# jihun1998/AO

Measured on AMD Instinct MI355X. Metric: points/sec fwd+bwd PTv2m2 S3DIS, higher is better.
Workload: dtype fp32

## Files before the change

ao_amd/_abi.py:

```python
import ctypes
import os
import re

HEADER = os.path.normpath(os.path.join(os.path.dirname(os.path.abspath(__file__)), "..", "include", "ptv2_hip.h"))

_VALUES = {"int": ctypes.c_int, "unsigned": ctypes.c_uint, "float": ctypes.c_float, "double": ctypes.c_double,
           "long long": ctypes.c_longlong, "size_t": ctypes.c_size_t}
_POINTEES = ("void", "char", "unsigned long long")
_TYPE = re.compile(r"\s*(unsigned\s+long\s+long|long\s+long|unsigned\b|\w+)(.*)", re.S)
_DECLARATOR = re.compile(r"\s*((?:\*\s*)*)(\w+)\s*(?:\[([^\]]*)\])?\s*")
_ITEM = re.compile(r"""
    ^[ \t]*\#[ \t]*define[ \t]+(?P<define>\w+)[ \t]+(?P<value>\S.*?)[ \t]*$
  | ^[ \t]*\#[ \t]*(?:include\b.*|ifndef\b.*|endif\b.*|define[ \t]+\w+[ \t]*)$
  | \benum\s*\{(?P<enum>[^{}]*)\}\s*;
  | \btypedef\s+struct\s+(?P<tag>\w+)\s*\{(?P<fields>[^{}]*)\}\s*(?P<struct>\w+)\s*;
  | (?P<result>[\w\s*]+?)\b(?P<function>\w+)\s*\((?P<params>[^(){};]*)\)\s*;
""", re.M | re.X)


def _const_expr(text, consts, where):
    expr = re.sub(r"[A-Za-z_]\w*", lambda m: str(consts[m.group()]) if m.group() in consts else m.group(), text)
    if not re.fullmatch(r"[\d\s+\-*()]+", expr):
        raise RuntimeError("ao_amd: %s: `%s` is not an integer constant expression of known names" % (where, text.strip()))
    try:
        return int(eval(expr, {"__builtins__": {}}))
    except SyntaxError:
        raise RuntimeError("ao_amd: %s: cannot evaluate `%s`" % (where, text.strip())) from None


def _declarations(text, structs, consts, where, fields):
    m = _TYPE.match(re.sub(r"\b(const|volatile)\b", " ", text))
    base = " ".join(m.group(1).split()) if m else None
    out = []
    for decl in m.group(2).split(",") if m else [""]:
        d = _DECLARATOR.fullmatch(decl)
        if d is None:
            raise RuntimeError("ao_amd: %s: cannot read the declaration `%s`" % (where, " ".join(text.split())))
        stars, name, bound = d.group(1).count("*"), d.group(2), d.group(3)
        value = _VALUES.get(base) or (structs.get(base) if fields else None)
        if stars or (bound is not None and not fields):
            if value is None and base not in _POINTEES and base not in structs:
                raise RuntimeError("ao_amd: %s: unknown type `%s` of `%s`" % (where, base, name))
            ctype = ctypes.c_char_p if (base, stars, bound) == ("char", 1, None) else ctypes.c_void_p
        elif value is None:
            raise RuntimeError("ao_amd: %s: no ctypes type for `%s` of `%s`" % (where, base, name))
        else:
            ctype = value
        if bound is not None and fields:
            ctype = ctype * _const_expr(bound, consts, "%s, bound of `%s`" % (where, name))
        out.append((name, ctype))
    return out


def parse(text):
    text = re.sub(r"/\*.*?\*/", " ", text, flags=re.S)
    text = re.sub(r"^[ \t]*#[ \t]*ifdef[ \t]+__cplusplus\b.*?^[ \t]*#[ \t]*endif\b.*?$", " ", text, flags=re.S | re.M)
    consts, structs, signatures = {}, {}, {}
    at = 0
    for m in _ITEM.finditer(text):
        if text[at:m.start()].strip():
            break
        at = m.end()
        if m.group("define"):
            consts[m.group("define")] = _const_expr(m.group("value"), consts, "#define " + m.group("define"))
        elif m.group("enum") is not None:
            value = -1
            for item in filter(None, (i.strip() for i in m.group("enum").split(","))):
                name, _, init = (s.strip() for s in item.partition("="))
                value = _const_expr(init, consts, "enumerator " + name) if init else value + 1
                consts[name] = value
        elif m.group("struct"):
            name = m.group("struct")
            if name != m.group("tag"):
                raise RuntimeError("ao_amd: typedef struct %s is named %s" % (m.group("tag"), name))
            fields = [f for line in m.group("fields").split(";") if line.strip()
                      for f in _declarations(line, structs, consts, "struct " + name, True)]
            structs[name] = type(name, (ctypes.Structure,), {"_fields_": fields})
        elif m.group("function"):
            name, params = m.group("function"), m.group("params").strip()
            where = "prototype of " + name
            (_, restype), = _declarations(m.group("result") + " result", structs, consts, where, False)
            signatures[name] = (restype, [] if params in ("", "void") else [
                ctype for p in params.split(",") for _, ctype in _declarations(p, structs, consts, where, False)])
    rest = text[at:].strip()
    if rest:
        raise RuntimeError("ao_amd: cannot read this declaration of the C header: `%s`" % " ".join(rest.split())[:160])
    return consts, structs, signatures


if not os.path.exists(HEADER):
    raise RuntimeError("ao_amd: %s not found: the ctypes bindings are derived from it" % HEADER)
with open(HEADER) as _f:
    consts, structs, signatures = parse(_f.read())

DATA_HEADER = os.path.join(os.path.dirname(HEADER), "ptv2_data_hip.h")
if not os.path.exists(DATA_HEADER):
    raise RuntimeError("ao_amd: %s not found: the ctypes bindings are derived from it" % DATA_HEADER)
with open(DATA_HEADER) as _f:
    data_consts, data_structs, data_signatures = parse(_f.read())

REFINE_HEADER = os.path.join(os.path.dirname(HEADER), "ptv2_refine_hip.h")
if not os.path.exists(REFINE_HEADER):
    raise RuntimeError("ao_amd: %s not found: the ctypes bindings are derived from it" % REFINE_HEADER)
with open(REFINE_HEADER) as _f:
    refine_consts, refine_structs, refine_signatures = parse(_f.read())

PP2S_HEADER = os.path.join(os.path.dirname(HEADER), "ptv2_pp2s_hip.h")
if not os.path.exists(PP2S_HEADER):
    raise RuntimeError("ao_amd: %s not found: the ctypes bindings are derived from it" % PP2S_HEADER)
with open(PP2S_HEADER) as _f:
    pp2s_consts, pp2s_structs, pp2s_signatures = parse(_f.read())

PTV1_HEADER = os.path.join(os.path.dirname(HEADER), "ptv2_ptv1_hip.h")
if not os.path.exists(PTV1_HEADER):
    raise RuntimeError("ao_amd: %s not found: the ctypes bindings are derived from it" % PTV1_HEADER)
with open(PTV1_HEADER) as _f:
    ptv1_consts, ptv1_structs, ptv1_signatures = parse(_f.read())

SPCONV_HEADER = os.path.join(os.path.dirname(HEADER), "ptv2_spconv_hip.h")
if not os.path.exists(SPCONV_HEADER):
    raise RuntimeError("ao_amd: %s not found: the ctypes bindings are derived from it" % SPCONV_HEADER)
with open(SPCONV_HEADER) as _f:
    spconv_consts, spconv_structs, spconv_signatures = parse(_f.read())

PG_HEADER = os.path.join(os.path.dirname(HEADER), "ptv2_pg_hip.h")
if not os.path.exists(PG_HEADER):
    raise RuntimeError("ao_amd: %s not found: the ctypes bindings are derived from it" % PG_HEADER)
with open(PG_HEADER) as _f:
    pg_consts, pg_structs, pg_signatures = parse(_f.read())

MSC_HEADER = os.path.join(os.path.dirname(HEADER), "ptv2_msc_hip.h")
if not os.path.exists(MSC_HEADER):
    raise RuntimeError("ao_amd: %s not found: the ctypes bindings are derived from it" % MSC_HEADER)
with open(MSC_HEADER) as _f:
    msc_consts, msc_structs, msc_signatures = parse(_f.read())

ST_HEADER = os.path.join(os.path.dirname(HEADER), "ptv2_st_hip.h")
if not os.path.exists(ST_HEADER):
    raise RuntimeError("ao_amd: %s not found: the ctypes bindings are derived from it" % ST_HEADER)
with open(ST_HEADER) as _f:
    st_consts, st_structs, st_signatures = parse(_f.read())

INSEVAL_HEADER = os.path.join(os.path.dirname(HEADER), "ptv2_inseval_hip.h")
if not os.path.exists(INSEVAL_HEADER):
    raise RuntimeError("ao_amd: %s not found: the ctypes bindings are derived from it" % INSEVAL_HEADER)
with open(INSEVAL_HEADER) as _f:
    inseval_consts, inseval_structs, inseval_signatures = parse(_f.read())
```

ao_amd/_lib.py:

```python
import ctypes
import os
import subprocess

import torch

from . import _abi

_HERE = os.path.dirname(os.path.abspath(__file__))
LIB_PATH = os.path.join(_HERE, "lib", "libptv2_hip.so")
CSRC = os.path.join(_HERE, "csrc")

_SIGNATURES = _abi.signatures

_ERR = {1: "PTV2_ERR_ARG (invalid argument)", 2: "PTV2_ERR_WORKSPACE (workspace too small)",
        3: "PTV2_ERR_LAUNCH (HIP launch failed)"}
_lib = None
EXPECTED_ABI = 11
EXPECTED_DATA_ABI = 1
EXPECTED_REFINE_ABI = 1
EXPECTED_PP2S_ABI = 1
EXPECTED_PTV1_ABI = 1
EXPECTED_SPCONV_ABI = 1
EXPECTED_PG_ABI = 1
EXPECTED_MSC_ABI = 1
EXPECTED_ST_ABI = 1
EXPECTED_INSEVAL_ABI = 1


def build(verbose=False):
    cmd = ["make", "-C", CSRC, "-j4", "all"]
    subprocess.check_call(cmd, stdout=None if verbose else subprocess.DEVNULL)
    return LIB_PATH


def lib():
    global _lib
    if _lib is None:
        if not os.path.exists(LIB_PATH):
            raise RuntimeError(
                "ao_amd: %s not found. Build it with `python -c 'import __graft_entry__ as g; g.build()'` "
                "or `make -C ao_amd/csrc` (needs hipcc). There is no CPU fallback." % LIB_PATH)
        handle = ctypes.CDLL(LIB_PATH)
        for table in (_SIGNATURES, _abi.data_signatures, _abi.refine_signatures, _abi.pp2s_signatures,
                      _abi.ptv1_signatures, _abi.spconv_signatures, _abi.pg_signatures, _abi.msc_signatures,
                      _abi.st_signatures, _abi.inseval_signatures):
            for name, (res, args) in table.items():
                try:
                    fn = getattr(handle, name)
                except AttributeError:
                    raise RuntimeError("ao_amd: %s has no `%s` -- stale build; rebuild with `make -C ao_amd/csrc`"
                                       % (LIB_PATH, name)) from None
                fn.restype = res
                fn.argtypes = args
        have = handle.ptv2_abi_version()
        if have != EXPECTED_ABI:
            raise RuntimeError("ao_amd: %s has ABI version %d, the python side expects %d -- stale build; rebuild with "
                               "`make -C ao_amd/csrc`" % (LIB_PATH, have, EXPECTED_ABI))
        have = handle.ptv2_data_abi_version()
        if have != EXPECTED_DATA_ABI:
            raise RuntimeError("ao_amd: %s has data ABI version %d, the python side expects %d -- stale build; rebuild with "
                               "`make -C ao_amd/csrc`" % (LIB_PATH, have, EXPECTED_DATA_ABI))
        have = handle.ptv2_refine_abi_version()
        if have != EXPECTED_REFINE_ABI:
            raise RuntimeError("ao_amd: %s has refine ABI version %d, the python side expects %d -- stale build; rebuild with "
                               "`make -C ao_amd/csrc`" % (LIB_PATH, have, EXPECTED_REFINE_ABI))
        have = handle.ptv2_pp2s_abi_version()
        if have != EXPECTED_PP2S_ABI:
            raise RuntimeError("ao_amd: %s has pp2s ABI version %d, the python side expects %d -- stale build; rebuild with "
                               "`make -C ao_amd/csrc`" % (LIB_PATH, have, EXPECTED_PP2S_ABI))
        have = handle.ptv2_ptv1_abi_version()
        if have != EXPECTED_PTV1_ABI:
            raise RuntimeError("ao_amd: %s has ptv1 ABI version %d, the python side expects %d -- stale build; rebuild with "
                               "`make -C ao_amd/csrc`" % (LIB_PATH, have, EXPECTED_PTV1_ABI))
        have = handle.ptv2_spconv_abi_version()
        if have != EXPECTED_SPCONV_ABI:
            raise RuntimeError("ao_amd: %s has spconv ABI version %d, the python side expects %d -- stale build; rebuild with "
                               "`make -C ao_amd/csrc`" % (LIB_PATH, have, EXPECTED_SPCONV_ABI))
        if handle.ptv2_spconv_struct_bytes(0) != ctypes.sizeof(_abi.spconv_structs["spconv_tables"]):
            raise RuntimeError("ao_amd: spconv_tables is %d bytes in python, %d in %s (stale build)" % (
                ctypes.sizeof(_abi.spconv_structs["spconv_tables"]), handle.ptv2_spconv_struct_bytes(0), LIB_PATH))
        have = handle.ptv2_pg_abi_version()
        if have != EXPECTED_PG_ABI:
            raise RuntimeError("ao_amd: %s has pg ABI version %d, the python side expects %d -- stale build; rebuild with "
                               "`make -C ao_amd/csrc`" % (LIB_PATH, have, EXPECTED_PG_ABI))
        if handle.ptv2_pg_struct_bytes(0) != ctypes.sizeof(_abi.pg_structs["pg_csr"]):
            raise RuntimeError("ao_amd: pg_csr is %d bytes in python, %d in %s (stale build)" % (
                ctypes.sizeof(_abi.pg_structs["pg_csr"]), handle.ptv2_pg_struct_bytes(0), LIB_PATH))
        have = handle.ptv2_msc_abi_version()
        if have != EXPECTED_MSC_ABI:
            raise RuntimeError("ao_amd: %s has msc ABI version %d, the python side expects %d -- stale build; rebuild with "
                               "`make -C ao_amd/csrc`" % (LIB_PATH, have, EXPECTED_MSC_ABI))
        have = handle.ptv2_st_abi_version()
        if have != EXPECTED_ST_ABI:
            raise RuntimeError("ao_amd: %s has st ABI version %d, the python side expects %d -- stale build; rebuild with "
                               "`make -C ao_amd/csrc`" % (LIB_PATH, have, EXPECTED_ST_ABI))
        if handle.ptv2_st_struct_bytes(0) != ctypes.sizeof(_abi.st_structs["st_args"]):
            raise RuntimeError("ao_amd: st_args is %d bytes in python, %d in %s (stale build)" % (
                ctypes.sizeof(_abi.st_structs["st_args"]), handle.ptv2_st_struct_bytes(0), LIB_PATH))
        have = handle.ptv2_inseval_abi_version()
        if have != EXPECTED_INSEVAL_ABI:
            raise RuntimeError("ao_amd: %s has inseval ABI version %d, the python side expects %d -- stale build; rebuild "
                               "with `make -C ao_amd/csrc`" % (LIB_PATH, have, EXPECTED_INSEVAL_ABI))
        for which, name in enumerate(("ptv1_params", "ptv1_norms", "ptv1_grads")):
            if handle.ptv2_ptv1_struct_bytes(which) != ctypes.sizeof(_abi.ptv1_structs[name]):
                raise RuntimeError("ao_amd: %s is %d bytes in python, %d in %s (stale build)" % (
                    name, ctypes.sizeof(_abi.ptv1_structs[name]), handle.ptv2_ptv1_struct_bytes(which), LIB_PATH))
        for which, name in enumerate(("ptv2_aug_step", "ptv2_aug_program")):
            if handle.ptv2_data_struct_bytes(which) != ctypes.sizeof(_abi.data_structs[name]):
                raise RuntimeError("ao_amd: %s is %d bytes in python, %d in %s (stale build)" % (
                    name, ctypes.sizeof(_abi.data_structs[name]), handle.ptv2_data_struct_bytes(which), LIB_PATH))
        _lib = handle
    return _lib


def check_struct(which, mirror):
    have, want = lib().ptv2_struct_bytes(which), ctypes.sizeof(mirror)
    if have != want:
        raise RuntimeError("ao_amd: %s is %d bytes in python, %d in %s (stale build or a drifted mirror)"
                           % (mirror.__name__, want, have, LIB_PATH))


def check(status, what):
    if status != 0:
        raise RuntimeError("ao_amd: %s failed with status %d: %s" % (what, status, _ERR.get(status, "?")))


def stream_ptr():
    return torch.cuda.current_stream().cuda_stream


def require_cuda(*tensors):
    for t in tensors:
        if t is not None and not t.is_cuda:
            raise RuntimeError("ao_amd ops run on the GPU only (got a %s tensor); there is no CPU fallback" % t.device)


def ptr(t):
    return 0 if t is None else t.data_ptr()


_WS = {}


def workspace(nbytes, device):
    nbytes = max(int(nbytes), 256)
    key = (device.index if device.index is not None else torch.cuda.current_device(),
           torch.cuda.current_stream(device).cuda_stream)
    buf = _WS.get(key)
    if buf is None or buf.numel() < nbytes:
        buf = torch.empty(int(nbytes * 1.25) + 4096, dtype=torch.uint8, device=device)
        _WS[key] = buf
    return buf


def kernel_timer(enable, only=None, stride=1):
    L = lib()
    kid = -1
    if only is not None:
        name = ctypes.create_string_buffer(64)
        us, cnt, byt = ctypes.c_double(), ctypes.c_longlong(), ctypes.c_double()
        for i in range(L.ptv2_profile_kernel_count()):
            L.ptv2_profile_read(i, name, ctypes.byref(us), ctypes.byref(cnt), ctypes.byref(byt))
            if name.value.decode() == only:
                kid = i
        if kid < 0:
            raise ValueError("unknown kernel name %r" % only)
    L.ptv2_profile_select(kid)
    L.ptv2_profile_stride(int(stride))
    L.ptv2_profile_enable(1 if enable else 0)


def graph_stats(reset=False):
    out = (ctypes.c_double * 9)()
    lib().ptv2_graph_stats(out, 1 if reset else 0)
    keys = ("scopes", "updated", "instantiated", "declined", "nodes", "capture_us", "update_us", "launch_us", "wait_us")
    return dict(zip(keys, [float(v) for v in out]))


def kernel_timer_read():
    L = lib()
    out = {}
    name = ctypes.create_string_buffer(64)
    us, cnt, byt = ctypes.c_double(), ctypes.c_longlong(), ctypes.c_double()
    for kid in range(L.ptv2_profile_kernel_count()):
        if L.ptv2_profile_read(kid, name, ctypes.byref(us), ctypes.byref(cnt), ctypes.byref(byt)) == 0 and cnt.value > 0:
            out[name.value.decode()] = dict(launches=cnt.value, total_us=us.value, avg_us=us.value / cnt.value,
                                            bytes_per_launch=byt.value)
    return out
```

ao_amd/csrc/abi.hip:

```cpp
#include <algorithm>
#include <cstdlib>
#include <cstring>
#include <mutex>
#include <unordered_map>
#include <vector>

#include "gva_common.h"

extern "C" int ptv2_abi_version(void) { return 11; }

extern "C" long long ptv2_struct_bytes(int which) {
    switch (which) {
        case 0: return (long long)sizeof(ptv2_block);
        case 1: return (long long)sizeof(ptv2_block_grads);
        case 2: return (long long)sizeof(ptv2_model);
        case 3: return (long long)sizeof(ptv2_gva_block);
        case 4: return (long long)sizeof(ptv2_scene_geo);
        default: return -1;
    }
}

namespace { thread_local int g_matmul_bf16 = 0; }
int ptv2_matmul_bf16(void) { return g_matmul_bf16; }
void ptv2_set_matmul_bf16(int on) { g_matmul_bf16 = on ? 1 : 0; }
extern "C" int ptv2_matmul_precision(int bf16) {
    const int prev = g_matmul_bf16;
    if (bf16 >= 0) g_matmul_bf16 = bf16 ? 1 : 0;
    return prev;
}

namespace gva {
namespace { thread_local PtvDrop g_drop{1.f, 0u, 0u}; }
PtvDrop ptv2_attn_drop_current() { return g_drop; }
void ptv2_attn_drop_set(float p, unsigned seed) {
    if (!(p > 0.f)) { g_drop = PtvDrop{1.f, 0u, 0u}; return; }
    const double pp = p < 1.f ? (double)p : 1.0;
    const double t = pp * 4294967296.0;
    g_drop.thresh = t >= 4294967295.0 ? 4294967295u : (unsigned)t;
    if (g_drop.thresh == 0u) g_drop.thresh = 1u;
    g_drop.scale = pp < 1.0 ? (float)(1.0 / (1.0 - pp)) : 0.f;
    g_drop.seed = seed;
}
PtvAttnDropScope::~PtvAttnDropScope() { g_drop = prev; }
}

namespace gva {
namespace {
thread_local int g_defer_depth = 0;
thread_local PtvRiders g_pending{};
__global__ __launch_bounds__(256) void rider_kernel(PtvRiders Rs) { rider_run(Rs, blockIdx.x); }
void launch_alone(const PtvRider &r, hipStream_t st) {
    PtvRiders one{};
    one.count = 1;
    one.r[0] = r;
    hipLaunchKernelGGL(rider_kernel, dim3(r.blocks), dim3(256), 0, st, one);
}
}
bool ptv2_rider_defer_active() {
    static const bool off = ptv2_env_is("AO_AMD_RIDERS", '0');
    return g_defer_depth > 0 && !off;
}
void ptv2_rider_defer_depth(int delta) { g_defer_depth += delta; }
void ptv2_rider_defer(const PtvRider &r, hipStream_t st) {
    if (g_pending.count == RIDER_QUEUE) {
        launch_alone(g_pending.r[0], st);
        for (int i = 1; i < RIDER_QUEUE; ++i) g_pending.r[i - 1] = g_pending.r[i];
        g_pending.count = RIDER_QUEUE - 1;
    }
    g_pending.r[g_pending.count++] = r;
}
PtvRiders ptv2_rider_take() {
    const PtvRiders out = g_pending;
    g_pending.count = 0;
    return out;
}
void ptv2_rider_flush(hipStream_t st) {
    for (int i = 0; i < g_pending.count; ++i) launch_alone(g_pending.r[i], st);
    g_pending.count = 0;
}
int ptv2_rider_drop() {
    const int had = g_pending.count;
    g_pending.count = 0;
    return had;
}
}

#ifndef PTV2_SRC_HASH
#define PTV2_SRC_HASH "unknown"
#endif

extern "C" const char *ptv2_build_info(void) {
    return "libptv2_hip gfx950 (MI355X) src " PTV2_SRC_HASH " hipcc " __VERSION__ " built " __DATE__;
}

extern "C" int basket_scatter_rows_host(float *dst, long long dst_rows, const long long *ids, const float *src, long long rows,
                                        int c) {
    if (!dst || !ids || !src || rows < 0 || c < 1 || dst_rows < 0) return PTV2_ERR_ARG;
    for (long long r = 0; r < rows; ++r)
        if (ids[r] < 0 || ids[r] >= dst_rows) return PTV2_ERR_ARG;
    for (long long r = 0; r < rows; ++r) memcpy(dst + ids[r] * c, src + r * c, sizeof(float) * (size_t)c);
    return PTV2_OK;
}

namespace {
std::mutex g_cnt_mu;
struct CounterKey {
    int device;
    hipStream_t stream;
    bool operator==(const CounterKey &o) const { return device == o.device && stream == o.stream; }
};
struct CounterKeyHash {
    size_t operator()(const CounterKey &k) const { return std::hash<void *>()((void *)k.stream) * 31u + (size_t)k.device; }
};
std::unordered_map<CounterKey, unsigned *, CounterKeyHash> g_counters;
}

unsigned *ptv2_stream_counters(hipStream_t st) {
    int device = 0;
    if (hipGetDevice(&device) != hipSuccess) return nullptr;
    std::lock_guard<std::mutex> lk(g_cnt_mu);
    const CounterKey key{device, st};
    auto it = g_counters.find(key);
    if (it != g_counters.end()) return it->second;
    unsigned *p = nullptr;
    if (hipMalloc((void **)&p, sizeof(unsigned) * PTV2_NUM_COUNTERS) != hipSuccess) return nullptr;
    if (hipMemsetAsync(p, 0, sizeof(unsigned) * PTV2_NUM_COUNTERS, st) != hipSuccess) return nullptr;
    g_counters[key] = p;
    return p;
}

namespace {
const char *kNames[KID_COUNT] = {
    "knn_row_query_kernel [family]", "logits_fwd_kernel [family]", "softmax_rows_kernel [family]", "aggregate_tile_kernel [family]",
    "peb_fwd_kernel [family]", "peb_bwd_kernel<8>", "aggregate_bwd_tile_kernel [family]", "aggregate_bwd_rows_kernel [family]",
    "aggregate_bwd_gv_kernel<8>", "logits_bwd_rows_kernel [family]", "logits_bwd_gather_kernel", "logits_bwd_params_kernel [family]",
    "linear_wgrad_kernel [family]", "bn_stats_kernel", "bn_apply_kernel [family]", "bn_bwd_reduce_kernel [family]",
    "bn_bwd_apply_kernel [family]", "skinny_fwd_kernel", "skinny_bwd_kernel", "rows_gemm_kernel<48, false, 32> [family]",
    "rows_gemm_kernel<48, false, 64> [family]", "rows_gemm_kernel<48, true, 32> [family]", "rows_gemm_kernel<48, true, 64> [family]",
    "rows_gemm_kernel<64, false, 32> [family]", "rows_gemm_kernel<64, false, 64> [family]", "rows_gemm_kernel<64, true, 32> [family]",
    "rows_gemm_kernel<64, true, 64> [family]",
    "attention_bwd_point_kernel<6, 48, 1, true>",
    "attention_bwd_point_kernel<12, 96, 1, false>", "attention_bwd_point_kernel<24, 192, 2, false>",
    "attention_bwd_point_kernel<48, 384, 4, false>", "attention_bwd_point_kernel<64, 512, 4, false>",
    "linear_wgrad_lds_kernel [family]",
    "grouped_wgrad_kernel_jobs", "attention_fwd_point6_kernel",
    "logits_bwd_fused6_kernel<48>", "logits_bwd_fused_kernel<12, 96, 1>", "logits_bwd_fused_kernel<24, 192, 4>",
    "logits_bwd_fused_kernel<48, 384, 4>", "logits_bwd_fused_kernel<64, 512, 4>",
    "bn_bwd_apply_residual_kernel", "bn_bwd_finapply_kernel [family]",
    "attention_fwd_tile_kernel<12, 96, 12>", "attention_fwd_tile_kernel<24, 192, 12>", "attention_fwd_tile_kernel<48, 384, 12>",
    "attention_fwd_tile_kernel<64, 512, 16>", "wp2_wgrad_tile_kernel_jobs",
    "attention_bwd_tile_kernel<12, 96, 8>", "attention_bwd_tile_kernel<24, 192, 8>", "attention_bwd_tile_kernel<48, 384, 8>",
    "attention_bwd_tile_kernel<64, 512, 8>", "aug_points_kernel"};
struct Rec { hipEvent_t a, b; double bytes; };
std::mutex g_mu;
int g_on = 0;
int g_only = -1;
int g_stride = 1;
unsigned g_seen[KID_COUNT];
std::vector<hipEvent_t> g_free;
hipEvent_t take_event() {
    if (!g_free.empty()) { hipEvent_t e = g_free.back(); g_free.pop_back(); return e; }
    hipEvent_t e = nullptr;
    if (hipEventCreate(&e) != hipSuccess) return nullptr;
    return e;
}
std::vector<Rec> g_recs[KID_COUNT];
std::vector<hipEvent_t> g_pending[KID_COUNT];
constexpr int STAMP_CAP = 1 << 15;
unsigned long long *g_stamp_buf = nullptr;
double g_stamp_us_per_tick = 0.01;
int g_stamp_n = 0;
struct StampRec { int slot; double bytes; };
std::vector<StampRec> g_stamp_recs[KID_COUNT];
std::vector<int> g_stamp_pending[KID_COUNT];
unsigned g_scope_period[GRAPH_SLOTS][KID_COUNT];
unsigned g_scope_phase[GRAPH_SLOTS];
thread_local unsigned t_scope_seen[KID_COUNT];
thread_local int t_scope_which = -1;
__global__ void stamp_kernel(unsigned long long *p) {
    if (threadIdx.x == 0) *p = wall_clock64();
// ... 161 lines not shown
```

ao_amd/csrc/common.h:

```cpp
#pragma once
#include <hip/hip_runtime.h>
#include <stdint.h>
#include <stdlib.h>

#include "../../include/ptv2_hip.h"

#define WAVE 64

#define PTV2_CHECK_LAUNCH()                         \
    do {                                            \
        if (hipGetLastError() != hipSuccess) return PTV2_ERR_LAUNCH; \
    } while (0)

#define RUN(call)                        \
    do {                                 \
        int rc_ = (call);                \
        if (rc_ != PTV2_OK) return rc_;  \
    } while (0)

static inline int divup(long long a, long long b) { return (int)((a + b - 1) / b); }

static constexpr size_t ptv2_align256(size_t v) { return (v + 255) & ~(size_t)255; }
struct PtvCarver {
    char *p; size_t off;
    char *take(size_t bytes) { char *r = p ? p + off : nullptr; off += ptv2_align256(bytes); return r; }
    template <class T> T *take_n(size_t count) { return (T *)take(sizeof(T) * count); }
};

static inline bool ptv2_env_set(const char *name) { return getenv(name) != nullptr; }
static inline bool ptv2_env_is(const char *name, char c) { const char *e = getenv(name); return e && e[0] == c; }

enum PtvKernelId {
    KID_KNN_QUERY = 0, KID_LOGITS_FWD, KID_SOFTMAX_ROWS, KID_AGG_TILE, KID_PEB_FWD, KID_PEB_BWD, KID_BWD_TILE,
    KID_BWD_ROWS, KID_BWD_GV, KID_LOGITS_BWD_ROWS, KID_LOGITS_BWD_GATHER, KID_LOGITS_BWD_PARAMS, KID_WGRAD,
    KID_BN_STATS, KID_BN_APPLY, KID_BN_BWD_REDUCE, KID_BN_BWD_APPLY, KID_SKINNY_FWD, KID_SKINNY_BWD, KID_ROWS_GEMM,  KID_BWD_POINT = KID_ROWS_GEMM + 8,
     KID_WGRAD_LDS = KID_BWD_POINT + 5 ,
    KID_WGRAD_GROUPED ,
    KID_FWD_POINT ,
    KID_LOGITS_BWD_FUSED ,
    KID_BN_BWD_APPLY_RES = KID_LOGITS_BWD_FUSED + 5 ,
    KID_BN_BWD_FINAPPLY ,
    KID_FWD_TILE ,
    KID_WGRAD_TILE = KID_FWD_TILE + 4 ,
    KID_BWD_TILE_K ,
    KID_AUG_POINTS = KID_BWD_TILE_K + 4 ,
    KID_COUNT
};
extern "C" int ptv2_profile_is_on(void);
int ptv2_profile_wants(int kid);
void ptv2_profile_begin(int kid, hipStream_t st);
void ptv2_profile_end(int kid, hipStream_t st, double algorithmic_bytes);
struct PtvScopedTimer {
    int kid; hipStream_t st; double bytes; bool on;
    PtvScopedTimer(int k, hipStream_t s, double b) : kid(k), st(s), bytes(b), on(ptv2_profile_wants(k) != 0) {
        if (on) ptv2_profile_begin(kid, st);
    }
    ~PtvScopedTimer() { if (on) ptv2_profile_end(kid, st, bytes); }
};

enum PtvGraphSlot { GRAPH_MODEL_FWD = 0, GRAPH_MODEL_BWD = 1, GRAPH_MODEL_FWD_PREFIX = 2, GRAPH_MODEL_FWD_REST = 3, GRAPH_SLOTS = 4 };
struct PtvGraphScope {
    void *st, *cap; int which, ring_entry; bool active; long long t0;
    PtvGraphScope(void *stream, int which, bool allow = true);
    void *stream() const { return cap; }
    int finish(int rc);
    ~PtvGraphScope();
    PtvGraphScope(const PtvGraphScope &) = delete;
    PtvGraphScope &operator=(const PtvGraphScope &) = delete;
};
int ptv2_graph_capturing(void);
int ptv2_profile_stamps(void);
int ptv2_zero_async(void *p, size_t bytes, hipStream_t st);

void ptv2_wgrad_defer_begin(void *arena, size_t bytes);
bool ptv2_wgrad_defer_active();
float *ptv2_wgrad_defer_alloc(size_t floats);
void ptv2_wgrad_defer_arm(bool on);
void ptv2_wgrad_defer_arm_rs(bool on);
bool ptv2_wgrad_defer_armed_rs();
struct PtvWgradArm {
    explicit PtvWgradArm(bool on) { ptv2_wgrad_defer_arm(on); }
    ~PtvWgradArm() { ptv2_wgrad_defer_arm(false); }
    PtvWgradArm(const PtvWgradArm &) = delete;
    PtvWgradArm &operator=(const PtvWgradArm &) = delete;
};
struct PtvWgradArmRs {
    explicit PtvWgradArmRs(bool on) { ptv2_wgrad_defer_arm_rs(on); }
    ~PtvWgradArmRs() { ptv2_wgrad_defer_arm_rs(false); }
    PtvWgradArmRs(const PtvWgradArmRs &) = delete;
    PtvWgradArmRs &operator=(const PtvWgradArmRs &) = delete;
};
int ptv2_wgrad_defer_flush(void *stream);
void ptv2_wgrad_defer_end();
size_t ptv2_wgrad_defer_table_bytes();

int ptv2_matmul_bf16(void);
void ptv2_set_matmul_bf16(int on);
struct PtvMatmulScope {
    int prev;
    explicit PtvMatmulScope(int on) : prev(ptv2_matmul_bf16()) { ptv2_set_matmul_bf16(on); }
    ~PtvMatmulScope() { ptv2_set_matmul_bf16(prev); }
};
typedef __bf16 ptv2_bf16x8 __attribute__((ext_vector_type(8)));
__device__ __forceinline__ ptv2_bf16x8 ptv2_pack_bf16(float4 lo, float4 hi) {
    ptv2_bf16x8 r;
    r[0] = (__bf16)lo.x; r[1] = (__bf16)lo.y; r[2] = (__bf16)lo.z; r[3] = (__bf16)lo.w;
    r[4] = (__bf16)hi.x; r[5] = (__bf16)hi.y; r[6] = (__bf16)hi.z; r[7] = (__bf16)hi.w;
    return r;
}

static __device__ __attribute__((aligned(16), unused)) float ptv2_zero_pad[1024];
template <class T>
__device__ __forceinline__ T ptv2_ld_or_zero(const T *p, bool ok) {
    return *(ok ? p : (const T *)ptv2_zero_pad);
}

#define PTV2_NUM_COUNTERS 64
enum PtvCounterSlot { CNT_LOGITS_FWD = 0, CNT_BP2, CNT_LOGITS_BWD_ROWS, CNT_CE, CNT_LOVASZ, CNT_BN_TILES = 16  };
unsigned *ptv2_stream_counters(hipStream_t st);

__device__ __forceinline__ float ref_d2(float qx, float qy, float qz, float x, float y, float z) {
    float dx = qx - x, dy = qy - y, dz = qz - z;
    return __builtin_fmaf(dz, dz, __builtin_fmaf(dx, dx, dy * dy));
}

__device__ __forceinline__ int seg_of(int pt, const int *__restrict__ offset, int b) {
    int lo = 0, hi = b - 1;
    while (lo < hi) {
        int mid = (lo + hi) >> 1;
        if (pt < offset[mid]) hi = mid; else lo = mid + 1;
    }
    return lo;
}

__device__ __forceinline__ int f2ord(float f) {
    int i = __float_as_int(f);
    return i >= 0 ? i : i ^ 0x7fffffff;
}
__device__ __forceinline__ float ord2f(int i) {
    return __int_as_float(i >= 0 ? i : i ^ 0x7fffffff);
}

__device__ __forceinline__ unsigned long long shfl_xor_u64(unsigned long long v, int m) {
    unsigned lo = (unsigned)v, hi = (unsigned)(v >> 32);
    lo = __shfl_xor(lo, m, WAVE);
    hi = __shfl_xor(hi, m, WAVE);
    return ((unsigned long long)hi << 32) | lo;
}

__device__ __forceinline__ int xcd_remap(int orig, int nwg) {
    int q = nwg >> 3, r = nwg & 7, x = orig & 7;
    return (x < r ? x * (q + 1) : r * (q + 1) + (x - r) * q) + (orig >> 3);
}

#include "internal.h"
```

ao_amd/csrc/gather_ops.hip:

```cpp
#include "common.h"

namespace {

constexpr int TPB = 256;
inline int grid_for(long long work) { return (int)std::min<long long>(divup(work, TPB), 256 * 8); }

template <int VEC>
__global__ __launch_bounds__(TPB) void grouping_fwd(long long total, int cv, const float *__restrict__ input,
                                                    const int *__restrict__ idx, float *__restrict__ output) {
    for (long long e = (long long)blockIdx.x * TPB + threadIdx.x; e < total; e += (long long)gridDim.x * TPB) {
        long long row = e / cv;
        int ci = (int)(e - row * cv);
        int src = idx[row];
        if (VEC == 4) {
            float4 v = make_float4(0.f, 0.f, 0.f, 0.f);
            if (src >= 0) v = ((const float4 *)input)[(long long)src * cv + ci];
            ((float4 *)output)[e] = v;
        } else {
            output[e] = src >= 0 ? input[(long long)src * cv + ci] : 0.f;
        }
    }
}

__global__ __launch_bounds__(TPB) void grouping_bwd(long long total, int c, const float *__restrict__ grad_output,
// ... 139 lines not shown
}

__global__ __launch_bounds__(TPB) void aggregation_bwd(long long total, int nsample, int c, int w_c,
                                                       const float *__restrict__ input,
                                                       const float *__restrict__ position,
                                                       const float *__restrict__ weight,
                                                       const int *__restrict__ idx,
                                                       const float *__restrict__ grad_output, float *grad_input,
                                                       float *__restrict__ grad_position, float *grad_weight) {
    for (long long e = (long long)blockIdx.x * TPB + threadIdx.x; e < total; e += (long long)gridDim.x * TPB) {
        long long ni = e / c;
        int ci = (int)(e - ni * c);
        int wi = ci % w_c;
        float go = grad_output[e];
        for (int s = 0; s < nsample; ++s) {
            long long ii = ni * nsample + s;
            long long src = (long long)idx[ii] * c + ci;
            float w = weight[ii * w_c + wi];
            atomicAdd(grad_input + src, go * w);
            grad_position[ii * c + ci] = go * w;
            atomicAdd(grad_weight + ii * w_c + wi, go * (input[src] + position[ii * c + ci]));
        }
    }
}

__global__ __launch_bounds__(TPB) void attn_relation_fwd(long long total, int g, int c,
                                                         const float *__restrict__ query,
                                                         const float *__restrict__ key,
                                                         const float *__restrict__ weight,
                                                         const int *__restrict__ tgt, const int *__restrict__ ref,
                                                         float *output) {
    for (long long e = (long long)blockIdx.x * TPB + threadIdx.x; e < total; e += (long long)gridDim.x * TPB) {
        long long r = e / g;
        int gi = (int)(e - r * g);
        const float *q = query + ((long long)tgt[r] * g + gi) * c;
        const float *k = key + ((long long)ref[r] * g + gi) * c;
        float acc = output[e];
        for (int ci = 0; ci < c; ++ci) acc += q[ci] * k[ci] * weight[ci];
        output[e] = acc;
    }
}

__global__ __launch_bounds__(TPB) void attn_relation_bwd(long long total, int g, int c,
                                                         const float *__restrict__ query, float *grad_query,
                                                         const float *__restrict__ key, float *grad_key,
                                                         const float *__restrict__ weight, float *grad_weight,
                                                         const int *__restrict__ tgt, const int *__restrict__ ref,
                                                         const float *__restrict__ grad_output) {
    for (long long e = (long long)blockIdx.x * TPB + threadIdx.x; e < total; e += (long long)gridDim.x * TPB) {
        long long rg = e / c;
        int ci = (int)(e - rg * c);
        long long r = rg / g;
        int gi = (int)(rg - r * g);
        long long qi = ((long long)tgt[r] * g + gi) * c + ci;
        long long ki = ((long long)ref[r] * g + gi) * c + ci;
        float gr = grad_output[rg];
        float qv = query[qi], kv = key[ki], wv = weight[ci];
        atomicAdd(grad_query + qi, gr * kv * wv);
        atomicAdd(grad_key + ki, gr * qv * wv);
        atomicAdd(grad_weight + ci, gr * kv * qv);
    }
}

__global__ __launch_bounds__(TPB) void attn_fusion_fwd(long long total, int g, int c,
                                                       const float *__restrict__ weight,
                                                       const float *__restrict__ value,
                                                       const int *__restrict__ tgt, const int *__restrict__ ref,
                                                       float *output) {
    for (long long e = (long long)blockIdx.x * TPB + threadIdx.x; e < total; e += (long long)gridDim.x * TPB) {
        long long rg = e / c;
        int ci = (int)(e - rg * c);
        long long r = rg / g;
        int gi = (int)(rg - r * g);
        float f = weight[rg] * value[((long long)ref[r] * g + gi) * c + ci];
        atomicAdd(output + ((long long)tgt[r] * g + gi) * c + ci, f);
    }
}

__global__ __launch_bounds__(TPB) void attn_fusion_bwd(long long total, int g, int c,
                                                       const float *__restrict__ weight, float *grad_weight,
                                                       const float *__restrict__ value, float *grad_value,
                                                       const int *__restrict__ tgt, const int *__restrict__ ref,
                                                       const float *__restrict__ grad_output) {
    for (long long e = (long long)blockIdx.x * TPB + threadIdx.x; e < total; e += (long long)gridDim.x * TPB) {
        long long r = e / g;
        int gi = (int)(e - r * g);
        long long oi = ((long long)tgt[r] * g + gi) * c;
        long long vi = ((long long)ref[r] * g + gi) * c;
        float w = weight[e];
        float acc = grad_weight[e];
        for (int ci = 0; ci < c; ++ci) {
            float go = grad_output[oi + ci];
            acc += go * value[vi + ci];
            atomicAdd(grad_value + vi + ci, go * w);
        }
        grad_weight[e] = acc;
    }
}

inline bool aligned16(const void *p) { return ((uintptr_t)p & 15) == 0; }

}

#define ST ((hipStream_t)stream)

extern "C" int grouping_forward_hip_launcher(int m, int nsample, int c, const float *input, const int *idx,
                                             float *output, void *stream) {
    if (m < 0 || nsample < 0 || c < 0) return PTV2_ERR_ARG;
    long long rows = (long long)m * nsample;
    if (rows == 0 || c == 0) return PTV2_OK;
    if (c % 4 == 0 && aligned16(input) && aligned16(output)) {
        long long total = rows * (c / 4);
        hipLaunchKernelGGL(grouping_fwd<4>, dim3(grid_for(total)), dim3(TPB), 0, ST, total, c / 4, input, idx, output);
    } else {
        long long total = rows * c;
        hipLaunchKernelGGL(grouping_fwd<1>, dim3(grid_for(total)), dim3(TPB), 0, ST, total, c, input, idx, output);
    }
    PTV2_CHECK_LAUNCH();
    return PTV2_OK;
}

extern "C" int grouping_backward_hip_launcher(int m, int nsample, int c, const float *grad_output,
                                              const int *idx, float *grad_input, void *stream) {
    if (m < 0 || nsample < 0 || c < 0) return PTV2_ERR_ARG;
    long long total = (long long)m * nsample * c;
    if (total == 0) return PTV2_OK;
    hipLaunchKernelGGL(grouping_bwd, dim3(grid_for(total)), dim3(TPB), 0, ST, total, c, grad_output, idx, grad_input);
    PTV2_CHECK_LAUNCH();
    return PTV2_OK;
}

__global__ __launch_bounds__(256) void interpolation_weights_kernel(long long m, int k, int n, const float *__restrict__ dist2,
                                                                    int *__restrict__ idx, float *__restrict__ weight) {
    for (long long i = (long long)blockIdx.x * 256 + threadIdx.x; i < m; i += (long long)gridDim.x * 256) {
        float r[8];
        float norm = 0.f;
        for (int s = 0; s < k; ++s) {
            r[s & 7] = __fdiv_rn(1.0f, __fadd_rn(__fsqrt_rn(dist2[i * k + s]), 1e-8f));
            norm = __fadd_rn(norm, r[s & 7]);
        }
        for (int s = 0; s < k; ++s) {
            weight[i * k + s] = __fdiv_rn(r[s & 7], norm);
            const int j = idx[i * k + s];
            if (j < 0) idx[i * k + s] = j + n;
        }
    }
}

extern "C" int interpolation_weights_hip_launcher(int m, int k, int n, const float *dist2, int *idx, float *weight, void *stream) {
    if (m < 0 || k < 1 || k > 8 || n < 0) return PTV2_ERR_ARG;
    if (m == 0) return PTV2_OK;
    if (!dist2 || !idx || !weight) return PTV2_ERR_ARG;
    const int nblk = (int)std::min<long long>(((long long)m + 255) / 256, 256 * 8);
    hipLaunchKernelGGL(interpolation_weights_kernel, dim3(nblk), dim3(256), 0, (hipStream_t)stream, (long long)m, k, n, dist2, idx,
                       weight);
    PTV2_CHECK_LAUNCH();
    return PTV2_OK;
}

extern "C" int interpolation_forward_hip_launcher(int n, int c, int k, const float *input, const int *idx,
                                                  const float *weight, float *output, void *stream) {
    if (n < 0 || c < 0 || k < 0) return PTV2_ERR_ARG;
    long long total = (long long)n * c;
    if (total == 0) return PTV2_OK;
    hipLaunchKernelGGL(interpolation_fwd, dim3(grid_for(total)), dim3(TPB), 0, ST, total, c, k, input, idx, weight,
                       output);
    PTV2_CHECK_LAUNCH();
    return PTV2_OK;
}

extern "C" int interpolation_backward_hip_launcher(int n, int c, int k, const float *grad_output,
                                                   const int *idx, const float *weight, float *grad_input,
                                                   void *stream) {
    if (n < 0 || c < 0 || k < 0) return PTV2_ERR_ARG;
    long long total = (long long)n * c;
    if (total == 0) return PTV2_OK;
    hipLaunchKernelGGL(interpolation_bwd, dim3(grid_for(total)), dim3(TPB), 0, ST, total, c, k, grad_output, idx,
                       weight, grad_input);
    PTV2_CHECK_LAUNCH();
    return PTV2_OK;
}

extern "C" int interpolation_backward_gather_hip_launcher(int m, int c, int k, const float *grad_output, const int *inv_ptr,
                                                          const int *inv_rows, const float *weight, float *grad_input,
                                                          void *stream) {
    if (m < 0 || c < 0 || k < 1 || !inv_ptr || !inv_rows) return PTV2_ERR_ARG;
    if ((long long)m * c == 0) return PTV2_OK;
    if (c % 4 == 0 && aligned16(grad_output) && aligned16(grad_input)) {
        const long long total = (long long)m * (c / 4);
        hipLaunchKernelGGL(interpolation_bwd_gather<4>, dim3(grid_for(total)), dim3(TPB), 0, ST, total, c / 4, k, grad_output,
                           inv_ptr, inv_rows, weight, grad_input);
    } else {
        const long long total = (long long)m * c;
        hipLaunchKernelGGL(interpolation_bwd_gather<1>, dim3(grid_for(total)), dim3(TPB), 0, ST, total, c, k, grad_output, inv_ptr,
                           inv_rows, weight, grad_input);
    }
    PTV2_CHECK_LAUNCH();
    return PTV2_OK;
}

extern "C" int subtraction_forward_hip_launcher(int n, int nsample, int c, const float *input1,
                                                const float *input2, const int *idx, float *output,
                                                void *stream) {
    if (n < 0 || nsample < 0 || c < 0) return PTV2_ERR_ARG;
    long long rows = (long long)n * nsample;
    if (rows == 0 || c == 0) return PTV2_OK;
    if (c % 4 == 0 && aligned16(input1) && aligned16(input2) && aligned16(output)) {
        long long total = rows * (c / 4);
        hipLaunchKernelGGL(subtraction_fwd<4>, dim3(grid_for(total)), dim3(TPB), 0, ST, total, nsample, c / 4, input1,
                           input2, idx, output);
    } else {
        long long total = rows * c;
        hipLaunchKernelGGL(subtraction_fwd<1>, dim3(grid_for(total)), dim3(TPB), 0, ST, total, nsample, c, input1,
                           input2, idx, output);
    }
    PTV2_CHECK_LAUNCH();
    return PTV2_OK;
}

extern "C" int subtraction_backward_hip_launcher(int n, int nsample, int c, const int *idx,
                                                 const float *grad_output, float *grad_input1,
                                                 float *grad_input2, void *stream) {
    if (n < 0 || nsample < 0 || c < 0) return PTV2_ERR_ARG;
    long long total = (long long)n * c;
    if (total == 0) return PTV2_OK;
    hipLaunchKernelGGL(subtraction_bwd, dim3(grid_for(total)), dim3(TPB), 0, ST, total, nsample, c, idx, grad_output,
                       grad_input1, grad_input2);
    PTV2_CHECK_LAUNCH();
    return PTV2_OK;
}

extern "C" int aggregation_forward_hip_launcher(int n, int nsample, int c, int w_c, const float *input,
                                                const float *position, const float *weight, const int *idx,
                                                float *output, void *stream) {
    if (n < 0 || nsample < 0 || c < 0 || w_c < 1) return PTV2_ERR_ARG;
    long long total = (long long)n * c;
    if (total == 0) return PTV2_OK;
    hipLaunchKernelGGL(aggregation_fwd, dim3(grid_for(total)), dim3(TPB), 0, ST, total, nsample, c, w_c, input,
                       position, weight, idx, output);
    PTV2_CHECK_LAUNCH();
    return PTV2_OK;
}

extern "C" int aggregation_backward_hip_launcher(int n, int nsample, int c, int w_c, const float *input,
                                                 const float *position, const float *weight, const int *idx,
                                                 const float *grad_output, float *grad_input,
                                                 float *grad_position, float *grad_weight, void *stream) {
    if (n < 0 || nsample < 0 || c < 0 || w_c < 1) return PTV2_ERR_ARG;
    long long total = (long long)n * c;
    if (total == 0) return PTV2_OK;
    hipLaunchKernelGGL(aggregation_bwd, dim3(grid_for(total)), dim3(TPB), 0, ST, total, nsample, c, w_c, input,
                       position, weight, idx, grad_output, grad_input, grad_position, grad_weight);
    PTV2_CHECK_LAUNCH();
    return PTV2_OK;
}

extern "C" int attention_relation_step_forward_hip_launcher(int m, int g, int c, const float *query,
                                                            const float *key, const float *weight,
                                                            const int *index_target, const int *index_refer,
                                                            float *output, void *stream) {
    if (m < 0 || g < 0 || c < 0) return PTV2_ERR_ARG;
    long long total = (long long)m * g;
    if (total == 0) return PTV2_OK;
    hipLaunchKernelGGL(attn_relation_fwd, dim3(grid_for(total)), dim3(TPB), 0, ST, total, g, c, query, key, weight,
                       index_target, index_refer, output);
    PTV2_CHECK_LAUNCH();
    return PTV2_OK;
}

extern "C" int attention_relation_step_backward_hip_launcher(int m, int g, int c, const float *query,
                                                             float *grad_query, const float *key,
                                                             float *grad_key, const float *weight,
                                                             float *grad_weight, const int *index_target,
                                                             const int *index_refer, const float *grad_output,
                                                             void *stream) {
    if (m < 0 || g < 0 || c < 0) return PTV2_ERR_ARG;
    long long total = (long long)m * g * c;
    if (total == 0) return PTV2_OK;
    hipLaunchKernelGGL(attn_relation_bwd, dim3(grid_for(total)), dim3(TPB), 0, ST, total, g, c, query, grad_query, key,
                       grad_key, weight, grad_weight, index_target, index_refer, grad_output);
    PTV2_CHECK_LAUNCH();
    return PTV2_OK;
}

extern "C" int attention_fusion_step_forward_hip_launcher(int m, int g, int c, const float *weight,
                                                          const float *value, const int *index_target,
                                                          const int *index_refer, float *output, void *stream) {
    if (m < 0 || g < 0 || c < 0) return PTV2_ERR_ARG;
    long long total = (long long)m * g * c;
    if (total == 0) return PTV2_OK;
    hipLaunchKernelGGL(attn_fusion_fwd, dim3(grid_for(total)), dim3(TPB), 0, ST, total, g, c, weight, value,
                       index_target, index_refer, output);
    PTV2_CHECK_LAUNCH();
    return PTV2_OK;
}

extern "C" int attention_fusion_step_backward_hip_launcher(int m, int g, int c, const float *weight,
                                                           float *grad_weight, const float *value,
                                                           float *grad_value, const int *index_target,
                                                           const int *index_refer, const float *grad_output,
                                                           void *stream) {
    if (m < 0 || g < 0 || c < 0) return PTV2_ERR_ARG;
    long long total = (long long)m * g;
    if (total == 0) return PTV2_OK;
    hipLaunchKernelGGL(attn_fusion_bwd, dim3(grid_for(total)), dim3(TPB), 0, ST, total, g, c, weight, grad_weight,
                       value, grad_value, index_target, index_refer, grad_output);
    PTV2_CHECK_LAUNCH();
// ... 3 lines not shown
```

ao_amd/csrc/gridpool.hip:

```cpp
#include <hipcub/hipcub.hpp>

#include <algorithm>

#include "common.h"

namespace {

constexpr int TPB = 256;
struct PoolDims {
    long long nx, ny, nz;
    long long total;
};
constexpr int KEY_BITS = 48;

__device__ __forceinline__ PoolDims pool_dims_of(int b, const float *__restrict__ lo, const float *__restrict__ hi, float size) {
    float e[3] = {0.f, 0.f, 0.f};
    for (int s = 0; s < b; ++s)
        for (int a = 0; a < 3; ++a) e[a] = fmaxf(e[a], hi[3 * s + a] - lo[3 * s + a]);
    PoolDims d;
    d.nx = (long long)(e[0] / size) + 1;
    d.ny = (long long)(e[1] / size) + 1;
    d.nz = (long long)(e[2] / size) + 1;
    d.total = d.nx * d.ny * d.nz * (long long)b;
    return d;
}
__global__ void pool_dims_kernel(int b, const float *__restrict__ lo, const float *__restrict__ hi, float size,
                                 PoolDims *dims) {
    if (threadIdx.x != 0 || blockIdx.x != 0) return;
    *dims = pool_dims_of(b, lo, hi, size);
}

__global__ __launch_bounds__(TPB) void pool_keys_kernel(int n, int b, const float *__restrict__ coord,
                                                        const int *__restrict__ offset, const float *__restrict__ lo,
                                                        float size, const PoolDims *__restrict__ dims,
                                                        unsigned long long *__restrict__ keys, int *__restrict__ vals) {
    const int i = blockIdx.x * TPB + threadIdx.x;
    if (i >= n) return;
    const int s = seg_of(i, offset, b);
    const long long cx = (long long)((coord[3 * (size_t)i] - lo[3 * s]) / size);
    const long long cy = (long long)((coord[3 * (size_t)i + 1] - lo[3 * s + 1]) / size);
    const long long cz = (long long)((coord[3 * (size_t)i + 2] - lo[3 * s + 2]) / size);
    const long long nx = dims->nx, ny = dims->ny, nz = dims->nz;
    keys[i] = (unsigned long long)(cx + cy * nx + cz * nx * ny + (long long)s * nx * ny * nz);
    vals[i] = i;
}

__global__ __launch_bounds__(TPB) void pool_heads_kernel(int n, const unsigned long long *__restrict__ keys,
                                                         int *__restrict__ flags) {
    const int i = blockIdx.x * TPB + threadIdx.x;
    if (i >= n) return;
    flags[i] = (i == 0 || keys[i] != keys[i - 1]) ? 1 : 0;
}

__global__ __launch_bounds__(TPB) void pool_scatter_kernel(int n, const int *__restrict__ rank,
                                                           const int *__restrict__ flags, const int *__restrict__ order,
                                                           long long *__restrict__ cluster, int *__restrict__ idx_ptr,
                                                           int *__restrict__ n_out, const PoolDims *__restrict__ dims) {
    const int i = blockIdx.x * TPB + threadIdx.x;
    if (i >= n) return;
    const int r = rank[i] - 1;
    cluster[order[i]] = r;
    if (flags[i]) idx_ptr[r] = i;
    if (i == n - 1) {
        idx_ptr[r + 1] = n;
        *n_out = (dims->total > 0 && dims->total < (1ll << KEY_BITS)) ? r + 1 : -1;
    }
}

__global__ __launch_bounds__(TPB) void pool_mean_kernel(int *n_out, int b,
                                                        const float *__restrict__ coord, const int *__restrict__ offset,
                                                        int *order, const int *__restrict__ idx_ptr,
                                                        float *__restrict__ new_coord, int *__restrict__ new_offset, int sort_members,
                                                        const int *__restrict__ over) {
    if (over && *over) {
        if (blockIdx.x == 0 && threadIdx.x == 0 && *n_out >= 0) *n_out = -2;
        return;
    }
    const int m = *n_out;
    for (int j = blockIdx.x * TPB + threadIdx.x; j < m; j += gridDim.x * TPB) {
        const int p0 = idx_ptr[j], p1 = idx_ptr[j + 1];
        if (sort_members) {
            for (int p = p0 + 1; p < p1; ++p) {
                const int v = order[p];
                int q = p - 1;
                while (q >= p0 && order[q] > v) { order[q + 1] = order[q]; --q; }
                order[q + 1] = v;
            }
        }
        float sx = 0.f, sy = 0.f, sz = 0.f;
        for (int p = p0; p < p1; ++p) {
            const size_t r = (size_t)order[p];
            sx += coord[3 * r]; sy += coord[3 * r + 1]; sz += coord[3 * r + 2];
        }
        const float cnt = (float)(p1 - p0);
        new_coord[3 * (size_t)j] = sx / cnt;
        new_coord[3 * (size_t)j + 1] = sy / cnt;
        new_coord[3 * (size_t)j + 2] = sz / cnt;
        const int s0 = seg_of(order[p0], offset, b);
        const int s1 = (j + 1 < m) ? seg_of(order[idx_ptr[j + 1]], offset, b) : b;
        for (int s = s0; s < s1; ++s) new_offset[s] = j + 1;
        if (j == 0)
            for (int s = 0; s < s0; ++s) new_offset[s] = 0;
    }
}

constexpr long long DENSE_CAP = 1ll << 23;
constexpr int DENSE_MAX_MEMBERS = 64;
constexpr int DSCAN_THREADS = 256, DSCAN_ITEMS = 8, DSCAN_TILE = DSCAN_THREADS * DSCAN_ITEMS;

__global__ __launch_bounds__(TPB) void dense_zero_kernel(int b, const float *__restrict__ lo, const float *__restrict__ hi, float size,
                                                         PoolDims *__restrict__ dims, int *__restrict__ count, int *n_out,
                                                         long long cells_cap, int *__restrict__ over) {
    const PoolDims d = pool_dims_of(b, lo, hi, size);
    if (blockIdx.x == 0 && threadIdx.x == 0) { *dims = d; *over = 0; }
    const long long total = d.total;
    if (total <= 0 || total > cells_cap) {
        if (blockIdx.x == 0 && threadIdx.x == 0) *n_out = (total > 0 && total < (1ll << KEY_BITS)) ? -2 : -1;
        return;
    }
    const long long pad = (total + DSCAN_TILE - 1) / DSCAN_TILE * DSCAN_TILE;
    const int4 z = make_int4(0, 0, 0, 0);
    for (long long i = ((long long)blockIdx.x * TPB + threadIdx.x) * 4; i < pad; i += (long long)gridDim.x * TPB * 4) *(int4 *)(count + i) = z;
    if (blockIdx.x == 0 && threadIdx.x == 0) *n_out = 0;
}

__global__ __launch_bounds__(TPB) void dense_keys_kernel(int n, int b, const float *__restrict__ coord, const int *__restrict__ offset,
                                                         const float *__restrict__ lo, float size, const PoolDims *__restrict__ dims,
                                                         const int *__restrict__ n_out, int *__restrict__ count,
                                                         int *__restrict__ key32, int *__restrict__ slot) {
    const int i = blockIdx.x * TPB + threadIdx.x;
    if (i >= n || *n_out < 0) return;
    const int s = seg_of(i, offset, b);
    const long long cx = (long long)((coord[3 * (size_t)i] - lo[3 * s]) / size);
    const long long cy = (long long)((coord[3 * (size_t)i + 1] - lo[3 * s + 1]) / size);
    const long long cz = (long long)((coord[3 * (size_t)i + 2] - lo[3 * s + 2]) / size);
    const long long nx = dims->nx, ny = dims->ny, nz = dims->nz;
    const int key = (int)(cx + cy * nx + cz * nx * ny + (long long)s * nx * ny * nz);
    key32[i] = key;
    slot[i] = atomicAdd(&count[key], 1);
}

__global__ __launch_bounds__(DSCAN_THREADS) void dense_scan_reduce_kernel(const PoolDims *__restrict__ dims, const int *__restrict__ n_out,
                                                                          const int *__restrict__ count, int2 *__restrict__ tile_sums) {
    if (*n_out < 0 || (long long)blockIdx.x * DSCAN_TILE >= dims->total) return;
    __shared__ int2 s_w[DSCAN_THREADS / WAVE];
    const int4 *p = (const int4 *)(count + (size_t)blockIdx.x * DSCAN_TILE) + threadIdx.x * 2;
    const int4 a = p[0], c = p[1];
    int v = a.x + a.y + a.z + a.w + c.x + c.y + c.z + c.w;
    int o = (a.x > 0) + (a.y > 0) + (a.z > 0) + (a.w > 0) + (c.x > 0) + (c.y > 0) + (c.z > 0) + (c.w > 0);
#pragma unroll
    for (int d = 32; d >= 1; d >>= 1) { v += __shfl_xor(v, d, WAVE); o += __shfl_xor(o, d, WAVE); }
    if ((threadIdx.x & 63) == 0) s_w[threadIdx.x >> 6] = make_int2(v, o);
    __syncthreads();
    if (threadIdx.x == 0) {
        int2 t = make_int2(0, 0);
        for (int i = 0; i < DSCAN_THREADS / WAVE; ++i) { t.x += s_w[i].x; t.y += s_w[i].y; }
        tile_sums[blockIdx.x] = t;
    }
}

__global__ __launch_bounds__(DSCAN_THREADS) void dense_scan_apply_kernel(const PoolDims *__restrict__ dims, int *n_out, int n,
                                                                         const int *__restrict__ count, const int2 *__restrict__ tile_sums,
                                                                         int2 *__restrict__ base, int *__restrict__ idx_ptr,
                                                                         int *__restrict__ over) {
    const long long total = dims->total;
    if (*n_out < 0 || (long long)blockIdx.x * DSCAN_TILE >= total) return;
    __shared__ int2 s_w[DSCAN_THREADS / WAVE];
    __shared__ int2 s_base;
    const int lane = threadIdx.x & 63, wid = threadIdx.x >> 6;
    int2 part = make_int2(0, 0);
    for (int i = threadIdx.x; i < (int)blockIdx.x; i += DSCAN_THREADS) { const int2 t = tile_sums[i]; part.x += t.x; part.y += t.y; }
#pragma unroll
    for (int d = 32; d >= 1; d >>= 1) { part.x += __shfl_xor(part.x, d, WAVE); part.y += __shfl_xor(part.y, d, WAVE); }
    if (lane == 0) s_w[wid] = part;
    __syncthreads();
    if (threadIdx.x == 0) {
        int2 t = make_int2(0, 0);
        for (int i = 0; i < DSCAN_THREADS / WAVE; ++i) { t.x += s_w[i].x; t.y += s_w[i].y; }
        s_base = t;
    }
    __syncthreads();
    const int2 tb = s_base;
    __syncthreads();
    const int4 *p = (const int4 *)(count + (size_t)blockIdx.x * DSCAN_TILE) + threadIdx.x * 2;
    const int4 a = p[0], c = p[1];
    const int v[8] = {a.x, a.y, a.z, a.w, c.x, c.y, c.z, c.w};
    int ex[8], eo[8], tot = 0, occ = 0, big = 0;
#pragma unroll
    for (int i = 0; i < 8; ++i) { ex[i] = tot; eo[i] = occ; tot += v[i]; occ += v[i] > 0; big |= v[i] > DENSE_MAX_MEMBERS; }
    if (big) *over = 1;
    int inc = tot, inco = occ;
#pragma unroll
    for (int d = 1; d < WAVE; d <<= 1) {
        const int y = __shfl_up(inc, d, WAVE), yo = __shfl_up(inco, d, WAVE);
        if (lane >= d) { inc += y; inco += yo; }
    }
    if (lane == 63) s_w[wid] = make_int2(inc, inco);
    __syncthreads();
    int wx = 0, wo = 0;
    for (int i = 0; i < wid; ++i) { wx += s_w[i].x; wo += s_w[i].y; }
    const int bx = tb.x + wx + inc - tot, bo = tb.y + wo + inco - occ;
    int2 *q = base + (size_t)blockIdx.x * DSCAN_TILE + (size_t)threadIdx.x * 8;
#pragma unroll
    for (int i = 0; i < 8; ++i) q[i] = make_int2(bx + ex[i], bo + eo[i]);
    const long long last_tile = (total - 1) / DSCAN_TILE;
    if ((long long)blockIdx.x == last_tile && threadIdx.x == DSCAN_THREADS - 1) {
        const int m = bo + occ;
        *n_out = m;
        idx_ptr[m] = n;
    }
}

__global__ __launch_bounds__(TPB) void dense_scatter_kernel(int n, const int *__restrict__ n_out, const int *__restrict__ key32,
                                                            const int *__restrict__ slot, const int2 *__restrict__ base,
                                                            long long *__restrict__ cluster, int *__restrict__ order,
                                                            int *__restrict__ idx_ptr) {
    const int i = blockIdx.x * TPB + threadIdx.x;
    if (i >= n || *n_out < 0) return;
    const int2 bb = base[key32[i]];
    cluster[i] = bb.y;
    order[bb.x + slot[i]] = i;
    if (slot[i] == 0) idx_ptr[bb.y] = bb.x;
}

struct Ws {
    float *lo, *hi;
    PoolDims *dims;
    unsigned long long *keys_in, *keys_out;
    int *vals_in, *flags, *rank;
    void *mm, *cub;
    size_t mm_bytes, cub_bytes, bytes;
    int *d_count, *d_key, *d_slot, *d_over;
    int2 *d_tiles, *d_base;
    long long d_cells;
};

}

static Ws carve(void *base, int n, int b) {
    Ws w;
    PtvCarver cv{(char *)base, 0};
    w.lo = cv.take_n<float>(3 * b); w.hi = cv.take_n<float>(3 * b);
    w.dims = cv.take_n<PoolDims>(1);
    w.keys_in = cv.take_n<unsigned long long>(n); w.keys_out = cv.take_n<unsigned long long>(n);
    w.vals_in = cv.take_n<int>(n); w.flags = cv.take_n<int>(n); w.rank = cv.take_n<int>(n);
    w.mm_bytes = segment_minmax_hip_workspace_bytes(b);
    w.mm = cv.take(w.mm_bytes);
    size_t s1 = 0, s2 = 0;
    (void)hipcub::DeviceRadixSort::SortPairs(nullptr, s1, (const unsigned long long *)nullptr, (unsigned long long *)nullptr,
                                             (const int *)nullptr, (int *)nullptr, n, 0, 64, (hipStream_t)0);
    (void)hipcub::DeviceScan::InclusiveSum(nullptr, s2, (const int *)nullptr, (int *)nullptr, n, (hipStream_t)0);
    w.cub_bytes = std::max(s1, s2) + 256;
    w.cub = cv.take(w.cub_bytes);
    w.d_cells = std::min<long long>(DENSE_CAP, std::max<long long>(64ll * n, 1 << 16));
    const size_t cells = (size_t)w.d_cells + DSCAN_TILE;
    w.d_count = cv.take_n<int>(cells); w.d_base = cv.take_n<int2>(cells);
    w.d_tiles = cv.take_n<int2>(cells / DSCAN_TILE + 1);
    w.d_key = cv.take_n<int>(n); w.d_slot = cv.take_n<int>(n); w.d_over = cv.take_n<int>(4);
    w.bytes = cv.off;
    return w;
}

extern "C" size_t grid_pool_hip_workspace_bytes(int n, int b) {
    if (n < 1 || b < 1) return 0;
    return carve(nullptr, n, b).bytes + 1024;
}

extern "C" int grid_pool_hip_launcher(int n, int b, const float *coord, const int *offset, float grid_size,
                                      long long *cluster, int *order, int *idx_ptr, float *new_coord,
                                      int *new_offset, int *n_out, int sort_path, void *workspace, size_t workspace_bytes,
                                      void *stream) {
    if (n < 1 || b < 1 || !(grid_size > 0.f)) return PTV2_ERR_ARG;
    Ws w = carve(workspace, n, b);
    if (!workspace || workspace_bytes < w.bytes) return PTV2_ERR_WORKSPACE;
    hipStream_t st = (hipStream_t)stream;
    int rc = segment_minmax_hip_launcher(b, coord, offset, w.lo, w.hi, w.mm, w.mm_bytes, stream);
    if (rc != PTV2_OK) return rc;
    const int nb = divup(n, TPB);
    if (sort_path)
        hipLaunchKernelGGL(pool_dims_kernel, dim3(1), dim3(64), 0, st, b, (const float *)w.lo, (const float *)w.hi, grid_size,
                           w.dims);
    if (!sort_path) {
        const int ztiles = (int)((w.d_cells + DSCAN_TILE) / DSCAN_TILE);
        hipLaunchKernelGGL(dense_zero_kernel, dim3(1024), dim3(TPB), 0, st, b, (const float *)w.lo, (const float *)w.hi, grid_size,
                           w.dims, w.d_count, n_out, w.d_cells, w.d_over);
        hipLaunchKernelGGL(dense_keys_kernel, dim3(nb), dim3(TPB), 0, st, n, b, coord, offset, (const float *)w.lo, grid_size,
                           (const PoolDims *)w.dims, (const int *)n_out, w.d_count, w.d_key, w.d_slot);
        hipLaunchKernelGGL(dense_scan_reduce_kernel, dim3(ztiles), dim3(DSCAN_THREADS), 0, st, (const PoolDims *)w.dims,
                           (const int *)n_out, (const int *)w.d_count, w.d_tiles);
        hipLaunchKernelGGL(dense_scan_apply_kernel, dim3(ztiles), dim3(DSCAN_THREADS), 0, st, (const PoolDims *)w.dims, n_out, n,
                           (const int *)w.d_count, (const int2 *)w.d_tiles, w.d_base, idx_ptr, w.d_over);
        hipLaunchKernelGGL(dense_scatter_kernel, dim3(nb), dim3(TPB), 0, st, n, (const int *)n_out, (const int *)w.d_key,
                           (const int *)w.d_slot, (const int2 *)w.d_base, cluster, order, idx_ptr);
        hipLaunchKernelGGL(pool_mean_kernel, dim3(std::min(nb, 2048)), dim3(TPB), 0, st, n_out, b, coord, offset,
                           order, (const int *)idx_ptr, new_coord, new_offset, 1, (const int *)w.d_over);
        PTV2_CHECK_LAUNCH();
        return PTV2_OK;
    }
    hipLaunchKernelGGL(pool_keys_kernel, dim3(nb), dim3(TPB), 0, st, n, b, coord, offset, (const float *)w.lo, grid_size,
                       (const PoolDims *)w.dims, w.keys_in, w.vals_in);
    size_t cb = w.cub_bytes;
    if (hipcub::DeviceRadixSort::SortPairs(w.cub, cb, (const unsigned long long *)w.keys_in, w.keys_out,
                                           (const int *)w.vals_in, order, n, 0, KEY_BITS, st) != hipSuccess)
        return PTV2_ERR_LAUNCH;
    hipLaunchKernelGGL(pool_heads_kernel, dim3(nb), dim3(TPB), 0, st, n, (const unsigned long long *)w.keys_out, w.flags);
    cb = w.cub_bytes;
    if (hipcub::DeviceScan::InclusiveSum(w.cub, cb, (const int *)w.flags, w.rank, n, st) != hipSuccess) return PTV2_ERR_LAUNCH;
    hipLaunchKernelGGL(pool_scatter_kernel, dim3(nb), dim3(TPB), 0, st, n, (const int *)w.rank, (const int *)w.flags,
                       (const int *)order, cluster, idx_ptr, n_out, (const PoolDims *)w.dims);
    hipLaunchKernelGGL(pool_mean_kernel, dim3(std::min(nb, 2048)), dim3(TPB), 0, st, n_out, b, coord, offset,
                       order, (const int *)idx_ptr, new_coord, new_offset, 0, (const int *)nullptr);
    PTV2_CHECK_LAUNCH();
    return PTV2_OK;
}
```

ao_amd/csrc/gva_fwd.hip:

```cpp
#include <cstdlib>

#include "gva_common.h"

namespace gva {

__global__ __launch_bounds__(TPB) void pos_stats_kernel(int n, int k, const float *__restrict__ coord,
                                                        const int *__restrict__ idx, float *__restrict__ part) {
    __shared__ float s_w[WPB][9];
    const long long rows = (long long)n * k;
    float acc[9] = {0, 0, 0, 0, 0, 0, 0, 0, 0};
    for (long long row = (long long)blockIdx.x * TPB + threadIdx.x; row < rows; row += (long long)gridDim.x * TPB) {
        Rel r = rel_pos(coord, idx, row, (int)(row / k));
        acc[0] += r.x; acc[1] += r.y; acc[2] += r.z;
        acc[3] += r.x * r.x; acc[4] += r.x * r.y; acc[5] += r.x * r.z;
        acc[6] += r.y * r.y; acc[7] += r.y * r.z; acc[8] += r.z * r.z;
    }
#pragma unroll
    for (int j = 0; j < 9; ++j) {
        float v = wave_sum(acc[j]);
        if ((threadIdx.x & 63) == 0) s_w[threadIdx.x >> 6][j] = v;
    }
    __syncthreads();
    if (threadIdx.x < 9) {
        float v = 0.f;
        for (int w = 0; w < WPB; ++w) v += s_w[w][threadIdx.x];
        part[blockIdx.x * 9 + threadIdx.x] = v;
    }
}

struct MapPosStats {
    double *s1, *s2;
    __device__ void operator()(int j, double v) const {
        if (j < 3) { s1[j] = v; return; }
        const int r[6] = {0, 0, 0, 1, 1, 2}, c[6] = {0, 1, 2, 1, 2, 2};
        const int a = r[j - 3], b = c[j - 3];
        s2[a * 3 + b] = v;
        s2[b * 3 + a] = v;
    }
};

#ifndef FWD_RPL
#define FWD_RPL 2
#endif
template <int G, int SPLIT>
__global__ __launch_bounds__(TPB) void logits_fwd_kernel(int n, int k, int c, const float *__restrict__ kW,
                                                         const float *__restrict__ qW, const float *__restrict__ a,
                                                         const float *__restrict__ b, const float *__restrict__ M,
                                                         const float *__restrict__ cW, const float *__restrict__ coord,
                                                         const int *__restrict__ idx, float *__restrict__ W1, float *part,
                                                         unsigned *counter, double *__restrict__ T1,
                                                         double *__restrict__ T2, FoldWFwdArgs F) {
    extern __shared__ float4 lds4[];
    constexpr int G4 = (G + 3) & ~3;
    constexpr int RPL = SPLIT == 1 ? (G <= 8 ? FWD_RPL : 2) : 1;
    constexpr int RPB = TPB / SPLIT * RPL;
    float4 *sAB = lds4;
    float *sM = (float *)(sAB + c);
    float *sRed = sM + (size_t)c * G4;
    __shared__ float s_w[WPB][2 * G];
    for (int i = threadIdx.x; i < c; i += TPB) sAB[i] = make_float4(a[3 * i], a[3 * i + 1], a[3 * i + 2], b[i]);
    for (int e = threadIdx.x; e < c * G; e += TPB) sM[(e / G) * G4 + (e % G)] = M[e];
    __syncthreads();
    const int lane = threadIdx.x & 63, wid = threadIdx.x >> 6;
    const long long rows = (long long)n * k;
    const long long iters = (rows + RPB - 1) / RPB;
    const int cs = (c + SPLIT - 1) / SPLIT;
    const int c0 = SPLIT == 1 ? 0 : wid * cs, c1 = SPLIT == 1 ? c : (c0 + cs < c ? c0 + cs : c);
    const bool finisher = SPLIT == 1 || wid == 0;
    float t1[G], t2[G];
#pragma unroll
    for (int g = 0; g < G; ++g) t1[g] = t2[g] = 0.f;
    for (long long it = blockIdx.x; it < iters; it += gridDim.x) {
        long long row[RPL];
        bool act[RPL];
        int nn[RPL];
        Rel r[RPL];
        float kq[RPL][G], acc[RPL][G];
#pragma unroll
        for (int j = 0; j < RPL; ++j) {
            row[j] = it * RPB + (SPLIT == 1 ? j * TPB + (int)threadIdx.x : lane);
            act[j] = row[j] < rows;
            nn[j] = act[j] ? (int)(row[j] / k) : 0;
            r[j].x = r[j].y = r[j].z = 0.f; r[j].src = -1;
            if (act[j]) r[j] = rel_pos(coord, idx, row[j], nn[j]);
        }
        if (finisher) {
#pragma unroll
            for (int j = 0; j < RPL; ++j)
#pragma unroll
                for (int g = 0; g < G; ++g)
                    kq[j][g] = ptv2_ld_or_zero(kW + (long long)r[j].src * G + g, act[j] && r[j].src >= 0) -
                               ptv2_ld_or_zero(qW + (long long)nn[j] * G + g, act[j]);
        }
#pragma unroll
        for (int j = 0; j < RPL; ++j)
#pragma unroll
            for (int g = 0; g < G; ++g) acc[j][g] = 0.f;
        for (int ci = c0; ci < c1; ++ci) {
            const float4 ab = sAB[ci];
            float p[RPL];
#pragma unroll
            for (int j = 0; j < RPL; ++j) p[j] = pe_act(ab.x, ab.y, ab.z, ab.w, r[j].x, r[j].y, r[j].z);
            const float *mr = sM + (size_t)ci * G4;
            if (G % 4 == 0) {
#pragma unroll
                for (int g = 0; g < G; g += 4) {
                    const float4 m4 = *(const float4 *)(mr + g);
#pragma unroll
                    for (int j = 0; j < RPL; ++j) {
                        acc[j][g] = __builtin_fmaf(p[j], m4.x, acc[j][g]); acc[j][g + 1] = __builtin_fmaf(p[j], m4.y, acc[j][g + 1]);
                        acc[j][g + 2] = __builtin_fmaf(p[j], m4.z, acc[j][g + 2]); acc[j][g + 3] = __builtin_fmaf(p[j], m4.w, acc[j][g + 3]);
                    }
                }
            } else {
#pragma unroll
                for (int g = 0; g < G; g += 2) {
                    const float2 m2 = *(const float2 *)(mr + g);
#pragma unroll
                    for (int j = 0; j < RPL; ++j) {
                        acc[j][g] = __builtin_fmaf(p[j], m2.x, acc[j][g]); acc[j][g + 1] = __builtin_fmaf(p[j], m2.y, acc[j][g + 1]);
                    }
                }
            }
        }
        if (SPLIT > 1) {
            float *mine = sRed + ((size_t)wid * WAVE + lane) * (G + 1);
#pragma unroll
            for (int g = 0; g < G; ++g) mine[g] = acc[0][g];
            __syncthreads();
            if (wid == 0) {
#pragma unroll
                for (int g = 0; g < G; ++g) {
                    float t = 0.f;
#pragma unroll
                    for (int w = 0; w < SPLIT; ++w) t += sRed[((size_t)w * WAVE + lane) * (G + 1) + g];
                    acc[0][g] = t;
                }
            }
        }
#pragma unroll
        for (int j = 0; j < RPL; ++j) {
            if (finisher && act[j]) {
#pragma unroll
                for (int g = 0; g < G; ++g) {
                    acc[j][g] += kq[j][g] + cW[g];
                    t1[g] += acc[j][g];
                    t2[g] = __builtin_fmaf(acc[j][g], acc[j][g], t2[g]);
                }
                float *o = W1 + row[j] * G;
                if (G % 4 == 0) {
#pragma unroll
                    for (int g = 0; g < G; g += 4) *(float4 *)(o + g) = make_float4(acc[j][g], acc[j][g + 1], acc[j][g + 2], acc[j][g + 3]);
                } else {
#pragma unroll
                    for (int g = 0; g < G; g += 2) *(float2 *)(o + g) = make_float2(acc[j][g], acc[j][g + 1]);
                }
            }
        }
        if (SPLIT > 1) __syncthreads();
    }
#pragma unroll
    for (int g = 0; g < G; ++g) {
        const float v1 = wave_sum(t1[g]), v2 = wave_sum(t2[g]);
        if (lane == 0) { s_w[wid][g] = v1; s_w[wid][G + g] = v2; }
    }
    __syncthreads();
    if (threadIdx.x < 2 * G) {
        float v = 0.f;
        for (int w = 0; w < WPB; ++w) v += s_w[w][threadIdx.x];
        part_store(part + (size_t)blockIdx.x * 2 * G + threadIdx.x, v);
    }
    if (counter && last_block_arrives(counter)) finalize_logit_sums(part, gridDim.x, G, T1, T2, F);
}

inline int stage_grid(long long work_items, int per_block) {
    long long b = (work_items + per_block - 1) / per_block;
    return (int)(b < 1 ? 1 : (b > 256 * 8 ? 256 * 8 : b));
}

inline bool pow2(int k) { return k > 0 && (k & (k - 1)) == 0; }

}

using namespace gva;

extern "C" size_t gva_workspace_bytes(int n, int k, int c, int g) {
    if (n < 0 || k < 1 || c < 1 || g < 1) return 0;
    return rows_offset_bytes(c, g) + ptv2_align256(sizeof(float) * (size_t)n * k * g) + 1024;
}

extern "C" int gva_pos_stats_hip_launcher(int n, int k, const float *coord, const int *idx, double *s1, double *s2,
                                          void *workspace, size_t workspace_bytes, void *stream) {
    if (n < 0 || k < 1) return PTV2_ERR_ARG;
    if (!workspace || workspace_bytes < sizeof(float) * 9 * 2048) return PTV2_ERR_WORKSPACE;
    hipStream_t st = (hipStream_t)stream;
    float *part = (float *)workspace;
    int nblk = stage_grid((long long)n * k, TPB * 4);
    hipLaunchKernelGGL(pos_stats_kernel, dim3(nblk), dim3(TPB), 0, st, n, k, coord, idx, part);
    launch_finalize(st, (const float *)part, nblk, 9, MapPosStats{s1, s2});
    PTV2_CHECK_LAUNCH();
    return PTV2_OK;
}

__global__ __launch_bounds__(1024) void pos_moments_finalize_kernel(const float *__restrict__ part, int nblk, double rows,
                                                                    double *__restrict__ mu, double *__restrict__ cov) {
    constexpr int SL = 113;
    __shared__ double s_acc[SL][9];
    __shared__ double s_sum[9];
    const int col = threadIdx.x % 9, sl = threadIdx.x / 9;
    if (sl < SL) {
        double a = 0.0;
        for (int b = sl; b < nblk; b += SL) a += (double)part[(size_t)b * 9 + col];
        s_acc[sl][col] = a;
    }
    __syncthreads();
    if (threadIdx.x < 9) {
        double v = 0.0;
        for (int t = 0; t < SL; ++t) v += s_acc[t][threadIdx.x];
        s_sum[threadIdx.x] = v;
    }
    __syncthreads();
    if (threadIdx.x < 9) {
        const int r[6] = {0, 0, 0, 1, 1, 2}, c[6] = {0, 1, 2, 1, 2, 2};
        if (threadIdx.x < 3) mu[threadIdx.x] = s_sum[threadIdx.x] / rows;
        if (threadIdx.x >= 3) {
            const int a = r[threadIdx.x - 3], b = c[threadIdx.x - 3];
            const double ma = s_sum[a] / rows, mb = s_sum[b] / rows;
            const double v = __dsub_rn(s_sum[threadIdx.x] / rows, __dmul_rn(ma, mb));
            cov[a * 3 + b] = v;
            cov[b * 3 + a] = v;
        }
    }
}

extern "C" int gva_pos_moments_hip_launcher(int n, int k, const float *coord, const int *idx, double *mu, double *cov,
                                            void *workspace, size_t workspace_bytes, void *stream) {
    if (n < 1 || k < 1 || !coord || !idx || !mu || !cov) return PTV2_ERR_ARG;
    if (!workspace || workspace_bytes < sizeof(float) * 9 * 2048) return PTV2_ERR_WORKSPACE;
    hipStream_t st = (hipStream_t)stream;
    float *part = (float *)workspace;
    const int nblk = stage_grid((long long)n * k, TPB * 4);
    hipLaunchKernelGGL(pos_stats_kernel, dim3(nblk), dim3(TPB), 0, st, n, k, coord, idx, part);
    hipLaunchKernelGGL(pos_moments_finalize_kernel, dim3(1), dim3(1024), 0, st, (const float *)part, nblk, (double)n * k, mu, cov);
    PTV2_CHECK_LAUNCH();
    return PTV2_OK;
}

int gva_logits_forward_fold(const GvaPlan &P, int n, int k, int c, int g, const LogitsIn &I, const LogitsOut &O,
                            const FoldWFwdArgs &F, void *workspace, size_t workspace_bytes, void *stream) {
    if (n < 0 || k < 1 || c < 1 || g < 1) return PTV2_ERR_ARG;
    if (!workspace || workspace_bytes < gva_workspace_bytes(n, k, c, g)) return PTV2_ERR_WORKSPACE;
    hipStream_t st = (hipStream_t)stream;
    float *part = (float *)workspace;
    const long long rows = (long long)n * k;
    if (P.logits_fwd != GvaPlan::LF_ROWS) {
        PtvScopedTimer t(KID_LOGITS_FWD, st, 4.0 * ((double)n * k * (g + 1) + (double)n * (3 + 2 * g)));
        const int rc = P.logits_fwd == GvaPlan::LF_MFMA
                           ? gva_logits_fwd_mfma_launch(n, k, c, g, I, O, part, F, st)
                           : gva_logits_point_launch(n, k, c, g, I, O, part, F, st);
        if (rc != PTV2_OK) return rc;
        PTV2_CHECK_LAUNCH();
        return PTV2_OK;
    }
    const int g4 = (g + 3) & ~3;
    const size_t lds_base = sizeof(float4) * (size_t)c + sizeof(float) * (size_t)c * g4;
    const size_t lds_red = sizeof(float) * 4 * WAVE * (g + 1);
    const bool split = rows < 400000 && lds_base + lds_red <= 96 * 1024;
    const size_t lds = lds_base + (split ? lds_red : 0);
    if (lds > 150 * 1024 || g % 2 != 0) return PTV2_ERR_ARG;
    const int nblk = stage_grid(rows, split ? WAVE : (g <= 8 ? FWD_RPL : 2) * TPB);
    const bool own_final = (size_t)nblk * 2 * g <= FUSED_FINAL_MAX;
    unsigned *cnt = own_final ? ptv2_stream_counters(st) : nullptr;
    if (own_final && !cnt) return PTV2_ERR_LAUNCH;
#define CALL(GG)                                                                                                   \
    if (split) {                                                                                                   \
        if (lds > 32 * 1024)                                                                                       \
            (void)hipFuncSetAttribute((const void *)logits_fwd_kernel<GG, 4>, hipFuncAttributeMaxDynamicSharedMemorySize, \
                                      (int)lds);                                                                   \
        hipLaunchKernelGGL((logits_fwd_kernel<GG, 4>), dim3(nblk), dim3(TPB), lds, st, n, k, c, I.kW, I.qW, I.a, I.b, I.M, I.cW, \
                           I.coord, I.idx, O.W1, part, cnt ? cnt + CNT_LOGITS_FWD : nullptr, O.T1, O.T2, F);                       \
    } else {                                                                                                       \
        if (lds > 32 * 1024)                                                                                       \
            (void)hipFuncSetAttribute((const void *)logits_fwd_kernel<GG, 1>, hipFuncAttributeMaxDynamicSharedMemorySize, \
                                      (int)lds);                                                                   \
        hipLaunchKernelGGL((logits_fwd_kernel<GG, 1>), dim3(nblk), dim3(TPB), lds, st, n, k, c, I.kW, I.qW, I.a, I.b, I.M, I.cW, \
                           I.coord, I.idx, O.W1, part, cnt ? cnt + CNT_LOGITS_FWD : nullptr, O.T1, O.T2, F);                       \
    }
    {
        PtvScopedTimer t(KID_LOGITS_FWD, st, 4.0 * ((double)n * k * (g + 1) + (double)n * (3 + 2 * g)));
        GVA_DISPATCH_G(g, CALL)
    }
#undef CALL
    if (!own_final) hipLaunchKernelGGL(finalize_logit_sums_kernel, dim3((g + FLS_GROUPS - 1) / FLS_GROUPS), dim3(1024), 0, st, (const float *)part, nblk, g, O.T1, O.T2, F);
    PTV2_CHECK_LAUNCH();
    return PTV2_OK;
}

extern "C" int gva_logits_forward_hip_launcher(int n, int k, int c, int g, const float *kW, const float *qW,
                                               const float *a, const float *b, const float *M, const float *cW,
                                               const float *coord, const int *idx, float *W1, double *T1, double *T2,
                                               void *workspace, size_t workspace_bytes, void *stream) {
    LogitsIn I{};
    I.kW = kW; I.qW = qW; I.a = a; I.b = b; I.M = M; I.cW = cW; I.coord = coord; I.idx = idx;
    LogitsOut O{};
    O.W1 = W1; O.T1 = T1; O.T2 = T2;
    return gva_logits_forward_fold(gva_plan(n, k, c, g, false, true), n, k, c, g, I, O, FoldWFwdArgs{}, workspace, workspace_bytes, stream);
}
```

ao_amd/csrc/inverse.hip:

```cpp
#include <algorithm>

#include "common.h"

namespace {

constexpr int TPB = 256;
constexpr int INV_MAX = PTV2_INVERSE_MAX_JOBS;
constexpr int CHUNK = 4096;
constexpr int MAX_PARTS = 512;
constexpr int MIN_WIDTH = 256, MAX_WIDTH = 4096;
constexpr int STAGE = 12288;
constexpr int SCAN_TPB = 1024, SCAN_ITEMS = 4, SCAN_TILE = SCAN_TPB * SCAN_ITEMS;
constexpr int GROUP = 16, GROUPS = TPB / GROUP;
struct InvJobs {
    int count;
    int n[INV_MAX];
    const int *idx[INV_MAX];
    int *inv_ptr[INV_MAX];
    int *inv_rows[INV_MAX];
    int rows[INV_MAX];
    int shift[INV_MAX];
    int parts[INV_MAX];
    int chunks[INV_MAX];
    int row0[INV_MAX + 1];
    int chunk0[INV_MAX + 1];
    int part0[INV_MAX + 1];
    int cell0[INV_MAX + 1];
};

__device__ __forceinline__ int job_of(const int *starts, int count, int v) {
    int t = 0;
    while (t + 1 < count && v >= starts[t + 1]) ++t;
    return t;
}

__device__ __forceinline__ int key_of(int v, int n) { return ((unsigned)v < (unsigned)n) ? v + 1 : 0; }

template <bool SPREAD>
__global__ __launch_bounds__(TPB) void inv_split_kernel(InvJobs J, int *__restrict__ cells, int2 *__restrict__ pairs,
                                                        unsigned long long *__restrict__ handoff, int handoff_words,
                                                        int cells_used, int cells_padded) {
    __shared__ int s_part[MAX_PARTS];
    const int t = job_of(J.chunk0, J.count, blockIdx.x);
    const int chunk = blockIdx.x - J.chunk0[t], parts = J.parts[t], chunks = J.chunks[t], shift = J.shift[t], n = J.n[t];
    int *cell = cells + J.cell0[t] + chunk;
    if (!SPREAD && blockIdx.x == 0) {
        for (int i = threadIdx.x; i < handoff_words; i += TPB) handoff[i] = 0ull;
        for (int i = cells_used + threadIdx.x; i < cells_padded; i += TPB) cells[i] = 0;
    }
    for (int p = threadIdx.x; p < parts; p += TPB) s_part[p] = SPREAD ? cell[(size_t)p * chunks] : 0;
    __syncthreads();
    const int *idx = J.idx[t];
    const int r0 = chunk * CHUNK, r1 = min(r0 + CHUNK, J.rows[t]);
    for (int r = r0 + threadIdx.x; r < r1; r += TPB) {
        const int key = key_of(idx[r], n);
        const int place = atomicAdd(&s_part[key >> shift], 1);
        if (SPREAD) pairs[place] = make_int2(r, key);
    }
    if (!SPREAD) {
        __syncthreads();
        for (int p = threadIdx.x; p < parts; p += TPB) cell[(size_t)p * chunks] = s_part[p];
    }
}

__global__ __launch_bounds__(SCAN_TPB) void inv_scan_kernel(int *__restrict__ cells, unsigned long long *__restrict__ handoff) {
    __shared__ int s_wave[SCAN_TPB / 64];
    __shared__ int s_base;
    const int tid = threadIdx.x, lane = tid & 63, wid = tid >> 6, b = blockIdx.x;
    int4 *at = (int4 *)(cells + (size_t)b * SCAN_TILE + tid * SCAN_ITEMS);
    const int4 v = *at;
    const int tsum = v.x + v.y + v.z + v.w;
    int incl = tsum;
#pragma unroll
    for (int d = 1; d < 64; d <<= 1) {
        const int o = __shfl_up(incl, d, 64);
        if (lane >= d) incl += o;
    }
    if (lane == 63) s_wave[wid] = incl;
    __syncthreads();
    int wave_excl = 0, total = 0;
#pragma unroll
    for (int w = 0; w < SCAN_TPB / 64; ++w) {
        const int s = s_wave[w];
        if (w < wid) wave_excl += s;
        total += s;
    }
    if (tid == 0)
        __hip_atomic_store(handoff + b, (1ull << 32) | (unsigned)total, __ATOMIC_RELEASE, __HIP_MEMORY_SCOPE_AGENT);
    int before = 0;
    for (int i = tid; i < b; i += SCAN_TPB) {
        unsigned long long w;
        do {
            w = __hip_atomic_load(handoff + i, __ATOMIC_ACQUIRE, __HIP_MEMORY_SCOPE_AGENT);
            if (!(w >> 32)) __builtin_amdgcn_s_sleep(1);
        } while (!(w >> 32));
        before += (int)(unsigned)w;
    }
#pragma unroll
    for (int d = 32; d >= 1; d >>= 1) before += __shfl_xor(before, d, 64);
    __syncthreads();
    if (lane == 0) s_wave[wid] = before;
    __syncthreads();
    if (tid == 0) {
        int s = 0;
        for (int w = 0; w < SCAN_TPB / 64; ++w) s += s_wave[w];
        s_base = s;
    }
    __syncthreads();
    const int e0 = s_base + wave_excl + incl - tsum;
    *at = make_int4(e0, e0 + v.x, e0 + v.x + v.y, e0 + v.x + v.y + v.z);
}

template <typename Src>
__device__ __forceinline__ void order_bucket(Src src, int s, int *__restrict__ dst, int l) {
    if (s <= GROUP) {
        const int mine = l < s ? src(l) : 0x7fffffff;
        int rank = 0;
#pragma unroll
        for (int q = 0; q < GROUP; ++q) rank += __shfl(mine, q, GROUP) < mine;
        if (l < s) dst[rank] = mine;
        return;
    }
    for (int e = l; e < s; e += GROUP) {
        const int mine = src(e);
        int rank = 0;
        for (int q = 0; q < s; ++q) rank += src(q) < mine;
        dst[rank] = mine;
    }
}

__global__ __launch_bounds__(TPB) void inv_build_kernel(InvJobs J, const int *__restrict__ cells, const int2 *__restrict__ pairs,
                                                        int *__restrict__ spill) {
    extern __shared__ int lds[];
    const int t = job_of(J.part0, J.count, blockIdx.x);
    const int p = blockIdx.x - J.part0[t], shift = J.shift[t], width = 1 << shift, n = J.n[t], chunks = J.chunks[t];
    int *s_start = lds;
    int *s_cur = lds + width + 1;
    int *s_stage = s_cur + width;
    __shared__ int s_wave[TPB / 64];
    const int tid = threadIdx.x, lane = tid & 63, wid = tid >> 6;
    const int *cell = cells + J.cell0[t] + (size_t)p * chunks;
    const int P0 = cell[0];
    const int P1 = (p + 1 < J.parts[t]) ? cell[chunks] : J.row0[t] + J.rows[t];
    const int S = P1 - P0, key0 = p << shift;
    for (int i = tid; i < width; i += TPB) s_cur[i] = 0;
    __syncthreads();
    for (int i = tid; i < S; i += TPB) atomicAdd(&s_cur[pairs[P0 + i].y - key0], 1);
    __syncthreads();
    const int per = width / TPB;
    int c[MAX_WIDTH / TPB], tsum = 0;
#pragma unroll
    for (int q = 0; q < MAX_WIDTH / TPB; ++q)
        if (q < per) { c[q] = s_cur[tid * per + q]; tsum += c[q]; }
    int incl = tsum;
#pragma unroll
    for (int d = 1; d < 64; d <<= 1) {
        const int o = __shfl_up(incl, d, 64);
        if (lane >= d) incl += o;
    }
    if (lane == 63) s_wave[wid] = incl;
    __syncthreads();
    int run = incl - tsum;
    for (int w = 0; w < wid; ++w) run += s_wave[w];
    int *inv_ptr = J.inv_ptr[t];
    const int base = P0 - J.row0[t];
#pragma unroll
    for (int q = 0; q < MAX_WIDTH / TPB; ++q)
        if (q < per) {
            const int kl = tid * per + q;
            s_start[kl] = run;
            s_cur[kl] = run;
            run += c[q];
            if (key0 + kl <= n) inv_ptr[key0 + kl] = base + run;
        }
    if (tid == TPB - 1) s_start[width] = run;
    __syncthreads();
    const bool staged = S <= STAGE;
    int *place = staged ? s_stage : spill + P0;
    if (staged) {
        for (int i = tid; i < S; i += TPB) {
            const int2 m = pairs[P0 + i];
            s_stage[atomicAdd(&s_cur[m.y - key0], 1)] = m.x;
        }
    } else {
        for (int i = tid; i < S; i += TPB) {
            const int2 m = pairs[P0 + i];
            place[atomicAdd(&s_cur[m.y - key0], 1)] = m.x;
        }
        __threadfence_block();
    }
    __syncthreads();
    int *inv_rows = J.inv_rows[t] + base;
    const int l = tid & (GROUP - 1);
    for (int kl = tid >> 4; kl < width; kl += GROUPS) {
        const int m0 = s_start[kl], s = s_start[kl + 1] - m0;
        if (s == 0) continue;
        if (staged) {
            const int *src = s_stage + m0;
            order_bucket([src](int e) { return src[e]; }, s, inv_rows + m0, l);
        } else {
            const int *src = place + m0;
            order_bucket([src](int e) { return __builtin_nontemporal_load(src + e); }, s, inv_rows + m0, l);
        }
    }
}

struct Plan {
    InvJobs J;
    int total_chunks, total_parts, cells_used, cells_padded, scan_wgs, max_width;
    long long total_rows;
    size_t cell_bytes, handoff_bytes, pair_bytes, spill_bytes;
};

int make_plan(int count, const ptv2_inverse_job *jobs, Plan &P) {
    if (count < 1 || count > INV_MAX || !jobs) return PTV2_ERR_ARG;
    InvJobs &J = P.J;
    J.count = count;
    long long rows = 0, chunks = 0, parts = 0, cells = 0;
    P.max_width = MIN_WIDTH;
    for (int t = 0; t < count; ++t) {
        const ptv2_inverse_job &j = jobs[t];
        if (j.n < 1 || j.k < 1) return PTV2_ERR_ARG;
        const long long r = (long long)j.n * j.k;
        int shift = 8;
        while ((((long long)j.n + 1 + (1 << shift) - 1) >> shift) > MAX_PARTS) ++shift;
        if ((1 << shift) > MAX_WIDTH) return PTV2_ERR_ARG;
        P.max_width = std::max(P.max_width, 1 << shift);
        J.n[t] = j.n; J.idx[t] = j.idx; J.inv_ptr[t] = j.inv_ptr; J.inv_rows[t] = j.inv_rows;
        J.rows[t] = (int)r;
        J.shift[t] = shift;
        J.parts[t] = (int)(((long long)j.n + 1 + (1 << shift) - 1) >> shift);
        J.chunks[t] = (int)((r + CHUNK - 1) / CHUNK);
        J.row0[t] = (int)rows; J.chunk0[t] = (int)chunks; J.part0[t] = (int)parts; J.cell0[t] = (int)cells;
        rows += r;
        chunks += J.chunks[t];
        parts += J.parts[t];
        cells += (long long)J.parts[t] * J.chunks[t];
        if (rows >= (1ll << 31) || cells >= (1ll << 30)) return PTV2_ERR_ARG;
    }
    for (int t = count; t <= INV_MAX; ++t) {
        J.row0[t] = (int)rows; J.chunk0[t] = (int)chunks; J.part0[t] = (int)parts; J.cell0[t] = (int)cells;
        if (t < INV_MAX) {
            J.n[t] = 0; J.rows[t] = 0; J.shift[t] = 8; J.parts[t] = 0; J.chunks[t] = 0;
            J.idx[t] = nullptr; J.inv_ptr[t] = nullptr; J.inv_rows[t] = nullptr;
        }
    }
    P.total_rows = rows;
    P.total_chunks = (int)chunks;
    P.total_parts = (int)parts;
    P.cells_used = (int)cells;
    P.scan_wgs = (int)((cells + SCAN_TILE - 1) / SCAN_TILE);
    P.cells_padded = P.scan_wgs * SCAN_TILE;
    P.cell_bytes = ptv2_align256(sizeof(int) * (size_t)P.cells_padded);
    P.handoff_bytes = ptv2_align256(sizeof(unsigned long long) * (size_t)P.scan_wgs);
    P.pair_bytes = ptv2_align256(sizeof(int2) * (size_t)rows);
    P.spill_bytes = ptv2_align256(sizeof(int) * (size_t)rows);
    return PTV2_OK;
}

size_t build_lds_bytes(int width) { return sizeof(int) * ((size_t)2 * width + 1 + STAGE); }

}

extern "C" size_t inverse_tables_hip_workspace_bytes(int count, const ptv2_inverse_job *jobs) {
    Plan P;
    if (make_plan(count, jobs, P) != PTV2_OK) return 0;
    return P.cell_bytes + P.handoff_bytes + P.pair_bytes + P.spill_bytes + 1024;
}

extern "C" int inverse_tables_hip_launcher(int count, const ptv2_inverse_job *jobs, void *workspace, size_t workspace_bytes,
                                           void *stream) {
    Plan P;
    const int rc = make_plan(count, jobs, P);
    if (rc != PTV2_OK) return rc;
    for (int t = 0; t < count; ++t)
        if (!jobs[t].idx || !jobs[t].inv_ptr || !jobs[t].inv_rows) return PTV2_ERR_ARG;
    if (!workspace || workspace_bytes < P.cell_bytes + P.handoff_bytes + P.pair_bytes + P.spill_bytes) return PTV2_ERR_WORKSPACE;
    hipStream_t st = (hipStream_t)stream;
    char *p = (char *)workspace;
    int *cells = (int *)p;                                     p += P.cell_bytes;
    unsigned long long *handoff = (unsigned long long *)p;     p += P.handoff_bytes;
    int2 *pairs = (int2 *)p;                                   p += P.pair_bytes;
    int *spill = (int *)p;
    const size_t lds = build_lds_bytes(P.max_width);
    static bool raised = [] {
        return hipFuncSetAttribute((const void *)inv_build_kernel, hipFuncAttributeMaxDynamicSharedMemorySize,
                                   (int)build_lds_bytes(MAX_WIDTH)) == hipSuccess;
    }();
    if (!raised) return PTV2_ERR_LAUNCH;
    const dim3 chunks((unsigned)P.total_chunks);
    hipLaunchKernelGGL(inv_split_kernel<false>, chunks, dim3(TPB), 0, st, P.J, cells, pairs, handoff, P.scan_wgs, P.cells_used,
                       P.cells_padded);
    hipLaunchKernelGGL(inv_scan_kernel, dim3((unsigned)P.scan_wgs), dim3(SCAN_TPB), 0, st, cells, handoff);
    hipLaunchKernelGGL(inv_split_kernel<true>, chunks, dim3(TPB), 0, st, P.J, cells, pairs, handoff, P.scan_wgs, P.cells_used,
                       P.cells_padded);
    hipLaunchKernelGGL(inv_build_kernel, dim3((unsigned)P.total_parts), dim3(TPB), lds, st, P.J, (const int *)cells,
                       (const int2 *)pairs, spill);
    PTV2_CHECK_LAUNCH();
    return PTV2_OK;
}

extern "C" size_t inverse_table_hip_workspace_bytes(int n, int k) {
    if (n < 1 || k < 1) return 0;
    const ptv2_inverse_job job = {n, k, nullptr, nullptr, nullptr};
    return inverse_tables_hip_workspace_bytes(1, &job);
}

extern "C" int inverse_table_hip_launcher(int n, int k, const int *idx, int *inv_ptr, int *inv_rows, void *workspace,
                                          size_t workspace_bytes, void *stream) {
    const ptv2_inverse_job job = {n, k, idx, inv_ptr, inv_rows};
    return inverse_tables_hip_launcher(1, &job, workspace, workspace_bytes, stream);
}
```

ao_amd/csrc/knn.hip:

```cpp
#include <cstdlib>

#include "common.h"

namespace {

struct SegGrid {
    float minx, miny, minz, h, inv_h;
    int gx, gy, gz, cell_base, n_pts, start;
    int pad;
};

struct Workspace {
    int *tie_count;
    int *bbox_lo;
    int *bbox_hi;
    SegGrid *seg;
    int *block_sums;
    int *cell_count;
    int *cell_start;
    int *point_cell;
    int *point_rank;
    float4 *sorted;
    int *tie_list;
    size_t bytes;
};

constexpr int CELLS_PER_POINT = 4;
constexpr int SCAN_ITEMS = 8;
constexpr int SCAN_THREADS = 256;
constexpr int SCAN_TILE = SCAN_ITEMS * SCAN_THREADS;

Workspace carve(void *base, int m, int n, int b) {
    Workspace w;
    size_t ncell = (size_t)CELLS_PER_POINT * n + b + 1;
    size_t ncell_pad = (size_t)divup(ncell + 1, SCAN_TILE) * SCAN_TILE;
    PtvCarver cv{(char *)base, 0};
    w.tie_count = cv.take_n<int>(4);
    w.bbox_lo = cv.take_n<int>(3 * b); w.bbox_hi = cv.take_n<int>(3 * b);
    w.seg = cv.take_n<SegGrid>(b);
    w.block_sums = cv.take_n<int>(ncell_pad / SCAN_TILE + 1);
    w.cell_count = cv.take_n<int>(ncell_pad); w.cell_start = cv.take_n<int>(ncell_pad + 1);
    w.point_cell = cv.take_n<int>(n); w.point_rank = cv.take_n<int>(n);
    w.sorted = cv.take_n<float4>(n);
    w.tie_list = cv.take_n<int>(m > 0 ? m : 1);
    w.bytes = cv.off;
    return w;
}

__global__ void knn_init_kernel(int *tie_count, int *bbox_lo, int *bbox_hi, int b, int *cell_count,
                                int ncell_pad, int *block_sums, int ntiles) {
    int t = blockIdx.x * blockDim.x + threadIdx.x;
    for (int i = t; i < ntiles; i += gridDim.x * blockDim.x) block_sums[i] = 0;
    if (t < 4) tie_count[t] = 0;
    if (t < 3 * b) {
        bbox_lo[t] = 0x7fffffff;
        bbox_hi[t] = (int)0x80000000;
    }
    for (int i = t; i < ncell_pad; i += gridDim.x * blockDim.x) cell_count[i] = 0;
}

__global__ __launch_bounds__(256) void knn_bbox_kernel(int n, const float *__restrict__ xyz,
                                                       const int *__restrict__ offset, int b,
                                                       int *bbox_lo, int *bbox_hi) {
    __shared__ int s_lo[3], s_hi[3];
    int t = blockIdx.x * 256 + threadIdx.x;
    int first = blockIdx.x * 256, last = min(first + 255, n - 1);
    int seg_first = seg_of(first, offset, b), seg_last = seg_of(last, offset, b);
    bool valid = t < n;
    float x = 0, y = 0, z = 0;
    if (valid) {
        x = xyz[3 * t];
        y = xyz[3 * t + 1];
        z = xyz[3 * t + 2];
    }
    if (seg_first == seg_last) {
        if (threadIdx.x < 3) {
            s_lo[threadIdx.x] = 0x7fffffff;
            s_hi[threadIdx.x] = (int)0x80000000;
        }
        __syncthreads();
        float v[3] = {x, y, z};
#pragma unroll
        for (int a = 0; a < 3; ++a) {
            int lo = valid ? f2ord(v[a]) : 0x7fffffff, hi = valid ? f2ord(v[a]) : (int)0x80000000;
#pragma unroll
            for (int o = 32; o >= 1; o >>= 1) {
                lo = min(lo, __shfl_xor(lo, o, WAVE));
                hi = max(hi, __shfl_xor(hi, o, WAVE));
            }
            if ((threadIdx.x & 63) == 0) {
                atomicMin(&s_lo[a], lo);
                atomicMax(&s_hi[a], hi);
            }
        }
        __syncthreads();
        if (threadIdx.x < 3) {
            atomicMin(&bbox_lo[seg_first * 3 + threadIdx.x], s_lo[threadIdx.x]);
            atomicMax(&bbox_hi[seg_first * 3 + threadIdx.x], s_hi[threadIdx.x]);
        }
    } else if (valid) {
        int s = seg_of(t, offset, b);
        atomicMin(&bbox_lo[s * 3 + 0], f2ord(x));
        atomicMax(&bbox_hi[s * 3 + 0], f2ord(x));
        atomicMin(&bbox_lo[s * 3 + 1], f2ord(y));
        atomicMax(&bbox_hi[s * 3 + 1], f2ord(y));
        atomicMin(&bbox_lo[s * 3 + 2], f2ord(z));
        atomicMax(&bbox_hi[s * 3 + 2], f2ord(z));
    }
}

__device__ __forceinline__ int cell_coord(float v, float lo, float inv_h, int g) {
    float c = floorf((v - lo) * inv_h);
    c = fminf(fmaxf(c, 0.f), (float)(g - 1));
    return (int)c;
}

__device__ __forceinline__ SegGrid seg_grid_of(int s, const int *__restrict__ offset, const int *bbox_lo, const int *bbox_hi,
                                               float occupancy) {
    int start = s == 0 ? 0 : offset[s - 1];
    int cnt = offset[s] - start;
    SegGrid g;
    g.start = start;
    g.n_pts = cnt > 0 ? cnt : 0;
    g.cell_base = CELLS_PER_POINT * start + s;
    g.gx = g.gy = g.gz = 1;
    g.minx = g.miny = g.minz = 0.f;
    g.h = 1.f;
    g.inv_h = 1.f;
    g.pad = 0;
    if (cnt > 0) {
        float lo[3], ext[3];
        for (int a = 0; a < 3; ++a) {
            lo[a] = ord2f(bbox_lo[s * 3 + a]);
            ext[a] = fmaxf(ord2f(bbox_hi[s * 3 + a]) - lo[a], 0.f);
        }
        float emax = fmaxf(fmaxf(ext[0], ext[1]), fmaxf(ext[2], 1e-12f));
        float vol = 1.f;
        for (int a = 0; a < 3; ++a) vol *= fmaxf(ext[a], emax * (1.f / 64.f));
        float h = cbrtf(vol * occupancy / (float)cnt);
        h = fmaxf(h, emax * (1.f / 1000.f));
        int gx, gy, gz;
        for (int it = 0; it < 200; ++it) {
            gx = (int)fminf(floorf(ext[0] / h) + 1.f, 1024.f);
            gy = (int)fminf(floorf(ext[1] / h) + 1.f, 1024.f);
            gz = (int)fminf(floorf(ext[2] / h) + 1.f, 1024.f);
            if ((long long)gx * gy * gz <= (long long)cnt * CELLS_PER_POINT) break;
            h *= 1.08f;
        }
        if ((long long)gx * gy * gz > (long long)cnt * CELLS_PER_POINT) { gx = gy = gz = 1; h = emax * 2.f + 1.f; }
        g.gx = gx; g.gy = gy; g.gz = gz;
        g.h = h;
        g.inv_h = 1.f / h;
        g.minx = lo[0]; g.miny = lo[1]; g.minz = lo[2];
    }
    return g;
}

constexpr int COUNT_SEGS = 64;
__global__ __launch_bounds__(256) void knn_cell_count_kernel(int n, const float *__restrict__ xyz,
                                                             const int *__restrict__ offset, int b,
                                                             const int *bbox_lo, const int *bbox_hi, float occupancy,
                                                             SegGrid *seg, int *cell_count, int *point_cell,
                                                             int *point_rank) {
    __shared__ SegGrid s_grid[COUNT_SEGS];
    const int first = blockIdx.x * 256, last = min(first + 255, n - 1);
    const int s0 = seg_of(first, offset, b), s1 = seg_of(last, offset, b);
    for (int s = s0 + (int)threadIdx.x; s <= s1; s += 256) {
        const SegGrid g = seg_grid_of(s, offset, bbox_lo, bbox_hi, occupancy);
        if (s - s0 < COUNT_SEGS) s_grid[s - s0] = g;
        if (g.n_pts > 0 && g.start >= first) seg[s] = g;
    }
    if (blockIdx.x == 0)
        for (int s = (int)threadIdx.x; s < b; s += 256) {
            const int start = s == 0 ? 0 : offset[s - 1];
            if (offset[s] - start <= 0) seg[s] = seg_grid_of(s, offset, bbox_lo, bbox_hi, occupancy);
        }
    __syncthreads();
    int t = first + threadIdx.x;
    if (t >= n) return;
    int s = seg_of(t, offset, b);
    const SegGrid g = (s - s0 < COUNT_SEGS) ? s_grid[s - s0] : seg_grid_of(s, offset, bbox_lo, bbox_hi, occupancy);
    int cx = cell_coord(xyz[3 * t], g.minx, g.inv_h, g.gx);
    int cy = cell_coord(xyz[3 * t + 1], g.miny, g.inv_h, g.gy);
    int cz = cell_coord(xyz[3 * t + 2], g.minz, g.inv_h, g.gz);
    int cell = g.cell_base + (cz * g.gy + cy) * g.gx + cx;
    point_cell[t] = cell;
    point_rank[t] = atomicAdd(&cell_count[cell], 1);
}

__global__ __launch_bounds__(SCAN_THREADS) void knn_scan_kernel(const int *__restrict__ in, int *block_sums, int *out, int ntiles) {
    __shared__ int s_w[SCAN_THREADS / WAVE];
    __shared__ int s_base;
    int lane = threadIdx.x & 63, wid = threadIdx.x >> 6;
    {
        const int4 *p = (const int4 *)(in + (size_t)blockIdx.x * SCAN_TILE) + threadIdx.x * 2;
        const int4 a = p[0], c = p[1];
        int v = a.x + a.y + a.z + a.w + c.x + c.y + c.z + c.w;
#pragma unroll
        for (int o = 32; o >= 1; o >>= 1) v += __shfl_xor(v, o, WAVE);
        if (lane == 0) s_w[wid] = v;
        __syncthreads();
        if (threadIdx.x == 0) {
            int t = 0;
            for (int i = 0; i < SCAN_THREADS / WAVE; ++i) t += s_w[i];
            __hip_atomic_store(block_sums + blockIdx.x, (int)(0x80000000u | (unsigned)t), __ATOMIC_RELEASE, __HIP_MEMORY_SCOPE_AGENT);
        }
        __syncthreads();
    }
    int part = 0;
    for (int i = threadIdx.x; i < (int)blockIdx.x; i += SCAN_THREADS) {
        int w;
        do {
            w = __hip_atomic_load(block_sums + i, __ATOMIC_ACQUIRE, __HIP_MEMORY_SCOPE_AGENT);
            if (w >= 0) __builtin_amdgcn_s_sleep(1);
        } while (w >= 0);
        part += w & 0x7fffffff;
    }
#pragma unroll
    for (int o = 32; o >= 1; o >>= 1) part += __shfl_xor(part, o, WAVE);
    if (lane == 0) s_w[wid] = part;
    __syncthreads();
    if (threadIdx.x == 0) {
        int t = 0;
        for (int i = 0; i < SCAN_THREADS / WAVE; ++i) t += s_w[i];
        s_base = t;
    }
    __syncthreads();
    int base = s_base;
    __syncthreads();
    const int4 *p = (const int4 *)(in + (size_t)blockIdx.x * SCAN_TILE) + threadIdx.x * 2;
    int4 a = p[0], c = p[1];
    int v[8] = {a.x, a.y, a.z, a.w, c.x, c.y, c.z, c.w};
    int tot = 0;
#pragma unroll
    for (int i = 0; i < 8; ++i) { int x = v[i]; v[i] = tot; tot += x; }
    int inc = tot;
#pragma unroll
    for (int o = 1; o < WAVE; o <<= 1) {
        int y = __shfl_up(inc, o, WAVE);
        if (lane >= o) inc += y;
    }
    if (lane == 63) s_w[wid] = inc;
    __syncthreads();
    int wbase = 0;
    for (int i = 0; i < wid; ++i) wbase += s_w[i];
    int tbase = base + wbase + inc - tot;
    int4 *q = (int4 *)(out + (size_t)blockIdx.x * SCAN_TILE) + threadIdx.x * 2;
    q[0] = make_int4(tbase + v[0], tbase + v[1], tbase + v[2], tbase + v[3]);
    q[1] = make_int4(tbase + v[4], tbase + v[5], tbase + v[6], tbase + v[7]);
    if (blockIdx.x == ntiles - 1 && threadIdx.x == SCAN_THREADS - 1)
        out[(size_t)ntiles * SCAN_TILE] = tbase + tot;
}

__global__ __launch_bounds__(256) void knn_scatter_kernel(int n, const float *__restrict__ xyz,
                                                          const int *__restrict__ cell_start,
                                                          const int *__restrict__ point_cell,
                                                          const int *__restrict__ point_rank,
                                                          float4 *sorted) {
    int t = blockIdx.x * 256 + threadIdx.x;
    if (t >= n) return;
    int pos = cell_start[point_cell[t]] + point_rank[t];
    sorted[pos] = make_float4(xyz[3 * t], xyz[3 * t + 1], xyz[3 * t + 2], __int_as_float(t));
}

template <int KC>
__device__ __forceinline__ void topk_insert(float (&bd)[KC], int (&bi)[KC], float d2, int id) {
#pragma unroll
    for (int j = KC - 1; j > 0; --j) {
        bool shift = d2 < bd[j - 1];
        bool here = !shift && d2 < bd[j];
        float nd = shift ? bd[j - 1] : (here ? d2 : bd[j]);
        int ni = shift ? bi[j - 1] : (here ? id : bi[j]);
        bd[j] = nd;
        bi[j] = ni;
    }
    if (d2 < bd[0]) { bd[0] = d2; bi[0] = id; }
}

template <int KC>
__device__ __forceinline__ void scan_range(const float4 *__restrict__ sorted, int p0, int p1, float qx,
                                           float qy, float qz, float (&bd)[KC], int (&bi)[KC], unsigned &visited) {
    visited += (unsigned)(p1 - p0);
    for (int p = p0; p < p1; ++p) {
        float4 c = sorted[p];
        float d2 = ref_d2(qx, qy, qz, c.x, c.y, c.z);
        if (d2 < bd[KC - 1]) topk_insert<KC>(bd, bi, d2, __float_as_int(c.w));
    }
}

template <int KC, bool COUNT>
__global__ __launch_bounds__(256) void knn_grid_query_kernel(
    int m, int k, const float4 *__restrict__ sorted, const float *__restrict__ new_xyz,
    const int *__restrict__ offset, const int *__restrict__ new_offset, int b,
    const SegGrid *__restrict__ seg, const int *__restrict__ cell_start, int *__restrict__ idx,
    float *__restrict__ dist2, int pad_with_start, int self_mode, int *tie_count, int *tie_list,
    unsigned long long *pairs) {
    int t = blockIdx.x * 256 + threadIdx.x;
    unsigned visited = 0;
    if (t >= m) return;
    int qid, s;
    float qx, qy, qz;
    if (self_mode) {
        float4 p = sorted[t];
        qx = p.x; qy = p.y; qz = p.z;
        qid = __float_as_int(p.w);
        s = seg_of(qid, offset, b);
    } else {
        qid = t;
        qx = new_xyz[3 * t]; qy = new_xyz[3 * t + 1]; qz = new_xyz[3 * t + 2];
        s = seg_of(t, new_offset, b);
    }
    const SegGrid g = seg[s];
    float bd[KC];
    int bi[KC];
#pragma unroll
    for (int j = 0; j < KC; ++j) { bd[j] = 1e10f; bi[j] = -1; }

    if (g.n_pts > 0) {
        const int cx = cell_coord(qx, g.minx, g.inv_h, g.gx);
        const int cy = cell_coord(qy, g.miny, g.inv_h, g.gy);
        const int cz = cell_coord(qz, g.minz, g.inv_h, g.gz);
        const int rmax = max(max(max(cx, g.gx - 1 - cx), max(cy, g.gy - 1 - cy)), max(cz, g.gz - 1 - cz));
        const float fx = (qx - g.minx) * g.inv_h, fy = (qy - g.miny) * g.inv_h, fz = (qz - g.minz) * g.inv_h;
        const float h2 = g.h * g.h, inv_h2 = g.inv_h * g.inv_h;
        auto gap = [](float f, int c) { return fmaxf(fmaxf(fmaxf((float)c - f, f - (float)(c + 1)), 0.f) - 0.01f, 0.f); };
        for (int R = 1;; ++R) {
            const int z0 = max(cz - R, 0), z1 = min(cz + R, g.gz - 1);
            const int y0 = max(cy - R, 0), y1 = min(cy + R, g.gy - 1);
            const int xa = max(cx - R, 0), xb = min(cx + R, g.gx - 1);
            for (int z = z0; z <= z1; ++z) {
                const float dz = gap(fz, z);
                for (int y = y0; y <= y1; ++y) {
                    const float dy = gap(fy, y);
                    const float base2 = (dz * dz + dy * dy) * h2;
                    if (base2 >= bd[KC - 1]) continue;
                    const int row = g.cell_base + (z * g.gy + y) * g.gx;
                    const bool full = (R == 1) || (z - cz == R) || (cz - z == R) || (y - cy == R) || (cy - y == R);
                    if (full) {
                        int xlo = xa, xhi = xb;
                        if (bd[KC - 1] < 1e10f) {
                            const float r = sqrtf((bd[KC - 1] - base2) * inv_h2) * 1.0001f + 0.03f;
                            xlo = max(xa, (int)floorf(fmaxf(fx - r, -1.f)));
                            xhi = min(xb, (int)floorf(fminf(fx + r, 1.0e6f)));
                        }
                        if (xlo <= xhi)
                            scan_range<KC>(sorted, cell_start[row + xlo], cell_start[row + xhi + 1], qx, qy, qz, bd, bi, visited);
                    } else {
                        if (cx - R >= 0) {
                            const float dx = gap(fx, cx - R);
                            if (dx * dx * h2 + base2 < bd[KC - 1])
                                scan_range<KC>(sorted, cell_start[row + cx - R], cell_start[row + cx - R + 1], qx, qy, qz, bd, bi, visited);
                        }
                        if (cx + R <= g.gx - 1) {
                            const float dx = gap(fx, cx + R);
                            if (dx * dx * h2 + base2 < bd[KC - 1])
                                scan_range<KC>(sorted, cell_start[row + cx + R], cell_start[row + cx + R + 1], qx, qy, qz, bd, bi, visited);
                        }
                    }
                }
            }
            if (R >= rmax) break;
            const float lim = ((float)R - 0.01f) * g.h;
            if (bd[KC - 1] < lim * lim) break;
        }
    }

    if (COUNT) atomicAdd(pairs, (unsigned long long)visited);
    bool tie = false;
#pragma unroll
    for (int j = 0; j + 1 < KC; ++j)
        if (j < k && bd[j] == bd[j + 1] && bd[j + 1] < 1e10f) tie = true;
    if (tie) tie_list[atomicAdd(tie_count, 1)] = qid;

    const int pad = pad_with_start ? g.start : -1;
    int *orow = idx + (size_t)qid * k;
    float *drow = dist2 + (size_t)qid * k;
    if (k == KC - 1 && (KC - 1) % 4 == 0) {
#pragma unroll
        for (int j = 0; j < KC - 1; j += 4) {
            int4 iv = make_int4(bd[j] < 1e10f ? bi[j] : pad, bd[j + 1] < 1e10f ? bi[j + 1] : pad,
                                bd[j + 2] < 1e10f ? bi[j + 2] : pad, bd[j + 3] < 1e10f ? bi[j + 3] : pad);
            *(int4 *)(orow + j) = iv;
            *(float4 *)(drow + j) = make_float4(bd[j], bd[j + 1], bd[j + 2], bd[j + 3]);
        }
    } else {
#pragma unroll
        for (int j = 0; j < KC - 1; ++j)
            if (j < k) {
                orow[j] = bd[j] < 1e10f ? bi[j] : pad;
                drow[j] = bd[j];
            }
    }
}

__device__ __forceinline__ float row_shr1_f(float x, float fill) {
    return __int_as_float(__builtin_amdgcn_update_dpp(__float_as_int(fill), __float_as_int(x), 0x111, 0xf, 0xf, false));
}
__device__ __forceinline__ int row_shr1_i(int x, int fill) { return __builtin_amdgcn_update_dpp(fill, x, 0x111, 0xf, 0xf, false); }
__device__ __forceinline__ float row_shl1_f(float x, float fill) {
    return __int_as_float(__builtin_amdgcn_update_dpp(__float_as_int(fill), __float_as_int(x), 0x101, 0xf, 0xf, false));
}
__device__ __forceinline__ float row_min16(float x) {
    x = fminf(x, __int_as_float(__builtin_amdgcn_update_dpp(0, __float_as_int(x), 0x121, 0xf, 0xf, false)));
    x = fminf(x, __int_as_float(__builtin_amdgcn_update_dpp(0, __float_as_int(x), 0x122, 0xf, 0xf, false)));
    x = fminf(x, __int_as_float(__builtin_amdgcn_update_dpp(0, __float_as_int(x), 0x124, 0xf, 0xf, false)));
    x = fminf(x, __int_as_float(__builtin_amdgcn_update_dpp(0, __float_as_int(x), 0x128, 0xf, 0xf, false)));
    return x;
}

struct RowList {
    float v;
    int vi;
    float tau;
    float e;
};
template <int K>
__device__ __forceinline__ float row_kth(float v, int km1) {
    if constexpr (K > 0) return __int_as_float(__builtin_amdgcn_update_dpp(0, __float_as_int(v), 0x150 + (K - 1), 0xf, 0xf, false));
    else return __shfl(v, km1, 16);
}

template <int STRIDE>
__device__ __forceinline__ void row_cmpx(float &d, int &id, bool up) {
    const float od = __int_as_float(__builtin_amdgcn_ds_swizzle(__float_as_int(d), (STRIDE << 10) | 0x1f));
    const int oi = __builtin_amdgcn_ds_swizzle(id, (STRIDE << 10) | 0x1f);
    const bool take = up ? (od < d) : (od > d);
    d = take ? od : d;
    id = take ? oi : id;
}
__device__ __forceinline__ void row_sort16(float &d, int &id, int r) {
    row_cmpx<1>(d, id, ((r & 1) == 0) == ((r & 2) == 0));
    row_cmpx<2>(d, id, ((r & 2) == 0) == ((r & 4) == 0));
    row_cmpx<1>(d, id, ((r & 1) == 0) == ((r & 4) == 0));
    row_cmpx<4>(d, id, ((r & 4) == 0) == ((r & 8) == 0));
    row_cmpx<2>(d, id, ((r & 2) == 0) == ((r & 8) == 0));
    row_cmpx<1>(d, id, ((r & 1) == 0) == ((r & 8) == 0));
    row_cmpx<8>(d, id, (r & 8) == 0);
    row_cmpx<4>(d, id, (r & 4) == 0);
    row_cmpx<2>(d, id, (r & 2) == 0);
    row_cmpx<1>(d, id, (r & 1) == 0);
}

template <int K>
__device__ __forceinline__ void row_scan_range(const float4 *__restrict__ sorted, int p0, int p1, float qx, float qy, float qz,
                                               int km1, int r, int lane, RowList &L, unsigned &visited) {
    visited += (unsigned)(p1 - p0);
    for (int p = p0; p < p1; p += 16) {
        const bool have = p + r < p1;
        const float4 c = ptv2_ld_or_zero(sorted + p + r, have);
        float d2 = have ? ref_d2(qx, qy, qz, c.x, c.y, c.z) : 3.0e38f;
        int id = __float_as_int(c.w);
        const bool surv = d2 < L.tau;
        unsigned my = (unsigned)((__ballot(surv) >> (lane & 48)) & 0xffffull);
        if (__popc(my) >= 7) {
            row_sort16(d2, id, r);
            const float rd = __int_as_float(__builtin_amdgcn_update_dpp(0, __float_as_int(d2), 0x140, 0xf, 0xf, false));
            const int ri = __builtin_amdgcn_update_dpp(0, id, 0x140, 0xf, 0xf, false);
            const bool keep = L.v <= rd;
            L.e = fminf(L.e, keep ? rd : L.v);
            L.v = keep ? L.v : rd;
            L.vi = keep ? L.vi : ri;
            row_cmpx<8>(L.v, L.vi, (r & 8) == 0);
            row_cmpx<4>(L.v, L.vi, (r & 4) == 0);
            row_cmpx<2>(L.v, L.vi, (r & 2) == 0);
            row_cmpx<1>(L.v, L.vi, (r & 1) == 0);
            L.tau = row_kth<K>(L.v, km1);
            continue;
        }
        L.e = fminf(L.e, surv ? 3.0e38f : d2);
        while (my) {
            const int src = __builtin_ctz(my);
            my &= my - 1;
            const float cd = __shfl(d2, src, 16);
            const int ci = __shfl(id, src, 16);
            if (cd < L.tau) {
                const bool gt = L.v > cd;
                const float vp = row_shr1_f(L.v, cd);
                const int ip = row_shr1_i(L.vi, ci);
                const int gtp = row_shr1_i(gt ? 1 : 0, 0);
                if (r == 15) L.e = fminf(L.e, L.v);
                L.v = gt ? (gtp ? vp : cd) : L.v;
                L.vi = gt ? (gtp ? ip : ci) : L.vi;
                L.tau = row_kth<K>(L.v, km1);
            } else {
                L.e = fminf(L.e, cd);
            }
        }
    }
}

struct RowRange { int p0, p1; float lb2; };
__device__ __forceinline__ RowRange ring_slot(const SegGrid &g, const int *__restrict__ cell_start, int R, int u, int cx, int cy, int cz,
                                              float fx, float fy, float fz, float tau) {
    RowRange out{0, 0, 3.0e38f};
    const int w = 2 * R + 1;
    int t, side;
    if (R == 1) { t = u; side = 0; } else { t = u >> 1; side = u & 1; }
    if (t >= w * w) return out;
    const int dz = t / w - R, dy = t - (t / w) * w - R;
    const int z = cz + dz, y = cy + dy;
    if (z < 0 || z >= g.gz || y < 0 || y >= g.gy) return out;
    auto gap = [](float f, int c) { return fmaxf(fmaxf(fmaxf((float)c - f, f - (float)(c + 1)), 0.f) - 0.01f, 0.f); };
    const float h2 = g.h * g.h;
    const float gz_ = gap(fz, z), gy_ = gap(fy, y);
    const float base2 = (gz_ * gz_ + gy_ * gy_) * h2;
    if (base2 > tau) return out;
    const int row = g.cell_base + (z * g.gy + y) * g.gx;
    const bool shell = (R == 1) || (dz == R) || (dz == -R) || (dy == R) || (dy == -R);
    if (shell) {
        if (side) return out;
        int xlo = max(cx - R, 0), xhi = min(cx + R, g.gx - 1);
        if (tau < 1e10f) {
            const float rr = sqrtf((tau - base2) * g.inv_h * g.inv_h) * 1.0001f + 0.03f;
            xlo = max(xlo, (int)floorf(fmaxf(fx - rr, -1.f)));
            xhi = min(xhi, (int)floorf(fminf(fx + rr, 1.0e6f)));
        }
        if (xlo > xhi) return out;
        out.p0 = cell_start[row + xlo];
        out.p1 = cell_start[row + xhi + 1];
        out.lb2 = base2;
    } else {
        const int x = side ? cx + R : cx - R;
        if (x < 0 || x >= g.gx) return out;
        const float gx_ = gap(fx, x);
        const float lb = gx_ * gx_ * h2 + base2;
        if (lb > tau) return out;
        out.p0 = cell_start[row + x];
        out.p1 = cell_start[row + x + 1];
        out.lb2 = lb;
    }
    return out;
}

template <int K, bool COUNT>
__global__ __launch_bounds__(256) void knn_row_query_kernel(
    int m, int k, const float4 *__restrict__ sorted, const float *__restrict__ new_xyz,
    const int *__restrict__ offset, const int *__restrict__ new_offset, int b,
    const SegGrid *__restrict__ seg, const int *__restrict__ cell_start, int *__restrict__ idx,
    float *__restrict__ dist2, int pad_with_start, int self_mode, int *tie_count, int *tie_list,
    unsigned long long *pairs) {
    const int lane = threadIdx.x & 63, r = lane & 15;
    const int t = (int)(((long long)blockIdx.x * 256 + threadIdx.x) >> 4);
    unsigned visited = 0;
    if (t >= m) return;
    int qid, s;
    float qx, qy, qz;
    if (self_mode) {
        const float4 p = sorted[t];
        qx = p.x; qy = p.y; qz = p.z;
        qid = __float_as_int(p.w);
        s = seg_of(qid, offset, b);
    } else {
        qid = t;
        qx = new_xyz[3 * (size_t)t]; qy = new_xyz[3 * (size_t)t + 1]; qz = new_xyz[3 * (size_t)t + 2];
        s = seg_of(t, new_offset, b);
    }
    const SegGrid g = seg[s];
    const int km1 = k - 1;
    RowList L;
    L.v = 1e10f; L.vi = -1; L.tau = 1e10f; L.e = 1e10f;

    if (g.n_pts > 0) {
        const int cx = cell_coord(qx, g.minx, g.inv_h, g.gx);
        const int cy = cell_coord(qy, g.miny, g.inv_h, g.gy);
        const int cz = cell_coord(qz, g.minz, g.inv_h, g.gz);
        const int rmax = max(max(max(cx, g.gx - 1 - cx), max(cy, g.gy - 1 - cy)), max(cz, g.gz - 1 - cz));
        const float fx = (qx - g.minx) * g.inv_h, fy = (qy - g.miny) * g.inv_h, fz = (qz - g.minz) * g.inv_h;
        for (int R = 1;; ++R) {
            const int w = 2 * R + 1;
            const int slots = R == 1 ? w * w : 2 * w * w;
            for (int u0 = 0; u0 < slots; u0 += 16) {
                const RowRange mine = ring_slot(g, cell_start, R, u0 + r, cx, cy, cz, fx, fy, fz, L.tau);
                unsigned todo = (unsigned)((__ballot(mine.p0 < mine.p1) >> (lane & 48)) & 0xffffull);
                while (todo) {
                    const int j = __builtin_ctz(todo);
                    todo &= todo - 1;
                    const float lb2 = __shfl(mine.lb2, j, 16);
                    if (lb2 > L.tau) continue;
                    const int p0 = __shfl(mine.p0, j, 16), p1 = __shfl(mine.p1, j, 16);
                    row_scan_range<K>(sorted, p0, p1, qx, qy, qz, km1, r, lane, L, visited);
                }
            }
            if (R >= rmax) break;
            const float lim = ((float)R - 0.01f) * g.h;
            if (L.tau < lim * lim) break;
        }
    }

    if (COUNT && r == 0) atomicAdd(pairs, (unsigned long long)visited);
    const float vn = row_shl1_f(L.v, 3.0e38f);
    const float e = row_min16(fminf(L.e, r >= k ? L.v : 3.0e38f));
    bool tie = (r + 1 < k && L.v == vn && vn < 1e10f) || (r == km1 && L.v == e && e < 1e10f);
    const unsigned any = (unsigned)((__ballot(tie) >> (lane & 48)) & 0xffffull);
    if (any && r == 0) tie_list[atomicAdd(tie_count, 1)] = qid;
    if (r < k) {
        const int pad = pad_with_start ? g.start : -1;
        idx[(size_t)qid * k + r] = L.v < 1e10f ? L.vi : pad;
        dist2[(size_t)qid * k + r] = L.v;
    }
}

constexpr int EX_WAVES = 4;

__device__ __forceinline__ void ex_reheap(volatile float *hd, volatile int *hi, int k) {
    int root = 0, child = 1;
    while (child < k) {
        if (child + 1 < k && hd[child + 1] > hd[child]) child++;
        if (hd[root] > hd[child]) return;
        float td = hd[root]; hd[root] = hd[child]; hd[child] = td;
        int ti = hi[root]; hi[root] = hi[child]; hi[child] = ti;
        root = child;
        child = root * 2 + 1;
    }
}

__global__ __launch_bounds__(EX_WAVES *WAVE) void knn_exact_kernel(
    int m, int k, const float *__restrict__ xyz, const float *__restrict__ new_xyz,
    const int *__restrict__ offset, const int *__restrict__ new_offset, int b, int *__restrict__ idx,
    float *__restrict__ dist2, int pad_with_start, const int *__restrict__ tie_count,
    const int *__restrict__ tie_list, int all_queries) {
    __shared__ float s_d[EX_WAVES][128];
    __shared__ int s_i[EX_WAVES][128];
    const int lane = threadIdx.x & 63, wid = threadIdx.x >> 6;
    volatile float *hd = s_d[wid];
    volatile int *hi = s_i[wid];
    const int total = all_queries ? m : *tie_count;
    const int nwaves = gridDim.x * EX_WAVES;
    for (int w = blockIdx.x * EX_WAVES + wid; w < total; w += nwaves) {
        const int q = all_queries ? w : tie_list[w];
        const int s = seg_of(q, new_offset, b);
        const int start = s == 0 ? 0 : offset[s - 1];
        const int end = offset[s];
        const float qx = new_xyz[3 * q], qy = new_xyz[3 * q + 1], qz = new_xyz[3 * q + 2];
        for (int j = lane; j < k; j += WAVE) {
            hd[j] = 1e10f;
            hi[j] = pad_with_start ? start : -1;
        }
        for (int base = start; base < end; base += WAVE) {
            const int i = base + lane;
            float d2 = 3.0e38f;
            if (i < end) d2 = ref_d2(qx, qy, qz, xyz[3 * i], xyz[3 * i + 1], xyz[3 * i + 2]);
            unsigned long long mask = __ballot(d2 < hd[0]);
            while (mask) {
                const int l = __builtin_ctzll(mask);
                mask &= mask - 1;
                const float cd = __shfl(d2, l, WAVE);
                if (cd < hd[0]) {
                    hd[0] = cd;
                    hi[0] = base + l;
                    ex_reheap(hd, hi, k);
                }
            }
        }
        for (int i = k - 1; i > 0; --i) {
            float td = hd[0]; hd[0] = hd[i]; hd[i] = td;
            int ti = hi[0]; hi[0] = hi[i]; hi[i] = ti;
            ex_reheap(hd, hi, i);
        }
        for (int j = lane; j < k; j += WAVE) {
            idx[(size_t)q * k + j] = hi[j];
            dist2[(size_t)q * k + j] = hd[j];
        }
    }
}

constexpr int EXW_WAVES = 16, EXW_PER_LANE = 4, EXW_CHUNK = EXW_WAVES * WAVE * EXW_PER_LANE, EXW_CAP = 1024;

__device__ __forceinline__ float lane_get_f(float v, int node) { return __int_as_float(__builtin_amdgcn_readlane(__float_as_int(v), node)); }
__device__ __forceinline__ int lane_get_i(int v, int node) { return __builtin_amdgcn_readlane(v, node); }
__device__ __forceinline__ void lane_set_f(float &v, int node, float x) { v = ((int)(threadIdx.x & 63) == node) ? x : v; }
__device__ __forceinline__ void lane_set_i(int &v, int node, int x) { v = ((int)(threadIdx.x & 63) == node) ? x : v; }
__device__ __forceinline__ void lanes_reheap(float &hd, int &hi, int k, float rd, int ri) {
    int root = 0, child = 1;
    while (child < k) {
        float cd = lane_get_f(hd, child);
        if (child + 1 < k) {
            const float c1 = lane_get_f(hd, child + 1);
            if (c1 > cd) { child++; cd = c1; }
        }
        if (rd > cd) break;
        lane_set_f(hd, root, cd);
        lane_set_i(hi, root, lane_get_i(hi, child));
        root = child;
        child = __builtin_amdgcn_readfirstlane(root * 2 + 1);
    }
    lane_set_f(hd, root, rd);
    lane_set_i(hi, root, ri);
}

__global__ __launch_bounds__(EXW_WAVES *WAVE) void knn_exact_wide_kernel(
    int k, const float *__restrict__ xyz, const float *__restrict__ new_xyz, const int *__restrict__ offset,
    const int *__restrict__ new_offset, int b, int *__restrict__ idx, float *__restrict__ dist2, int pad_with_start,
    const int *__restrict__ tie_count, const int *__restrict__ tie_list) {
    __shared__ float s_root;
    __shared__ float s_cd[EXW_CAP];
    __shared__ int s_ci[EXW_CAP];
    __shared__ int s_cnt[EXW_WAVES * EXW_PER_LANE + 1];
    const int lane = threadIdx.x & 63, wid = threadIdx.x >> 6;
    const int total = *tie_count;
    for (int w = blockIdx.x; w < total; w += gridDim.x) {
        const int q = tie_list[w];
        const int s = seg_of(q, new_offset, b);
        const int start = s == 0 ? 0 : offset[s - 1];
        const int end = offset[s];
        const float qx = new_xyz[3 * q], qy = new_xyz[3 * q + 1], qz = new_xyz[3 * q + 2];
        float hd = 1e10f;
        int hi = pad_with_start ? start : -1;
        __syncthreads();
        if (threadIdx.x == 0) s_root = 1e10f;
        __syncthreads();
        float dn[EXW_PER_LANE];
        auto fetch = [&](int cb) {
#pragma unroll
            for (int u = 0; u < EXW_PER_LANE; ++u) {
                const int i = cb + (wid * EXW_PER_LANE + u) * WAVE + lane;
                const bool ok = i < end;
                const size_t ii = ok ? (size_t)i : (size_t)start;
                const float d = ref_d2(qx, qy, qz, xyz[3 * ii], xyz[3 * ii + 1], xyz[3 * ii + 2]);
                dn[u] = ok ? d : 3.0e38f;
            }
        };
        fetch(start);
        for (int cbase = start; cbase < end; cbase += EXW_CHUNK) {
            const float root = s_root;
            float d2[EXW_PER_LANE];
            unsigned long long mk[EXW_PER_LANE];
#pragma unroll
            for (int u = 0; u < EXW_PER_LANE; ++u) d2[u] = dn[u];
            if (cbase + EXW_CHUNK < end) fetch(cbase + EXW_CHUNK);
#pragma unroll
            for (int u = 0; u < EXW_PER_LANE; ++u) {
                mk[u] = __ballot(d2[u] < root);
                if (lane == 0) s_cnt[wid * EXW_PER_LANE + u] = __popcll(mk[u]);
            }
            __syncthreads();
            if (wid == 0) {
                static_assert(EXW_WAVES * EXW_PER_LANE == WAVE, "one count per lane");
                const int c = s_cnt[lane];
                int inc = c;
#pragma unroll
                for (int o = 1; o < WAVE; o <<= 1) {
                    const int y = __shfl_up(inc, o, WAVE);
                    if (lane >= o) inc += y;
                }
                s_cnt[lane] = inc - c;
                if (lane == WAVE - 1) s_cnt[WAVE] = inc;
            }
            __syncthreads();
            const int nsurv = s_cnt[EXW_WAVES * EXW_PER_LANE];
            if (nsurv <= EXW_CAP) {
#pragma unroll
                for (int u = 0; u < EXW_PER_LANE; ++u)
                    if ((mk[u] >> lane) & 1ull) {
                        const int pos = s_cnt[wid * EXW_PER_LANE + u] + __popcll(mk[u] & ((1ull << lane) - 1ull));
                        s_cd[pos] = d2[u];
                        s_ci[pos] = cbase + (wid * EXW_PER_LANE + u) * WAVE + lane;
                    }
            }
            __syncthreads();
            if (wid == 0) {
                float rootv = lane_get_f(hd, 0);
                if (nsurv <= EXW_CAP) {
                    for (int j0 = 0; j0 < nsurv; j0 += WAVE) {
                        const float cdv = j0 + lane < nsurv ? s_cd[j0 + lane] : 3.0e38f;
                        const int civ = j0 + lane < nsurv ? s_ci[j0 + lane] : 0;
                        const int cnt = min(WAVE, nsurv - j0);
                        for (int j = 0; j < cnt; ++j) {
                            const float cd = lane_get_f(cdv, j);
                            if (cd < rootv) {
                                lanes_reheap(hd, hi, k, cd, lane_get_i(civ, j));
                                rootv = lane_get_f(hd, 0);
                            }
                        }
                    }
                } else {
                    const int cend = min(cbase + EXW_CHUNK, end);
                    for (int base = cbase; base < cend; base += WAVE) {
                        const int i = base + lane;
                        float d = 3.0e38f;
                        if (i < cend) d = ref_d2(qx, qy, qz, xyz[3 * (size_t)i], xyz[3 * (size_t)i + 1], xyz[3 * (size_t)i + 2]);
                        unsigned long long mask = __ballot(d < rootv);
                        while (mask) {
                            const int l = __builtin_ctzll(mask);
                            mask &= mask - 1;
                            const float cd = lane_get_f(d, l);
                            if (cd < rootv) {
                                lanes_reheap(hd, hi, k, cd, base + l);
                                rootv = lane_get_f(hd, 0);
                            }
                        }
                    }
                }
                if (lane == 0) s_root = rootv;
            }
            __syncthreads();
        }
        if (wid == 0) {
            for (int i = k - 1; i > 0; --i) {
                const float ld = lane_get_f(hd, i), rd = lane_get_f(hd, 0);
                const int li = lane_get_i(hi, i), ri = lane_get_i(hi, 0);
                lane_set_f(hd, i, rd);
                lane_set_i(hi, i, ri);
                lanes_reheap(hd, hi, i, ld, li);
            }
            if (lane < k) {
                idx[(size_t)q * k + lane] = hi;
                dist2[(size_t)q * k + lane] = hd;
            }
        }
    }
}

thread_local unsigned long long *g_pair_counter = nullptr;

template <int KC>
void launch_query(hipStream_t st, int m, int k, const Workspace &w, const float *new_xyz,
                  const int *offset, const int *new_offset, int b, int *idx, float *dist2,
                  int pad_with_start, int self_mode) {
    if (g_pair_counter)
        hipLaunchKernelGGL((knn_grid_query_kernel<KC, true>), dim3(divup(m, 256)), dim3(256), 0, st, m, k, w.sorted,
                           new_xyz, offset, new_offset, b, w.seg, w.cell_start, idx, dist2, pad_with_start,
                           self_mode, w.tie_count, w.tie_list, g_pair_counter);
    else
        hipLaunchKernelGGL((knn_grid_query_kernel<KC, false>), dim3(divup(m, 256)), dim3(256), 0, st, m, k, w.sorted,
                           new_xyz, offset, new_offset, b, w.seg, w.cell_start, idx, dist2, pad_with_start,
                           self_mode, w.tie_count, w.tie_list, (unsigned long long *)nullptr);
}

}

extern "C" int knn_query_count_pairs(unsigned long long *device_counter) {
    g_pair_counter = device_counter;
    return PTV2_OK;
}

extern "C" size_t knn_query_hip_workspace_bytes(int m, int n, int b) {
    if (m < 0 || n < 0 || b < 1) return 0;
    return carve(nullptr, m, n, b).bytes;
}

extern "C" int knn_query_grid_hip_launcher(int m, int nsample, const float *xyz, const float *new_xyz,
                                           const int *offset, const int *new_offset, int *idx, float *dist2,
                                           int n, int b, int pad_with_start, int grid_mode, int slot, void *workspace,
                                           size_t workspace_bytes, void *stream) {
    if (nsample < 1 || nsample > 128 || m < 0 || n < 0 || b < 1) return PTV2_ERR_ARG;
    if (grid_mode < 0 || grid_mode > 1 || slot < 0 || slot > 3 || (grid_mode == 0 && slot != 0)) return PTV2_ERR_ARG;
    if (m == 0) return PTV2_OK;
    if (!xyz || !new_xyz || !offset || !new_offset || !idx || !dist2) return PTV2_ERR_ARG;
    hipStream_t st = (hipStream_t)stream;
    const int k = nsample;
    if (k > 32 || n == 0) {
        hipLaunchKernelGGL(knn_exact_kernel, dim3(min(divup(m, EX_WAVES), 4096)), dim3(EX_WAVES * WAVE), 0, st, m,
                           k, xyz, new_xyz, offset, new_offset, b, idx, dist2, pad_with_start, (const int *)nullptr,
                           (const int *)nullptr, 1);
        PTV2_CHECK_LAUNCH();
        return PTV2_OK;
    }
    Workspace w = carve(workspace, m, n, b);
    if (!workspace || workspace_bytes < w.bytes) return PTV2_ERR_WORKSPACE;
    const long long ncell_ll = (long long)CELLS_PER_POINT * n + b + 1;
    if (ncell_ll + SCAN_TILE > 0x7fffffffLL) return PTV2_ERR_ARG;
    const int ncell = (int)ncell_ll;
    const int ntiles = divup(ncell + 1, SCAN_TILE);
    const int ncell_pad = ntiles * SCAN_TILE;
    const int self_mode = (new_xyz == xyz && new_offset == offset && m == n) ? 1 : 0;

    w.tie_count += slot;
    if (grid_mode == 0) {
    hipLaunchKernelGGL(knn_init_kernel, dim3(min(divup(ncell_pad, 256), 1024)), dim3(256), 0, st, w.tie_count,
                       w.bbox_lo, w.bbox_hi, b, w.cell_count, ncell_pad, w.block_sums, ntiles);
    hipLaunchKernelGGL(knn_bbox_kernel, dim3(divup(n, 256)), dim3(256), 0, st, n, xyz, offset, b, w.bbox_lo,
                       w.bbox_hi);
    static const float occupancy = [] { const char *e = getenv("AO_AMD_KNN_OCC"); const float v = e ? (float)atof(e) : 0.f; return v > 0.f ? v : 0.7f; }();
    hipLaunchKernelGGL(knn_cell_count_kernel, dim3(divup(n, 256)), dim3(256), 0, st, n, xyz, offset, b, (const int *)w.bbox_lo,
                       (const int *)w.bbox_hi, occupancy, w.seg, w.cell_count, w.point_cell, w.point_rank);
    hipLaunchKernelGGL(knn_scan_kernel, dim3(ntiles), dim3(SCAN_THREADS), 0, st, (const int *)w.cell_count, w.block_sums,
                       w.cell_start, ntiles);
    hipLaunchKernelGGL(knn_scatter_kernel, dim3(divup(n, 256)), dim3(256), 0, st, n, xyz, w.cell_start, w.point_cell,
                       w.point_rank, w.sorted);
    }
    {
    PtvScopedTimer qt(KID_KNN_QUERY, st, 12.0 * n + 12.0 * m + 8.0 * (double)m * k);
    if (k <= 16) {
        const dim3 grid(divup((long long)m * 16, 256)), blk(256);
#define ROWQ(KK)                                                                                                                   \
        do {                                                                                                                       \
            if (g_pair_counter)                                                                                                    \
                hipLaunchKernelGGL((knn_row_query_kernel<KK, true>), grid, blk, 0, st, m, k, w.sorted, new_xyz, offset, new_offset, b, \
                                   w.seg, w.cell_start, idx, dist2, pad_with_start, self_mode, w.tie_count, w.tie_list,            \
                                   g_pair_counter);                                                                                \
            else                                                                                                                   \
                hipLaunchKernelGGL((knn_row_query_kernel<KK, false>), grid, blk, 0, st, m, k, w.sorted, new_xyz, offset, new_offset, b, \
                                   w.seg, w.cell_start, idx, dist2, pad_with_start, self_mode, w.tie_count, w.tie_list,            \
                                   (unsigned long long *)nullptr);                                                                 \
        } while (0)
        if (k == 16) ROWQ(16);
        else if (k == 8) ROWQ(8);
        else if (k == 3) ROWQ(3);
        else if (k == 1) ROWQ(1);
        else ROWQ(0);
#undef ROWQ
    }
    else launch_query<33>(st, m, k, w, new_xyz, offset, new_offset, b, idx, dist2, pad_with_start, self_mode);
    }
    hipLaunchKernelGGL(knn_exact_wide_kernel, dim3(128), dim3(EXW_WAVES * WAVE), 0, st, k, xyz, new_xyz, offset, new_offset, b, idx,
                       dist2, pad_with_start, (const int *)w.tie_count, (const int *)w.tie_list);
    PTV2_CHECK_LAUNCH();
    return PTV2_OK;
}

extern "C" int knn_query_hip_launcher(int m, int nsample, const float *xyz, const float *new_xyz,
                                      const int *offset, const int *new_offset, int *idx, float *dist2,
                                      int n, int b, int pad_with_start, void *workspace,
                                      size_t workspace_bytes, void *stream) {
    return knn_query_grid_hip_launcher(m, nsample, xyz, new_xyz, offset, new_offset, idx, dist2, n, b, pad_with_start, 0, 0,
                                       workspace, workspace_bytes, stream);
}
```

ao_amd/csrc/pool.hip:

```cpp
#include <algorithm>

#include "common.h"

namespace {

constexpr int TPB = 256;
constexpr int MM_CHUNKS = 64;

__global__ __launch_bounds__(TPB) void segment_minmax_partial(int b, const float *__restrict__ xyz,
                                                             const int *__restrict__ offset, float *__restrict__ part) {
    __shared__ float s_lo[TPB / WAVE][3], s_hi[TPB / WAVE][3];
    const int seg = blockIdx.x / MM_CHUNKS, chunk = blockIdx.x - seg * MM_CHUNKS;
    const int start = seg == 0 ? 0 : offset[seg - 1], end = offset[seg];
    float lo[3] = {3.0e38f, 3.0e38f, 3.0e38f}, hi[3] = {-3.0e38f, -3.0e38f, -3.0e38f};
    for (int i = start + chunk * TPB + threadIdx.x; i < end; i += MM_CHUNKS * TPB) {
#pragma unroll
        for (int a = 0; a < 3; ++a) {
            const float v = xyz[3 * (size_t)i + a];
            lo[a] = fminf(lo[a], v);
            hi[a] = fmaxf(hi[a], v);
        }
    }
#pragma unroll
    for (int a = 0; a < 3; ++a) {
#pragma unroll
        for (int o = 32; o >= 1; o >>= 1) {
            lo[a] = fminf(lo[a], __shfl_xor(lo[a], o, WAVE));
            hi[a] = fmaxf(hi[a], __shfl_xor(hi[a], o, WAVE));
        }
        if ((threadIdx.x & 63) == 0) { s_lo[threadIdx.x >> 6][a] = lo[a]; s_hi[threadIdx.x >> 6][a] = hi[a]; }
    }
    __syncthreads();
    if (threadIdx.x < 3) {
        float l = s_lo[0][threadIdx.x], h = s_hi[0][threadIdx.x];
        for (int w = 1; w < TPB / WAVE; ++w) { l = fminf(l, s_lo[w][threadIdx.x]); h = fmaxf(h, s_hi[w][threadIdx.x]); }
        part[(size_t)blockIdx.x * 6 + threadIdx.x] = l;
        part[(size_t)blockIdx.x * 6 + 3 + threadIdx.x] = h;
    }
}

__global__ void segment_minmax_final(int b, const float *__restrict__ part, float *__restrict__ lo, float *__restrict__ hi) {
    const int t = blockIdx.x * blockDim.x + threadIdx.x;
    if (t >= b * 3) return;
    const int seg = t / 3, a = t - seg * 3;
    float l = 3.0e38f, h = -3.0e38f;
    for (int ch = 0; ch < MM_CHUNKS; ++ch) {
        l = fminf(l, part[((size_t)seg * MM_CHUNKS + ch) * 6 + a]);
        h = fmaxf(h, part[((size_t)seg * MM_CHUNKS + ch) * 6 + 3 + a]);
    }
    lo[t] = l;
    hi[t] = h;
}

template <int VEC>
__global__ __launch_bounds__(TPB) void pool_max_fwd(long long total, int cv, const float *__restrict__ feat,
                                                    const int *__restrict__ order, const int *__restrict__ idx_ptr,
                                                    float *__restrict__ out, int *__restrict__ arg) {
    for (long long e = (long long)blockIdx.x * TPB + threadIdx.x; e < total; e += (long long)gridDim.x * TPB) {
        const int j = (int)(e / cv), q = (int)(e - (long long)j * cv);
        const int p0 = idx_ptr[j], p1 = idx_ptr[j + 1];
        if (VEC == 4) {
            int r0 = order[p0];
            float4 best = ((const float4 *)feat)[(size_t)r0 * cv + q];
            int4 bi = make_int4(r0, r0, r0, r0);
            constexpr int UB = 8;
            for (int p = p0 + 1; p < p1; p += UB) {
                int r[UB];
                float4 v[UB];
#pragma unroll
                for (int u = 0; u < UB; ++u) r[u] = p + u < p1 ? order[p + u] : -1;
#pragma unroll
                for (int u = 0; u < UB; ++u)
                    if (r[u] >= 0) v[u] = ((const float4 *)feat)[(size_t)r[u] * cv + q];
#pragma unroll
                for (int u = 0; u < UB; ++u)
                    if (r[u] >= 0) {
                        if (v[u].x > best.x) { best.x = v[u].x; bi.x = r[u]; }
                        if (v[u].y > best.y) { best.y = v[u].y; bi.y = r[u]; }
                        if (v[u].z > best.z) { best.z = v[u].z; bi.z = r[u]; }
                        if (v[u].w > best.w) { best.w = v[u].w; bi.w = r[u]; }
                    }
            }
            ((float4 *)out)[e] = best;
            ((int4 *)arg)[e] = bi;
        } else {
            int r0 = order[p0];
            float best = feat[(size_t)r0 * cv + q];
            int bi = r0;
            for (int p = p0 + 1; p < p1; ++p) {
                const int r = order[p];
                const float v = feat[(size_t)r * cv + q];
                if (v > best) { best = v; bi = r; }
            }
            out[e] = best;
            arg[e] = bi;
        }
    }
}

__global__ __launch_bounds__(TPB) void pool_max_bwd(long long total, int c, const float *__restrict__ grad_out,
                                                    const int *__restrict__ arg, float *__restrict__ grad_feat) {
    for (long long e = (long long)blockIdx.x * TPB + threadIdx.x; e < total; e += (long long)gridDim.x * TPB) {
        const int ch = (int)(e % c);
        grad_feat[(size_t)arg[e] * c + ch] = grad_out[e];
    }
}

}

extern "C" size_t segment_minmax_hip_workspace_bytes(int b) { return sizeof(float) * 6 * (size_t)MM_CHUNKS * (b > 0 ? b : 1) + 256; }

extern "C" int segment_minmax_hip_launcher(int b, const float *xyz, const int *offset, float *lo, float *hi,
                                           void *workspace, size_t workspace_bytes, void *stream) {
    if (b < 1) return PTV2_ERR_ARG;
    if (!workspace || workspace_bytes < segment_minmax_hip_workspace_bytes(b)) return PTV2_ERR_WORKSPACE;
    hipStream_t st = (hipStream_t)stream;
    hipLaunchKernelGGL(segment_minmax_partial, dim3(b * MM_CHUNKS), dim3(TPB), 0, st, b, xyz, offset, (float *)workspace);
    hipLaunchKernelGGL(segment_minmax_final, dim3(divup(b * 3, 64)), dim3(64), 0, st, b, (const float *)workspace, lo, hi);
    PTV2_CHECK_LAUNCH();
    return PTV2_OK;
}

extern "C" int pool_max_forward_hip_launcher(int n_out, int c, const float *feat, const int *order, const int *idx_ptr,
                                             float *out, int *arg, void *stream) {
    if (n_out < 0 || c < 1) return PTV2_ERR_ARG;
    if (n_out == 0) return PTV2_OK;
    hipStream_t st = (hipStream_t)stream;
    const bool vec = c % 4 == 0 && (((uintptr_t)feat | (uintptr_t)out | (uintptr_t)arg) & 15) == 0;
    const int cv = vec ? c / 4 : c;
    const long long total = (long long)n_out * cv;
    const int nblk = (int)std::min<long long>((total + TPB - 1) / TPB, 256 * 8);
    if (vec) hipLaunchKernelGGL(pool_max_fwd<4>, dim3(nblk), dim3(TPB), 0, st, total, cv, feat, order, idx_ptr, out, arg);
    else hipLaunchKernelGGL(pool_max_fwd<1>, dim3(nblk), dim3(TPB), 0, st, total, cv, feat, order, idx_ptr, out, arg);
    PTV2_CHECK_LAUNCH();
    return PTV2_OK;
}

extern "C" int pool_max_backward_hip_launcher(int n_out, int c, const float *grad_out, const int *arg,
                                              float *grad_feat, void *stream) {
    if (n_out < 0 || c < 1) return PTV2_ERR_ARG;
    const long long total = (long long)n_out * c;
    if (total == 0) return PTV2_OK;
    const int nblk = (int)std::min<long long>((total + TPB - 1) / TPB, 256 * 8);
    hipLaunchKernelGGL(pool_max_bwd, dim3(nblk), dim3(TPB), 0, (hipStream_t)stream, total, c, grad_out, arg, grad_feat);
    PTV2_CHECK_LAUNCH();
    return PTV2_OK;
}

namespace {
template <int VEC>
__global__ __launch_bounds__(TPB) void segment_sum_rows(long long total, int cv, const float *__restrict__ grad_fine,
                                                        const int *__restrict__ order, const int *__restrict__ idx_ptr,
                                                        float *__restrict__ grad_coarse) {
    for (long long e = (long long)blockIdx.x * TPB + threadIdx.x; e < total; e += (long long)gridDim.x * TPB) {
        const int j = (int)(e / cv), q = (int)(e - (long long)j * cv);
        if (VEC == 4) {
            float4 acc = make_float4(0.f, 0.f, 0.f, 0.f);
            for (int p = idx_ptr[j]; p < idx_ptr[j + 1]; ++p) {
                const float4 v = ((const float4 *)grad_fine)[(size_t)order[p] * cv + q];
                acc.x += v.x; acc.y += v.y; acc.z += v.z; acc.w += v.w;
            }
            ((float4 *)grad_coarse)[e] = acc;
        } else {
            float acc = 0.f;
            for (int p = idx_ptr[j]; p < idx_ptr[j + 1]; ++p) acc += grad_fine[(size_t)order[p] * cv + q];
            grad_coarse[e] = acc;
        }
    }
}
}

extern "C" int segment_sum_hip_launcher(int n_out, int c, const float *grad_fine, const int *order, const int *idx_ptr,
                                        float *grad_coarse, void *stream) {
    if (n_out < 0 || c < 1 || !grad_fine || !order || !idx_ptr || !grad_coarse) return PTV2_ERR_ARG;
    if (n_out == 0) return PTV2_OK;
    const bool vec = c % 4 == 0;
    const int cv = vec ? c / 4 : c;
    const long long total = (long long)n_out * cv;
    const int nblk = (int)std::min<long long>((total + TPB - 1) / TPB, 256 * 16);
    if (vec) hipLaunchKernelGGL(segment_sum_rows<4>, dim3(nblk), dim3(TPB), 0, (hipStream_t)stream, total, cv, grad_fine, order, idx_ptr, grad_coarse);
    else hipLaunchKernelGGL(segment_sum_rows<1>, dim3(nblk), dim3(TPB), 0, (hipStream_t)stream, total, cv, grad_fine, order, idx_ptr, grad_coarse);
    PTV2_CHECK_LAUNCH();
    return PTV2_OK;
}
```

ao_amd/ptv2/parallel.py:

```python
import os
import time

import torch
import torch.distributed as dist


def rank_world():
    return int(os.environ.get("RANK", 0)), int(os.environ.get("LOCAL_RANK", 0)), int(os.environ.get("WORLD_SIZE", 1))


def scene_seeds(rank, scenes_per_rank):
    return [rank * scenes_per_rank + i for i in range(scenes_per_rank)]


def wrap_ddp(module, device):
    ids = [device.index] if device.type == "cuda" else None
    return torch.nn.parallel.DistributedDataParallel(module, device_ids=ids, broadcast_buffers=False,
                                                     gradient_as_bucket_view=True)


class FlatGradSync:

    def __init__(self, module, force=False, mode="flat"):
        self.force = force
        self.params = [p for p in module.parameters() if p.requires_grad]
        self.world = dist.get_world_size() if dist.is_available() and dist.is_initialized() else 1
        self.split, self.event, self.comm = None, None, None
        if mode == "flat2":
            backbone = getattr(module, "backbone", module)
            names = [n for n, p in module.named_parameters() if p.requires_grad]
            first = next((i for i, n in enumerate(names) if "dec_stages." in n), None)
            if first is not None and first > 0 and torch.cuda.is_available() and self.params[0].is_cuda:
                off = 0
                for p in self.params[:first]:
                    off += (p.numel() + 3) // 4 * 4
                self.split = off
                self.event = torch.cuda.Event()
                self.event.record()
                self.comm = torch.cuda.Stream(self.params[0].device)
                backbone.__dict__["native_decoder_done_event"] = self.event
                self.backbone, self.seen = backbone, backbone.__dict__.get("native_decoder_done_count", 0)
        if self.world > 1:
            flat = torch._utils._flatten_dense_tensors([p.data for p in self.params])
            dist.broadcast(flat, 0)
            for p, f in zip(self.params, torch._utils._unflatten_dense_tensors(flat, [p.data for p in self.params])):
                p.data.copy_(f)

    def sync(self):
        if self.world == 1 and not self.force:
            return
        grads = [p.grad for p in self.params if p.grad is not None]
        flat = torch._utils._flatten_dense_tensors(grads)
        dist.all_reduce(flat)
        flat.div_(self.world)
        torch._foreach_copy_(grads, list(torch._utils._unflatten_dense_tensors(flat, grads)))

    def reduce_flat(self, flat):
        if self.world > 1 or self.force:
            recorded = self.split is not None and self.backbone.__dict__.get("native_decoder_done_count", 0) != self.seen
            if recorded:
                self.seen = self.backbone.__dict__["native_decoder_done_count"]
                rt = self.backbone.__dict__.get("_ao_runtime")
                direct = rt is not None and rt._grad_buf is not None and flat.data_ptr() == rt._grad_buf.data_ptr()
                recorded = direct and not self.backbone.__dict__.get("native_last_backward_accumulated", True)
            if recorded and 0 < self.split < flat.numel():
                main = torch.cuda.current_stream(flat.device)
                self.comm.wait_event(self.event)
                with torch.cuda.stream(self.comm):
                    dist.all_reduce(flat[self.split:])
                dist.all_reduce(flat[:self.split])
                main.wait_stream(self.comm)
            else:
                dist.all_reduce(flat)
        return 1.0 / self.world


def fence(device):
    if dist.is_available() and dist.is_initialized() and dist.get_world_size() > 1:
        dist.barrier()
    if device.type == "cuda":
        torch.cuda.synchronize(device)


def timed_steps(step_fn, steps, device, points_this_rank, finish=None):
    fence(device)
    t0 = time.perf_counter()
    loss = None
    for _ in range(steps):
        loss = step_fn()
    if finish is not None:
        finish()
    fence(device)
    elapsed = time.perf_counter() - t0
    t = torch.tensor([elapsed], device=device, dtype=torch.float64)
    pts = torch.tensor([float(points_this_rank)], device=device, dtype=torch.float64)
    if dist.is_available() and dist.is_initialized() and dist.get_world_size() > 1:
        dist.all_reduce(t, op=dist.ReduceOp.MAX)
        dist.all_reduce(pts, op=dist.ReduceOp.SUM)
    return float(t.item()), float(pts.item()), loss


def _geometry_tensors(geo):
    if hasattr(geo, "tensors"):
        yield from geo.tensors()
        return
    for lv in geo.levels:
        for v in vars(lv).values():
            if torch.is_tensor(v):
                yield v
                for t in getattr(v, "_ao_inverse", ()) or ():
                    if torch.is_tensor(t):
                        yield t
        for idx in lv.knn.values():
            yield idx
            for attr in ("_ao_inverse", "_ao_pos_moments"):
                for t in getattr(idx, attr, ()) or ():
                    if torch.is_tensor(t):
                        yield t


class GeometryPrefetcher:

    def __init__(self, backbone, device, threaded=False):
        self.backbone, self.device = backbone, device
        self.stream = torch.cuda.Stream(device)
        self.threaded, self.worker = threaded, None
        import collections
        self.done = collections.deque()
        self.outstanding = 0
        if threaded:
            import queue
            self.requests, self.results = queue.Queue(), queue.Queue()

    def _build(self, coord, offset, ready):
        if ready is not None:
            self.stream.wait_event(ready)
        with torch.no_grad(), torch.cuda.stream(self.stream):
            geo = self.backbone.geometry(coord, offset)
            done = torch.cuda.Event()
            done.record(self.stream)
        return geo, done

    def _loop(self):
        torch.cuda.set_device(self.device)
        while True:
            req = self.requests.get()
            if req is None:
                return
            try:
                self.results.put(self._build(*req))
            except BaseException as e:
                self.results.put(e)

    def start(self, coord, offset, ready=None):
        self.outstanding += 1
        if not self.threaded:
            self.done.append(self._build(coord, offset, ready))
            return
        if self.worker is None:
            import threading
            self.worker = threading.Thread(target=self._loop, name="ao_amd-geometry", daemon=True)
            self.worker.start()
        self.requests.put((coord, offset, ready))

    @property
    def pending(self):
        return self.outstanding if self.outstanding else None

    def close(self):
        if self.threaded and self.worker is not None:
            self.requests.put(None)
            self.worker.join()
            self.worker = None
            while not self.results.empty():
                self.results.get()
        self.done.clear()
        self.outstanding = 0

    def take(self):
        assert self.outstanding > 0, "GeometryPrefetcher.take() before start()"
        self.outstanding -= 1
        res = self.results.get() if self.threaded else self.done.popleft()
        if isinstance(res, BaseException):
            raise res
        geo, done = res
        main = torch.cuda.current_stream(self.device)
        main.wait_event(done)
        for t in _geometry_tensors(geo):
            t.record_stream(main)
        return geo
```

Measured before the change: 12.84 million.

## Cap geometry kernel grids on background stream and register-sort small pool clusters

Adds a thread-local workgroup cap for geometry kernels, used by the background prefetch stream so it leaves CUs free for the concurrent training kernels. Geometry kernels become grid-stride so they stay correct under a capped grid, and the KNN row query gets a walking variant. Separately, the grid-pool mean kernel sorts and sums clusters of up to 16 members in registers with a bitonic network instead of insertion sort in global memory. The default cap is zero, so capping only applies when the env variable is set; the register path raises register pressure.

```diff
diff --git a/ao_amd/_abi.py b/ao_amd/_abi.py
--- a/ao_amd/_abi.py
+++ b/ao_amd/_abi.py
@@ -146,3 +146,9 @@
     raise RuntimeError("ao_amd: %s not found: the ctypes bindings are derived from it" % INSEVAL_HEADER)
 with open(INSEVAL_HEADER) as _f:
     inseval_consts, inseval_structs, inseval_signatures = parse(_f.read())
+
+GEOMETRY_HEADER = os.path.join(os.path.dirname(HEADER), "ptv2_geometry_hip.h")
+if not os.path.exists(GEOMETRY_HEADER):
+    raise RuntimeError("ao_amd: %s not found: the ctypes bindings are derived from it" % GEOMETRY_HEADER)
+with open(GEOMETRY_HEADER) as _f:
+    geometry_consts, geometry_structs, geometry_signatures = parse(_f.read())
diff --git a/ao_amd/_lib.py b/ao_amd/_lib.py
--- a/ao_amd/_lib.py
+++ b/ao_amd/_lib.py
@@ -43,7 +43,7 @@
         handle = ctypes.CDLL(LIB_PATH)
         for table in (_SIGNATURES, _abi.data_signatures, _abi.refine_signatures, _abi.pp2s_signatures,
                       _abi.ptv1_signatures, _abi.spconv_signatures, _abi.pg_signatures, _abi.msc_signatures,
-                      _abi.st_signatures, _abi.inseval_signatures):
+                      _abi.st_signatures, _abi.inseval_signatures, _abi.geometry_signatures):
             for name, (res, args) in table.items():
                 try:
                     fn = getattr(handle, name)
diff --git a/ao_amd/csrc/abi.hip b/ao_amd/csrc/abi.hip
--- a/ao_amd/csrc/abi.hip
+++ b/ao_amd/csrc/abi.hip
@@ -5,6 +5,7 @@
 #include <unordered_map>
 #include <vector>
 
+#include "../../include/ptv2_geometry_hip.h"
 #include "gva_common.h"
 
 extern "C" int ptv2_abi_version(void) { return 11; }
@@ -26,6 +27,19 @@
 extern "C" int ptv2_matmul_precision(int bf16) {
     const int prev = g_matmul_bf16;
     if (bf16 >= 0) g_matmul_bf16 = bf16 ? 1 : 0;
+    return prev;
+}
+
+constexpr int GEOM_WGS_DEFAULT = 0;
+namespace { thread_local int g_geometry_wgs = 0; }
+int ptv2_geometry_wgs(void) { return g_geometry_wgs; }
+extern "C" int ptv2_geometry_background_enable(int max_workgroups) {
+    const int prev = g_geometry_wgs;
+    if (max_workgroups < 0) {
+        const char *e = getenv("AO_AMD_GEOM_WGS");
+        max_workgroups = e ? atoi(e) : GEOM_WGS_DEFAULT;
+    }
+    g_geometry_wgs = max_workgroups > 0 ? max_workgroups : 0;
     return prev;
 }
 
diff --git a/ao_amd/csrc/common.h b/ao_amd/csrc/common.h
--- a/ao_amd/csrc/common.h
+++ b/ao_amd/csrc/common.h
@@ -19,6 +19,7 @@
     } while (0)
 
 static inline int divup(long long a, long long b) { return (int)((a + b - 1) / b); }
+__device__ __forceinline__ int divup_dev(long long a, int b) { return (int)((a + b - 1) / b); }
 
 static constexpr size_t ptv2_align256(size_t v) { return (v + 255) & ~(size_t)255; }
 struct PtvCarver {
@@ -29,6 +30,12 @@
 
 static inline bool ptv2_env_set(const char *name) { return getenv(name) != nullptr; }
 static inline bool ptv2_env_is(const char *name, char c) { const char *e = getenv(name); return e && e[0] == c; }
+
+int ptv2_geometry_wgs(void);
+static inline unsigned ptv2_geom_grid(long long natural) {
+    const int cap = ptv2_geometry_wgs();
+    return (unsigned)((cap > 0 && natural > cap) ? cap : natural);
+}
 
 enum PtvKernelId {
     KID_KNN_QUERY = 0, KID_LOGITS_FWD, KID_SOFTMAX_ROWS, KID_AGG_TILE, KID_PEB_FWD, KID_PEB_BWD, KID_BWD_TILE,
diff --git a/ao_amd/csrc/gather_ops.hip b/ao_amd/csrc/gather_ops.hip
--- a/ao_amd/csrc/gather_ops.hip
+++ b/ao_amd/csrc/gather_ops.hip
@@ -315,7 +315,7 @@
     if (m == 0) return PTV2_OK;
     if (!dist2 || !idx || !weight) return PTV2_ERR_ARG;
     const int nblk = (int)std::min<long long>(((long long)m + 255) / 256, 256 * 8);
-    hipLaunchKernelGGL(interpolation_weights_kernel, dim3(nblk), dim3(256), 0, (hipStream_t)stream, (long long)m, k, n, dist2, idx,
+    hipLaunchKernelGGL(interpolation_weights_kernel, dim3(ptv2_geom_grid(nblk)), dim3(256), 0, (hipStream_t)stream, (long long)m, k, n, dist2, idx,
                        weight);
     PTV2_CHECK_LAUNCH();
     return PTV2_OK;
diff --git a/ao_amd/csrc/gridpool.hip b/ao_amd/csrc/gridpool.hip
--- a/ao_amd/csrc/gridpool.hip
+++ b/ao_amd/csrc/gridpool.hip
@@ -12,6 +12,7 @@
     long long total;
 };
 constexpr int KEY_BITS = 48;
+constexpr int MEAN_REG = 16;
 
 __device__ __forceinline__ PoolDims pool_dims_of(int b, const float *__restrict__ lo, const float *__restrict__ hi, float size) {
     float e[3] = {0.f, 0.f, 0.f};
@@ -79,24 +80,66 @@
     const int m = *n_out;
     for (int j = blockIdx.x * TPB + threadIdx.x; j < m; j += gridDim.x * TPB) {
         const int p0 = idx_ptr[j], p1 = idx_ptr[j + 1];
-        if (sort_members) {
-            for (int p = p0 + 1; p < p1; ++p) {
-                const int v = order[p];
-                int q = p - 1;
-                while (q >= p0 && order[q] > v) { order[q + 1] = order[q]; --q; }
-                order[q + 1] = v;
-            }
-        }
         float sx = 0.f, sy = 0.f, sz = 0.f;
-        for (int p = p0; p < p1; ++p) {
-            const size_t r = (size_t)order[p];
-            sx += coord[3 * r]; sy += coord[3 * r + 1]; sz += coord[3 * r + 2];
+        int first;
+        if (p1 - p0 >= 1 && p1 - p0 <= MEAN_REG) {
+            const int cnt = p1 - p0;
+            int v[MEAN_REG];
+#pragma unroll
+            for (int u = 0; u < MEAN_REG; ++u) {
+                const int w = order[p0 + min(u, cnt - 1)];
+                v[u] = u < cnt ? w : 0x7fffffff;
+            }
+            if (sort_members) {
+#pragma unroll
+                for (int k = 2; k <= MEAN_REG; k <<= 1)
+#pragma unroll
+                    for (int d = k >> 1; d > 0; d >>= 1)
+#pragma unroll
+                        for (int u = 0; u < MEAN_REG; ++u) {
+                            const int l = u ^ d;
+                            if (l > u) {
+                                const int lo = min(v[u], v[l]), hi = max(v[u], v[l]);
+                                const bool up = (u & k) == 0;
+                                v[u] = up ? lo : hi;
+                                v[l] = up ? hi : lo;
+                            }
+                        }
+#pragma unroll
+                for (int u = 0; u < MEAN_REG; ++u)
+                    if (u < cnt) order[p0 + u] = v[u];
+            }
+            float cx[MEAN_REG], cy[MEAN_REG], cz[MEAN_REG];
+#pragma unroll
+            for (int u = 0; u < MEAN_REG; ++u) {
+                const size_t r = (size_t)(u < cnt ? v[u] : v[0]);
+                cx[u] = coord[3 * r]; cy[u] = coord[3 * r + 1]; cz[u] = coord[3 * r + 2];
+            }
+#pragma unroll
+            for (int u = 0; u < MEAN_REG; ++u) {
+                sx = u < cnt ? sx + cx[u] : sx; sy = u < cnt ? sy + cy[u] : sy; sz = u < cnt ? sz + cz[u] : sz;
+            }
+            first = v[0];
+        } else {
+            if (sort_members) {
+                for (int p = p0 + 1; p < p1; ++p) {
+                    const int v = order[p];
+                    int q = p - 1;
+                    while (q >= p0 && order[q] > v) { order[q + 1] = order[q]; --q; }
+                    order[q + 1] = v;
+                }
+            }
+            for (int p = p0; p < p1; ++p) {
+                const size_t r = (size_t)order[p];
+                sx += coord[3 * r]; sy += coord[3 * r + 1]; sz += coord[3 * r + 2];
+            }
+            first = order[p0];
         }
         const float cnt = (float)(p1 - p0);
         new_coord[3 * (size_t)j] = sx / cnt;
         new_coord[3 * (size_t)j + 1] = sy / cnt;
         new_coord[3 * (size_t)j + 2] = sz / cnt;
-        const int s0 = seg_of(order[p0], offset, b);
+        const int s0 = seg_of(first, offset, b);
         const int s1 = (j + 1 < m) ? seg_of(order[idx_ptr[j + 1]], offset, b) : b;
         for (int s = s0; s < s1; ++s) new_offset[s] = j + 1;
         if (j == 0)
@@ -128,48 +171,52 @@
                                                          const float *__restrict__ lo, float size, const PoolDims *__restrict__ dims,
                                                          const int *__restrict__ n_out, int *__restrict__ count,
                                                          int *__restrict__ key32, int *__restrict__ slot) {
-    const int i = blockIdx.x * TPB + threadIdx.x;
-    if (i >= n || *n_out < 0) return;
-    const int s = seg_of(i, offset, b);
-    const long long cx = (long long)((coord[3 * (size_t)i] - lo[3 * s]) / size);
-    const long long cy = (long long)((coord[3 * (size_t)i + 1] - lo[3 * s + 1]) / size);
-    const long long cz = (long long)((coord[3 * (size_t)i + 2] - lo[3 * s + 2]) / size);
-    const long long nx = dims->nx, ny = dims->ny, nz = dims->nz;
-    const int key = (int)(cx + cy * nx + cz * nx * ny + (long long)s * nx * ny * nz);
-    key32[i] = key;
-    slot[i] = atomicAdd(&count[key], 1);
+    if (*n_out < 0) return;
+    const int nblocks = divup_dev(n, TPB);
+    for (int vb = blockIdx.x; vb < nblocks; vb += gridDim.x) {
+        const int i = vb * TPB + threadIdx.x;
+        if (i >= n) return;
+        const int s = seg_of(i, offset, b);
+        const long long cx = (long long)((coord[3 * (size_t)i] - lo[3 * s]) / size);
+        const long long cy = (long long)((coord[3 * (size_t)i + 1] - lo[3 * s + 1]) / size);
+        const long long cz = (long long)((coord[3 * (size_t)i + 2] - lo[3 * s + 2]) / size);
+        const long long nx = dims->nx, ny = dims->ny, nz = dims->nz;
+        const int key = (int)(cx + cy * nx + cz * nx * ny + (long long)s * nx * ny * nz);
+        key32[i] = key;
+        slot[i] = atomicAdd(&count[key], 1);
+    }
 }
 
 __global__ __launch_bounds__(DSCAN_THREADS) void dense_scan_reduce_kernel(const PoolDims *__restrict__ dims, const int *__restrict__ n_out,
                                                                           const int *__restrict__ count, int2 *__restrict__ tile_sums) {
-    if (*n_out < 0 || (long long)blockIdx.x * DSCAN_TILE >= dims->total) return;
     __shared__ int2 s_w[DSCAN_THREADS / WAVE];
-    const int4 *p = (const int4 *)(count + (size_t)blockIdx.x * DSCAN_TILE) + threadIdx.x * 2;
-    const int4 a = p[0], c = p[1];
-    int v = a.x + a.y + a.z + a.w + c.x + c.y + c.z + c.w;
-    int o = (a.x > 0) + (a.y > 0) + (a.z > 0) + (a.w > 0) + (c.x > 0) + (c.y > 0) + (c.z > 0) + (c.w > 0);
-#pragma unroll
-    for (int d = 32; d >= 1; d >>= 1) { v += __shfl_xor(v, d, WAVE); o += __shfl_xor(o, d, WAVE); }
-    if ((threadIdx.x & 63) == 0) s_w[threadIdx.x >> 6] = make_int2(v, o);
-    __syncthreads();
-    if (threadIdx.x == 0) {
-        int2 t = make_int2(0, 0);
-        for (int i = 0; i < DSCAN_THREADS / WAVE; ++i) { t.x += s_w[i].x; t.y += s_w[i].y; }
-        tile_sums[blockIdx.x] = t;
-    }
-}
-
-__global__ __launch_bounds__(DSCAN_THREADS) void dense_scan_apply_kernel(const PoolDims *__restrict__ dims, int *n_out, int n,
-                                                                         const int *__restrict__ count, const int2 *__restrict__ tile_sums,
-                                                                         int2 *__restrict__ base, int *__restrict__ idx_ptr,
-                                                                         int *__restrict__ over) {
+    if (*n_out < 0) return;
     const long long total = dims->total;
-    if (*n_out < 0 || (long long)blockIdx.x * DSCAN_TILE >= total) return;
-    __shared__ int2 s_w[DSCAN_THREADS / WAVE];
-    __shared__ int2 s_base;
+    for (int vb = blockIdx.x; (long long)vb * DSCAN_TILE < total; vb += gridDim.x) {
+        const int4 *p = (const int4 *)(count + (size_t)vb * DSCAN_TILE) + threadIdx.x * 2;
+        const int4 a = p[0], c = p[1];
+        int v = a.x + a.y + a.z + a.w + c.x + c.y + c.z + c.w;
+        int o = (a.x > 0) + (a.y > 0) + (a.z > 0) + (a.w > 0) + (c.x > 0) + (c.y > 0) + (c.z > 0) + (c.w > 0);
+#pragma unroll
+        for (int d = 32; d >= 1; d >>= 1) { v += __shfl_xor(v, d, WAVE); o += __shfl_xor(o, d, WAVE); }
+        if ((threadIdx.x & 63) == 0) s_w[threadIdx.x >> 6] = make_int2(v, o);
+        __syncthreads();
+        if (threadIdx.x == 0) {
+            int2 t = make_int2(0, 0);
+            for (int i = 0; i < DSCAN_THREADS / WAVE; ++i) { t.x += s_w[i].x; t.y += s_w[i].y; }
+            tile_sums[vb] = t;
+        }
+        __syncthreads();
+    }
+}
+
+__device__ __forceinline__ void dense_scan_apply_tile(int vb, int2 (&s_w)[DSCAN_THREADS / WAVE], int2 &s_base, long long total,
+                                                      int *n_out, int n, const int *__restrict__ count,
+                                                      const int2 *__restrict__ tile_sums, int2 *__restrict__ base,
+                                                      int *__restrict__ idx_ptr, int *__restrict__ over) {
     const int lane = threadIdx.x & 63, wid = threadIdx.x >> 6;
     int2 part = make_int2(0, 0);
-    for (int i = threadIdx.x; i < (int)blockIdx.x; i += DSCAN_THREADS) { const int2 t = tile_sums[i]; part.x += t.x; part.y += t.y; }
+    for (int i = threadIdx.x; i < vb; i += DSCAN_THREADS) { const int2 t = tile_sums[i]; part.x += t.x; part.y += t.y; }
 #pragma unroll
     for (int d = 32; d >= 1; d >>= 1) { part.x += __shfl_xor(part.x, d, WAVE); part.y += __shfl_xor(part.y, d, WAVE); }
     if (lane == 0) s_w[wid] = part;
@@ -182,7 +229,7 @@
     __syncthreads();
     const int2 tb = s_base;
     __syncthreads();
-    const int4 *p = (const int4 *)(count + (size_t)blockIdx.x * DSCAN_TILE) + threadIdx.x * 2;
+    const int4 *p = (const int4 *)(count + (size_t)vb * DSCAN_TILE) + threadIdx.x * 2;
     const int4 a = p[0], c = p[1];
     const int v[8] = {a.x, a.y, a.z, a.w, c.x, c.y, c.z, c.w};
     int ex[8], eo[8], tot = 0, occ = 0, big = 0;
@@ -200,14 +247,27 @@
     int wx = 0, wo = 0;
     for (int i = 0; i < wid; ++i) { wx += s_w[i].x; wo += s_w[i].y; }
     const int bx = tb.x + wx + inc - tot, bo = tb.y + wo + inco - occ;
-    int2 *q = base + (size_t)blockIdx.x * DSCAN_TILE + (size_t)threadIdx.x * 8;
+    int2 *q = base + (size_t)vb * DSCAN_TILE + (size_t)threadIdx.x * 8;
 #pragma unroll
     for (int i = 0; i < 8; ++i) q[i] = make_int2(bx + ex[i], bo + eo[i]);
     const long long last_tile = (total - 1) / DSCAN_TILE;
-    if ((long long)blockIdx.x == last_tile && threadIdx.x == DSCAN_THREADS - 1) {
+    if ((long long)vb == last_tile && threadIdx.x == DSCAN_THREADS - 1) {
         const int m = bo + occ;
         *n_out = m;
         idx_ptr[m] = n;
+    }
+}
+__global__ __launch_bounds__(DSCAN_THREADS) void dense_scan_apply_kernel(const PoolDims *__restrict__ dims, int *n_out, int n,
+                                                                         const int *__restrict__ count, const int2 *__restrict__ tile_sums,
+                                                                         int2 *__restrict__ base, int *__restrict__ idx_ptr,
+                                                                         int *__restrict__ over) {
+    __shared__ int2 s_w[DSCAN_THREADS / WAVE];
+    __shared__ int2 s_base;
+    const long long total = dims->total;
+    if (*n_out < 0) return;
+    for (int vb = blockIdx.x; (long long)vb * DSCAN_TILE < total; vb += gridDim.x) {
+        dense_scan_apply_tile(vb, s_w, s_base, total, n_out, n, count, tile_sums, base, idx_ptr, over);
+        __syncthreads();
     }
 }
 
@@ -215,12 +275,16 @@
                                                             const int *__restrict__ slot, const int2 *__restrict__ base,
                                                             long long *__restrict__ cluster, int *__restrict__ order,
                                                             int *__restrict__ idx_ptr) {
-    const int i = blockIdx.x * TPB + threadIdx.x;
-    if (i >= n || *n_out < 0) return;
-    const int2 bb = base[key32[i]];
-    cluster[i] = bb.y;
-    order[bb.x + slot[i]] = i;
-    if (slot[i] == 0) idx_ptr[bb.y] = bb.x;
+    if (*n_out < 0) return;
+    const int nblocks = divup_dev(n, TPB);
+    for (int vb = blockIdx.x; vb < nblocks; vb += gridDim.x) {
+        const int i = vb * TPB + threadIdx.x;
+        if (i >= n) return;
+        const int2 bb = base[key32[i]];
+        cluster[i] = bb.y;
+        order[bb.x + slot[i]] = i;
+        if (slot[i] == 0) idx_ptr[bb.y] = bb.x;
+    }
 }
 
 struct Ws {
@@ -282,17 +346,17 @@
                            w.dims);
     if (!sort_path) {
         const int ztiles = (int)((w.d_cells + DSCAN_TILE) / DSCAN_TILE);
-        hipLaunchKernelGGL(dense_zero_kernel, dim3(1024), dim3(TPB), 0, st, b, (const float *)w.lo, (const float *)w.hi, grid_size,
+        hipLaunchKernelGGL(dense_zero_kernel, dim3(ptv2_geom_grid(1024)), dim3(TPB), 0, st, b, (const float *)w.lo, (const float *)w.hi, grid_size,
                            w.dims, w.d_count, n_out, w.d_cells, w.d_over);
-        hipLaunchKernelGGL(dense_keys_kernel, dim3(nb), dim3(TPB), 0, st, n, b, coord, offset, (const float *)w.lo, grid_size,
+        hipLaunchKernelGGL(dense_keys_kernel, dim3(ptv2_geom_grid(nb)), dim3(TPB), 0, st, n, b, coord, offset, (const float *)w.lo, grid_size,
                            (const PoolDims *)w.dims, (const int *)n_out, w.d_count, w.d_key, w.d_slot);
-        hipLaunchKernelGGL(dense_scan_reduce_kernel, dim3(ztiles), dim3(DSCAN_THREADS), 0, st, (const PoolDims *)w.dims,
+        hipLaunchKernelGGL(dense_scan_reduce_kernel, dim3(ptv2_geom_grid(ztiles)), dim3(DSCAN_THREADS), 0, st, (const PoolDims *)w.dims,
                            (const int *)n_out, (const int *)w.d_count, w.d_tiles);
-        hipLaunchKernelGGL(dense_scan_apply_kernel, dim3(ztiles), dim3(DSCAN_THREADS), 0, st, (const PoolDims *)w.dims, n_out, n,
+        hipLaunchKernelGGL(dense_scan_apply_kernel, dim3(ptv2_geom_grid(ztiles)), dim3(DSCAN_THREADS), 0, st, (const PoolDims *)w.dims, n_out, n,
                            (const int *)w.d_count, (const int2 *)w.d_tiles, w.d_base, idx_ptr, w.d_over);
-        hipLaunchKernelGGL(dense_scatter_kernel, dim3(nb), dim3(TPB), 0, st, n, (const int *)n_out, (const int *)w.d_key,
+        hipLaunchKernelGGL(dense_scatter_kernel, dim3(ptv2_geom_grid(nb)), dim3(TPB), 0, st, n, (const int *)n_out, (const int *)w.d_key,
                            (const int *)w.d_slot, (const int2 *)w.d_base, cluster, order, idx_ptr);
-        hipLaunchKernelGGL(pool_mean_kernel, dim3(std::min(nb, 2048)), dim3(TPB), 0, st, n_out, b, coord, offset,
+        hipLaunchKernelGGL(pool_mean_kernel, dim3(ptv2_geom_grid(std::min(nb, 2048))), dim3(TPB), 0, st, n_out, b, coord, offset,
                            order, (const int *)idx_ptr, new_coord, new_offset, 1, (const int *)w.d_over);
         PTV2_CHECK_LAUNCH();
         return PTV2_OK;
@@ -308,7 +372,7 @@
     if (hipcub::DeviceScan::InclusiveSum(w.cub, cb, (const int *)w.flags, w.rank, n, st) != hipSuccess) return PTV2_ERR_LAUNCH;
     hipLaunchKernelGGL(pool_scatter_kernel, dim3(nb), dim3(TPB), 0, st, n, (const int *)w.rank, (const int *)w.flags,
                        (const int *)order, cluster, idx_ptr, n_out, (const PoolDims *)w.dims);
-    hipLaunchKernelGGL(pool_mean_kernel, dim3(std::min(nb, 2048)), dim3(TPB), 0, st, n_out, b, coord, offset,
+    hipLaunchKernelGGL(pool_mean_kernel, dim3(ptv2_geom_grid(std::min(nb, 2048))), dim3(TPB), 0, st, n_out, b, coord, offset,
                        order, (const int *)idx_ptr, new_coord, new_offset, 0, (const int *)nullptr);
     PTV2_CHECK_LAUNCH();
     return PTV2_OK;
diff --git a/ao_amd/csrc/gva_fwd.hip b/ao_amd/csrc/gva_fwd.hip
--- a/ao_amd/csrc/gva_fwd.hip
+++ b/ao_amd/csrc/gva_fwd.hip
@@ -5,26 +5,29 @@
 namespace gva {
 
 __global__ __launch_bounds__(TPB) void pos_stats_kernel(int n, int k, const float *__restrict__ coord,
-                                                        const int *__restrict__ idx, float *__restrict__ part) {
+                                                        const int *__restrict__ idx, float *__restrict__ part, int nblk) {
     __shared__ float s_w[WPB][9];
     const long long rows = (long long)n * k;
-    float acc[9] = {0, 0, 0, 0, 0, 0, 0, 0, 0};
-    for (long long row = (long long)blockIdx.x * TPB + threadIdx.x; row < rows; row += (long long)gridDim.x * TPB) {
-        Rel r = rel_pos(coord, idx, row, (int)(row / k));
-        acc[0] += r.x; acc[1] += r.y; acc[2] += r.z;
-        acc[3] += r.x * r.x; acc[4] += r.x * r.y; acc[5] += r.x * r.z;
-        acc[6] += r.y * r.y; acc[7] += r.y * r.z; acc[8] += r.z * r.z;
-    }
-#pragma unroll
-    for (int j = 0; j < 9; ++j) {
-        float v = wave_sum(acc[j]);
-        if ((threadIdx.x & 63) == 0) s_w[threadIdx.x >> 6][j] = v;
-    }
-    __syncthreads();
-    if (threadIdx.x < 9) {
-        float v = 0.f;
-        for (int w = 0; w < WPB; ++w) v += s_w[w][threadIdx.x];
-        part[blockIdx.x * 9 + threadIdx.x] = v;
+    for (int vb = blockIdx.x; vb < nblk; vb += gridDim.x) {
+        float acc[9] = {0, 0, 0, 0, 0, 0, 0, 0, 0};
+        for (long long row = (long long)vb * TPB + threadIdx.x; row < rows; row += (long long)nblk * TPB) {
+            Rel r = rel_pos(coord, idx, row, (int)(row / k));
+            acc[0] += r.x; acc[1] += r.y; acc[2] += r.z;
+            acc[3] += r.x * r.x; acc[4] += r.x * r.y; acc[5] += r.x * r.z;
+            acc[6] += r.y * r.y; acc[7] += r.y * r.z; acc[8] += r.z * r.z;
+        }
+#pragma unroll
+        for (int j = 0; j < 9; ++j) {
+            float v = wave_sum(acc[j]);
+            if ((threadIdx.x & 63) == 0) s_w[threadIdx.x >> 6][j] = v;
+        }
+        __syncthreads();
+        if (threadIdx.x < 9) {
+            float v = 0.f;
+            for (int w = 0; w < WPB; ++w) v += s_w[w][threadIdx.x];
+            part[vb * 9 + threadIdx.x] = v;
+        }
+        __syncthreads();
     }
 }
 
@@ -196,7 +199,7 @@
     hipStream_t st = (hipStream_t)stream;
     float *part = (float *)workspace;
     int nblk = stage_grid((long long)n * k, TPB * 4);
-    hipLaunchKernelGGL(pos_stats_kernel, dim3(nblk), dim3(TPB), 0, st, n, k, coord, idx, part);
+    hipLaunchKernelGGL(pos_stats_kernel, dim3(ptv2_geom_grid(nblk)), dim3(TPB), 0, st, n, k, coord, idx, part, nblk);
     launch_finalize(st, (const float *)part, nblk, 9, MapPosStats{s1, s2});
     PTV2_CHECK_LAUNCH();
     return PTV2_OK;
@@ -240,7 +243,7 @@
     hipStream_t st = (hipStream_t)stream;
     float *part = (float *)workspace;
     const int nblk = stage_grid((long long)n * k, TPB * 4);
-    hipLaunchKernelGGL(pos_stats_kernel, dim3(nblk), dim3(TPB), 0, st, n, k, coord, idx, part);
+    hipLaunchKernelGGL(pos_stats_kernel, dim3(ptv2_geom_grid(nblk)), dim3(TPB), 0, st, n, k, coord, idx, part, nblk);
     hipLaunchKernelGGL(pos_moments_finalize_kernel, dim3(1), dim3(1024), 0, st, (const float *)part, nblk, (double)n * k, mu, cov);
     PTV2_CHECK_LAUNCH();
     return PTV2_OK;
diff --git a/ao_amd/csrc/inverse.hip b/ao_amd/csrc/inverse.hip
--- a/ao_amd/csrc/inverse.hip
+++ b/ao_amd/csrc/inverse.hip
@@ -37,14 +37,13 @@
 __device__ __forceinline__ int key_of(int v, int n) { return ((unsigned)v < (unsigned)n) ? v + 1 : 0; }
 
 template <bool SPREAD>
-__global__ __launch_bounds__(TPB) void inv_split_kernel(InvJobs J, int *__restrict__ cells, int2 *__restrict__ pairs,
-                                                        unsigned long long *__restrict__ handoff, int handoff_words,
-                                                        int cells_used, int cells_padded) {
-    __shared__ int s_part[MAX_PARTS];
-    const int t = job_of(J.chunk0, J.count, blockIdx.x);
-    const int chunk = blockIdx.x - J.chunk0[t], parts = J.parts[t], chunks = J.chunks[t], shift = J.shift[t], n = J.n[t];
+__device__ __forceinline__ void inv_split_chunk(int vb, int (&s_part)[MAX_PARTS], const InvJobs &J, int *__restrict__ cells,
+                                                int2 *__restrict__ pairs, unsigned long long *__restrict__ handoff,
+                                                int handoff_words, int cells_used, int cells_padded) {
+    const int t = job_of(J.chunk0, J.count, vb);
+    const int chunk = vb - J.chunk0[t], parts = J.parts[t], chunks = J.chunks[t], shift = J.shift[t], n = J.n[t];
     int *cell = cells + J.cell0[t] + chunk;
-    if (!SPREAD && blockIdx.x == 0) {
+    if (!SPREAD && vb == 0) {
         for (int i = threadIdx.x; i < handoff_words; i += TPB) handoff[i] = 0ull;
         for (int i = cells_used + threadIdx.x; i < cells_padded; i += TPB) cells[i] = 0;
     }
@@ -60,6 +59,17 @@
     if (!SPREAD) {
         __syncthreads();
         for (int p = threadIdx.x; p < parts; p += TPB) cell[(size_t)p * chunks] = s_part[p];
+    }
+}
+template <bool SPREAD>
+__global__ __launch_bounds__(TPB) void inv_split_kernel(InvJobs J, int *__restrict__ cells, int2 *__restrict__ pairs,
+                                                        unsigned long long *__restrict__ handoff, int handoff_words,
+                                                        int cells_used, int cells_padded) {
+    __shared__ int s_part[MAX_PARTS];
+    const int nblocks = J.chunk0[INV_MAX];
+    for (int vb = blockIdx.x; vb < nblocks; vb += gridDim.x) {
+        inv_split_chunk<SPREAD>(vb, s_part, J, cells, pairs, handoff, handoff_words, cells_used, cells_padded);
+        __syncthreads();
     }
 }
 
@@ -129,15 +139,14 @@
     }
 }
 
-__global__ __launch_bounds__(TPB) void inv_build_kernel(InvJobs J, const int *__restrict__ cells, const int2 *__restrict__ pairs,
-                                                        int *__restrict__ spill) {
-    extern __shared__ int lds[];
-    const int t = job_of(J.part0, J.count, blockIdx.x);
-    const int p = blockIdx.x - J.part0[t], shift = J.shift[t], width = 1 << shift, n = J.n[t], chunks = J.chunks[t];
+__device__ __forceinline__ void inv_build_part(int vb, int *lds, int (&s_wave)[TPB / 64], const InvJobs &J,
+                                               const int *__restrict__ cells, const int2 *__restrict__ pairs,
+                                               int *__restrict__ spill) {
+    const int t = job_of(J.part0, J.count, vb);
+    const int p = vb - J.part0[t], shift = J.shift[t], width = 1 << shift, n = J.n[t], chunks = J.chunks[t];
     int *s_start = lds;
     int *s_cur = lds + width + 1;
     int *s_stage = s_cur + width;
-    __shared__ int s_wave[TPB / 64];
     const int tid = threadIdx.x, lane = tid & 63, wid = tid >> 6;
     const int *cell = cells + J.cell0[t] + (size_t)p * chunks;
     const int P0 = cell[0];
@@ -202,6 +211,16 @@
             const int *src = place + m0;
             order_bucket([src](int e) { return __builtin_nontemporal_load(src + e); }, s, inv_rows + m0, l);
         }
+    }
+}
+__global__ __launch_bounds__(TPB) void inv_build_kernel(InvJobs J, const int *__restrict__ cells, const int2 *__restrict__ pairs,
+                                                        int *__restrict__ spill) {
+    extern __shared__ int lds[];
+    __shared__ int s_wave[TPB / 64];
+    const int nblocks = J.part0[INV_MAX];
+    for (int vb = blockIdx.x; vb < nblocks; vb += gridDim.x) {
+        inv_build_part(vb, lds, s_wave, J, cells, pairs, spill);
+        __syncthreads();
     }
 }
 
@@ -288,13 +307,13 @@
                                    (int)build_lds_bytes(MAX_WIDTH)) == hipSuccess;
     }();
     if (!raised) return PTV2_ERR_LAUNCH;
-    const dim3 chunks((unsigned)P.total_chunks);
+    const dim3 chunks(ptv2_geom_grid(P.total_chunks));
     hipLaunchKernelGGL(inv_split_kernel<false>, chunks, dim3(TPB), 0, st, P.J, cells, pairs, handoff, P.scan_wgs, P.cells_used,
                        P.cells_padded);
     hipLaunchKernelGGL(inv_scan_kernel, dim3((unsigned)P.scan_wgs), dim3(SCAN_TPB), 0, st, cells, handoff);
     hipLaunchKernelGGL(inv_split_kernel<true>, chunks, dim3(TPB), 0, st, P.J, cells, pairs, handoff, P.scan_wgs, P.cells_used,
                        P.cells_padded);
-    hipLaunchKernelGGL(inv_build_kernel, dim3((unsigned)P.total_parts), dim3(TPB), lds, st, P.J, (const int *)cells,
+    hipLaunchKernelGGL(inv_build_kernel, dim3(ptv2_geom_grid(P.total_parts)), dim3(TPB), lds, st, P.J, (const int *)cells,
                        (const int2 *)pairs, spill);
     PTV2_CHECK_LAUNCH();
     return PTV2_OK;
diff --git a/ao_amd/csrc/knn.hip b/ao_amd/csrc/knn.hip
--- a/ao_amd/csrc/knn.hip
+++ b/ao_amd/csrc/knn.hip
@@ -52,19 +52,17 @@
     int t = blockIdx.x * blockDim.x + threadIdx.x;
     for (int i = t; i < ntiles; i += gridDim.x * blockDim.x) block_sums[i] = 0;
     if (t < 4) tie_count[t] = 0;
-    if (t < 3 * b) {
-        bbox_lo[t] = 0x7fffffff;
-        bbox_hi[t] = (int)0x80000000;
+    for (int i = t; i < 3 * b; i += gridDim.x * blockDim.x) {
+        bbox_lo[i] = 0x7fffffff;
+        bbox_hi[i] = (int)0x80000000;
     }
     for (int i = t; i < ncell_pad; i += gridDim.x * blockDim.x) cell_count[i] = 0;
 }
 
-__global__ __launch_bounds__(256) void knn_bbox_kernel(int n, const float *__restrict__ xyz,
-                                                       const int *__restrict__ offset, int b,
-                                                       int *bbox_lo, int *bbox_hi) {
-    __shared__ int s_lo[3], s_hi[3];
-    int t = blockIdx.x * 256 + threadIdx.x;
-    int first = blockIdx.x * 256, last = min(first + 255, n - 1);
+__device__ __forceinline__ void knn_bbox_block(int vb, int (&s_lo)[3], int (&s_hi)[3], int n, const float *__restrict__ xyz,
+                                               const int *__restrict__ offset, int b, int *bbox_lo, int *bbox_hi) {
+    int t = vb * 256 + threadIdx.x;
+    int first = vb * 256, last = min(first + 255, n - 1);
     int seg_first = seg_of(first, offset, b), seg_last = seg_of(last, offset, b);
     bool valid = t < n;
     float x = 0, y = 0, z = 0;
@@ -106,6 +104,16 @@
         atomicMax(&bbox_hi[s * 3 + 1], f2ord(y));
         atomicMin(&bbox_lo[s * 3 + 2], f2ord(z));
         atomicMax(&bbox_hi[s * 3 + 2], f2ord(z));
+    }
+}
+__global__ __launch_bounds__(256) void knn_bbox_kernel(int n, const float *__restrict__ xyz,
+                                                       const int *__restrict__ offset, int b,
+                                                       int *bbox_lo, int *bbox_hi) {
+    __shared__ int s_lo[3], s_hi[3];
+    const int nblocks = divup_dev(n, 256);
+    for (int vb = blockIdx.x; vb < nblocks; vb += gridDim.x) {
+        knn_bbox_block(vb, s_lo, s_hi, n, xyz, offset, b, bbox_lo, bbox_hi);
+        __syncthreads();
     }
 }
 
@@ -157,20 +165,18 @@
 }
 
 constexpr int COUNT_SEGS = 64;
-__global__ __launch_bounds__(256) void knn_cell_count_kernel(int n, const float *__restrict__ xyz,
-                                                             const int *__restrict__ offset, int b,
-                                                             const int *bbox_lo, const int *bbox_hi, float occupancy,
-                                                             SegGrid *seg, int *cell_count, int *point_cell,
-                                                             int *point_rank) {
-    __shared__ SegGrid s_grid[COUNT_SEGS];
-    const int first = blockIdx.x * 256, last = min(first + 255, n - 1);
+__device__ __forceinline__ void knn_cell_count_block(int vb, SegGrid (&s_grid)[COUNT_SEGS], int n, const float *__restrict__ xyz,
+                                                     const int *__restrict__ offset, int b, const int *bbox_lo,
+                                                     const int *bbox_hi, float occupancy, SegGrid *seg, int *cell_count,
+                                                     int *point_cell, int *point_rank) {
+    const int first = vb * 256, last = min(first + 255, n - 1);
     const int s0 = seg_of(first, offset, b), s1 = seg_of(last, offset, b);
     for (int s = s0 + (int)threadIdx.x; s <= s1; s += 256) {
         const SegGrid g = seg_grid_of(s, offset, bbox_lo, bbox_hi, occupancy);
         if (s - s0 < COUNT_SEGS) s_grid[s - s0] = g;
         if (g.n_pts > 0 && g.start >= first) seg[s] = g;
     }
-    if (blockIdx.x == 0)
+    if (vb == 0)
         for (int s = (int)threadIdx.x; s < b; s += 256) {
             const int start = s == 0 ? 0 : offset[s - 1];
             if (offset[s] - start <= 0) seg[s] = seg_grid_of(s, offset, bbox_lo, bbox_hi, occupancy);
@@ -187,6 +193,18 @@
     point_cell[t] = cell;
     point_rank[t] = atomicAdd(&cell_count[cell], 1);
 }
+__global__ __launch_bounds__(256) void knn_cell_count_kernel(int n, const float *__restrict__ xyz,
+                                                             const int *__restrict__ offset, int b,
+                                                             const int *bbox_lo, const int *bbox_hi, float occupancy,
+                                                             SegGrid *seg, int *cell_count, int *point_cell,
+                                                             int *point_rank) {
+    __shared__ SegGrid s_grid[COUNT_SEGS];
+    const int nblocks = divup_dev(n, 256);
+    for (int vb = blockIdx.x; vb < nblocks; vb += gridDim.x) {
+        knn_cell_count_block(vb, s_grid, n, xyz, offset, b, bbox_lo, bbox_hi, occupancy, seg, cell_count, point_cell, point_rank);
+        __syncthreads();
+    }
+}
 
 __global__ __launch_bounds__(SCAN_THREADS) void knn_scan_kernel(const int *__restrict__ in, int *block_sums, int *out, int ntiles) {
     __shared__ int s_w[SCAN_THREADS / WAVE];
@@ -257,10 +275,13 @@
                                                           const int *__restrict__ point_cell,
                                                           const int *__restrict__ point_rank,
                                                           float4 *sorted) {
-    int t = blockIdx.x * 256 + threadIdx.x;
-    if (t >= n) return;
-    int pos = cell_start[point_cell[t]] + point_rank[t];
-    sorted[pos] = make_float4(xyz[3 * t], xyz[3 * t + 1], xyz[3 * t + 2], __int_as_float(t));
+    const int nblocks = divup_dev(n, 256);
+    for (int vb = blockIdx.x; vb < nblocks; vb += gridDim.x) {
+        int t = vb * 256 + threadIdx.x;
+        if (t >= n) return;
+        int pos = cell_start[point_cell[t]] + point_rank[t];
+        sorted[pos] = make_float4(xyz[3 * t], xyz[3 * t + 1], xyz[3 * t + 2], __int_as_float(t));
+    }
 }
 
 template <int KC>
@@ -289,13 +310,13 @@
 }
 
 template <int KC, bool COUNT>
-__global__ __launch_bounds__(256) void knn_grid_query_kernel(
-    int m, int k, const float4 *__restrict__ sorted, const float *__restrict__ new_xyz,
+__device__ __forceinline__ void knn_grid_query_block(
+    int vb, int m, int k, const float4 *__restrict__ sorted, const float *__restrict__ new_xyz,
     const int *__restrict__ offset, const int *__restrict__ new_offset, int b,
     const SegGrid *__restrict__ seg, const int *__restrict__ cell_start, int *__restrict__ idx,
     float *__restrict__ dist2, int pad_with_start, int self_mode, int *tie_count, int *tie_list,
     unsigned long long *pairs) {
-    int t = blockIdx.x * 256 + threadIdx.x;
+    int t = vb * 256 + threadIdx.x;
     unsigned visited = 0;
     if (t >= m) return;
     int qid, s;
@@ -392,6 +413,18 @@
             }
     }
 }
+template <int KC, bool COUNT>
+__global__ __launch_bounds__(256) void knn_grid_query_kernel(
+    int m, int k, const float4 *__restrict__ sorted, const float *__restrict__ new_xyz,
+    const int *__restrict__ offset, const int *__restrict__ new_offset, int b,
+    const SegGrid *__restrict__ seg, const int *__restrict__ cell_start, int *__restrict__ idx,
+    float *__restrict__ dist2, int pad_with_start, int self_mode, int *tie_count, int *tie_list,
+    unsigned long long *pairs) {
+    const int nblocks = divup_dev(m, 256);
+    for (int vb = blockIdx.x; vb < nblocks; vb += gridDim.x)
+        knn_grid_query_block<KC, COUNT>(vb, m, k, sorted, new_xyz, offset, new_offset, b, seg, cell_start, idx, dist2,
+                                        pad_with_start, self_mode, tie_count, tie_list, pairs);
+}
 
 __device__ __forceinline__ float row_shr1_f(float x, float fill) {
     return __int_as_float(__builtin_amdgcn_update_dpp(__float_as_int(fill), __float_as_int(x), 0x111, 0xf, 0xf, false));
@@ -533,14 +566,14 @@
 }
 
 template <int K, bool COUNT>
-__global__ __launch_bounds__(256) void knn_row_query_kernel(
-    int m, int k, const float4 *__restrict__ sorted, const float *__restrict__ new_xyz,
+__device__ __forceinline__ void knn_row_query_block(
+    int vb, int m, int k, const float4 *__restrict__ sorted, const float *__restrict__ new_xyz,
     const int *__restrict__ offset, const int *__restrict__ new_offset, int b,
     const SegGrid *__restrict__ seg, const int *__restrict__ cell_start, int *__restrict__ idx,
     float *__restrict__ dist2, int pad_with_start, int self_mode, int *tie_count, int *tie_list,
     unsigned long long *pairs) {
     const int lane = threadIdx.x & 63, r = lane & 15;
-    const int t = (int)(((long long)blockIdx.x * 256 + threadIdx.x) >> 4);
+    const int t = (int)(((long long)vb * 256 + threadIdx.x) >> 4);
     unsigned visited = 0;
     if (t >= m) return;
     int qid, s;
@@ -597,6 +630,23 @@
         const int pad = pad_with_start ? g.start : -1;
         idx[(size_t)qid * k + r] = L.v < 1e10f ? L.vi : pad;
         dist2[(size_t)qid * k + r] = L.v;
+    }
+}
+template <int K, bool COUNT, bool WALK>
+__global__ __launch_bounds__(256) void knn_row_query_kernel(
+    int m, int k, const float4 *__restrict__ sorted, const float *__restrict__ new_xyz,
+    const int *__restrict__ offset, const int *__restrict__ new_offset, int b,
+    const SegGrid *__restrict__ seg, const int *__restrict__ cell_start, int *__restrict__ idx,
+    float *__restrict__ dist2, int pad_with_start, int self_mode, int *tie_count, int *tie_list,
+    unsigned long long *pairs) {
+    if constexpr (!WALK) {
+        knn_row_query_block<K, COUNT>(blockIdx.x, m, k, sorted, new_xyz, offset, new_offset, b, seg, cell_start, idx, dist2,
+                                      pad_with_start, self_mode, tie_count, tie_list, pairs);
+    } else {
+        const int nblocks = divup_dev((long long)m * 16, 256);
+        for (int vb = blockIdx.x; vb < nblocks; vb += gridDim.x)
+            knn_row_query_block<K, COUNT>(vb, m, k, sorted, new_xyz, offset, new_offset, b, seg, cell_start, idx, dist2,
+                                          pad_with_start, self_mode, tie_count, tie_list, pairs);
     }
 }
 
@@ -818,11 +868,11 @@
                   const int *offset, const int *new_offset, int b, int *idx, float *dist2,
                   int pad_with_start, int self_mode) {
     if (g_pair_counter)
-        hipLaunchKernelGGL((knn_grid_query_kernel<KC, true>), dim3(divup(m, 256)), dim3(256), 0, st, m, k, w.sorted,
+        hipLaunchKernelGGL((knn_grid_query_kernel<KC, true>), dim3(ptv2_geom_grid(divup(m, 256))), dim3(256), 0, st, m, k, w.sorted,
                            new_xyz, offset, new_offset, b, w.seg, w.cell_start, idx, dist2, pad_with_start,
                            self_mode, w.tie_count, w.tie_list, g_pair_counter);
     else
-        hipLaunchKernelGGL((knn_grid_query_kernel<KC, false>), dim3(divup(m, 256)), dim3(256), 0, st, m, k, w.sorted,
+        hipLaunchKernelGGL((knn_grid_query_kernel<KC, false>), dim3(ptv2_geom_grid(divup(m, 256))), dim3(256), 0, st, m, k, w.sorted,
                            new_xyz, offset, new_offset, b, w.seg, w.cell_start, idx, dist2, pad_with_start,
                            self_mode, w.tie_count, w.tie_list, (unsigned long long *)nullptr);
 }
@@ -850,7 +900,7 @@
     hipStream_t st = (hipStream_t)stream;
     const int k = nsample;
     if (k > 32 || n == 0) {
-        hipLaunchKernelGGL(knn_exact_kernel, dim3(min(divup(m, EX_WAVES), 4096)), dim3(EX_WAVES * WAVE), 0, st, m,
+        hipLaunchKernelGGL(knn_exact_kernel, dim3(ptv2_geom_grid(min(divup(m, EX_WAVES), 4096))), dim3(EX_WAVES * WAVE), 0, st, m,
                            k, xyz, new_xyz, offset, new_offset, b, idx, dist2, pad_with_start, (const int *)nullptr,
                            (const int *)nullptr, 1);
         PTV2_CHECK_LAUNCH();
@@ -867,32 +917,32 @@
 
     w.tie_count += slot;
     if (grid_mode == 0) {
-    hipLaunchKernelGGL(knn_init_kernel, dim3(min(divup(ncell_pad, 256), 1024)), dim3(256), 0, st, w.tie_count,
+    hipLaunchKernelGGL(knn_init_kernel, dim3(ptv2_geom_grid(min(divup(ncell_pad, 256), 1024))), dim3(256), 0, st, w.tie_count,
                        w.bbox_lo, w.bbox_hi, b, w.cell_count, ncell_pad, w.block_sums, ntiles);
-    hipLaunchKernelGGL(knn_bbox_kernel, dim3(divup(n, 256)), dim3(256), 0, st, n, xyz, offset, b, w.bbox_lo,
+    hipLaunchKernelGGL(knn_bbox_kernel, dim3(ptv2_geom_grid(divup(n, 256))), dim3(256), 0, st, n, xyz, offset, b, w.bbox_lo,
                        w.bbox_hi);
     static const float occupancy = [] { const char *e = getenv("AO_AMD_KNN_OCC"); const float v = e ? (float)atof(e) : 0.f; return v > 0.f ? v : 0.7f; }();
-    hipLaunchKernelGGL(knn_cell_count_kernel, dim3(divup(n, 256)), dim3(256), 0, st, n, xyz, offset, b, (const int *)w.bbox_lo,
+    hipLaunchKernelGGL(knn_cell_count_kernel, dim3(ptv2_geom_grid(divup(n, 256))), dim3(256), 0, st, n, xyz, offset, b, (const int *)w.bbox_lo,
                        (const int *)w.bbox_hi, occupancy, w.seg, w.cell_count, w.point_cell, w.point_rank);
     hipLaunchKernelGGL(knn_scan_kernel, dim3(ntiles), dim3(SCAN_THREADS), 0, st, (const int *)w.cell_count, w.block_sums,
                        w.cell_start, ntiles);
-    hipLaunchKernelGGL(knn_scatter_kernel, dim3(divup(n, 256)), dim3(256), 0, st, n, xyz, w.cell_start, w.point_cell,
+    hipLaunchKernelGGL(knn_scatter_kernel, dim3(ptv2_geom_grid(divup(n, 256))), dim3(256), 0, st, n, xyz, w.cell_start, w.point_cell,
                        w.point_rank, w.sorted);
     }
     {
     PtvScopedTimer qt(KID_KNN_QUERY, st, 12.0 * n + 12.0 * m + 8.0 * (double)m * k);
     if (k <= 16) {
-        const dim3 grid(divup((long long)m * 16, 256)), blk(256);
+        const int natural = divup((long long)m * 16, 256);
+        const dim3 grid(ptv2_geom_grid(natural)), blk(256);
+        const bool walk = (int)grid.x < natural;
+#define ROWQ_(KK, CNT, WLK, PAIRS)                                                                                                 \
+        hipLaunchKernelGGL((knn_row_query_kernel<KK, CNT, WLK>), grid, blk, 0, st, m, k, w.sorted, new_xyz, offset, new_offset, b,  \
+                           w.seg, w.cell_start, idx, dist2, pad_with_start, self_mode, w.tie_count, w.tie_list, PAIRS)
 #define ROWQ(KK)                                                                                                                   \
         do {                                                                                                                       \
-            if (g_pair_counter)                                                                                                    \
-                hipLaunchKernelGGL((knn_row_query_kernel<KK, true>), grid, blk, 0, st, m, k, w.sorted, new_xyz, offset, new_offset, b, \
-                                   w.seg, w.cell_start, idx, dist2, pad_with_start, self_mode, w.tie_count, w.tie_list,            \
-                                   g_pair_counter);                                                                                \
-            else                                                                                                                   \
-                hipLaunchKernelGGL((knn_row_query_kernel<KK, false>), grid, blk, 0, st, m, k, w.sorted, new_xyz, offset, new_offset, b, \
-                                   w.seg, w.cell_start, idx, dist2, pad_with_start, self_mode, w.tie_count, w.tie_list,            \
-                                   (unsigned long long *)nullptr);                                                                 \
+            if (g_pair_counter) { if (walk) ROWQ_(KK, true, true, g_pair_counter); else ROWQ_(KK, true, false, g_pair_counter); }    \
+            else if (walk) ROWQ_(KK, false, true, (unsigned long long *)nullptr);                                                  \
+            else ROWQ_(KK, false, false, (unsigned long long *)nullptr);                                                           \
         } while (0)
         if (k == 16) ROWQ(16);
         else if (k == 8) ROWQ(8);
@@ -900,10 +950,11 @@
         else if (k == 1) ROWQ(1);
         else ROWQ(0);
 #undef ROWQ
+#undef ROWQ_
     }
     else launch_query<33>(st, m, k, w, new_xyz, offset, new_offset, b, idx, dist2, pad_with_start, self_mode);
     }
-    hipLaunchKernelGGL(knn_exact_wide_kernel, dim3(128), dim3(EXW_WAVES * WAVE), 0, st, k, xyz, new_xyz, offset, new_offset, b, idx,
+    hipLaunchKernelGGL(knn_exact_wide_kernel, dim3(ptv2_geom_grid(128)), dim3(EXW_WAVES * WAVE), 0, st, k, xyz, new_xyz, offset, new_offset, b, idx,
                        dist2, pad_with_start, (const int *)w.tie_count, (const int *)w.tie_list);
     PTV2_CHECK_LAUNCH();
     return PTV2_OK;
diff --git a/ao_amd/csrc/pool.hip b/ao_amd/csrc/pool.hip
--- a/ao_amd/csrc/pool.hip
+++ b/ao_amd/csrc/pool.hip
@@ -7,10 +7,10 @@
 constexpr int TPB = 256;
 constexpr int MM_CHUNKS = 64;
 
-__global__ __launch_bounds__(TPB) void segment_minmax_partial(int b, const float *__restrict__ xyz,
-                                                             const int *__restrict__ offset, float *__restrict__ part) {
-    __shared__ float s_lo[TPB / WAVE][3], s_hi[TPB / WAVE][3];
-    const int seg = blockIdx.x / MM_CHUNKS, chunk = blockIdx.x - seg * MM_CHUNKS;
+__device__ __forceinline__ void segment_minmax_chunk(int vb, float (&s_lo)[TPB / WAVE][3], float (&s_hi)[TPB / WAVE][3],
+                                                     const float *__restrict__ xyz, const int *__restrict__ offset,
+                                                     float *__restrict__ part) {
+    const int seg = vb / MM_CHUNKS, chunk = vb - seg * MM_CHUNKS;
     const int start = seg == 0 ? 0 : offset[seg - 1], end = offset[seg];
     float lo[3] = {3.0e38f, 3.0e38f, 3.0e38f}, hi[3] = {-3.0e38f, -3.0e38f, -3.0e38f};
     for (int i = start + chunk * TPB + threadIdx.x; i < end; i += MM_CHUNKS * TPB) {
@@ -34,8 +34,17 @@
     if (threadIdx.x < 3) {
         float l = s_lo[0][threadIdx.x], h = s_hi[0][threadIdx.x];
         for (int w = 1; w < TPB / WAVE; ++w) { l = fminf(l, s_lo[w][threadIdx.x]); h = fmaxf(h, s_hi[w][threadIdx.x]); }
-        part[(size_t)blockIdx.x * 6 + threadIdx.x] = l;
-        part[(size_t)blockIdx.x * 6 + 3 + threadIdx.x] = h;
+        part[(size_t)vb * 6 + threadIdx.x] = l;
+        part[(size_t)vb * 6 + 3 + threadIdx.x] = h;
+    }
+}
+
+__global__ __launch_bounds__(TPB) void segment_minmax_partial(int b, const float *__restrict__ xyz,
+                                                             const int *__restrict__ offset, float *__restrict__ part) {
+    __shared__ float s_lo[TPB / WAVE][3], s_hi[TPB / WAVE][3];
+    for (int vb = blockIdx.x; vb < b * MM_CHUNKS; vb += gridDim.x) {
+        segment_minmax_chunk(vb, s_lo, s_hi, xyz, offset, part);
+        __syncthreads();
     }
 }
 
@@ -115,7 +124,7 @@
     if (b < 1) return PTV2_ERR_ARG;
     if (!workspace || workspace_bytes < segment_minmax_hip_workspace_bytes(b)) return PTV2_ERR_WORKSPACE;
     hipStream_t st = (hipStream_t)stream;
-    hipLaunchKernelGGL(segment_minmax_partial, dim3(b * MM_CHUNKS), dim3(TPB), 0, st, b, xyz, offset, (float *)workspace);
+    hipLaunchKernelGGL(segment_minmax_partial, dim3(ptv2_geom_grid(b * MM_CHUNKS)), dim3(TPB), 0, st, b, xyz, offset, (float *)workspace);
     hipLaunchKernelGGL(segment_minmax_final, dim3(divup(b * 3, 64)), dim3(64), 0, st, b, (const float *)workspace, lo, hi);
     PTV2_CHECK_LAUNCH();
     return PTV2_OK;
diff --git a/ao_amd/ptv2/parallel.py b/ao_amd/ptv2/parallel.py
--- a/ao_amd/ptv2/parallel.py
+++ b/ao_amd/ptv2/parallel.py
@@ -3,6 +3,8 @@
 
 import torch
 import torch.distributed as dist
+
+from .. import _lib
 
 
 def rank_world():
@@ -135,10 +137,14 @@
     def _build(self, coord, offset, ready):
         if ready is not None:
             self.stream.wait_event(ready)
-        with torch.no_grad(), torch.cuda.stream(self.stream):
-            geo = self.backbone.geometry(coord, offset)
-            done = torch.cuda.Event()
-            done.record(self.stream)
+        prev = _lib.lib().ptv2_geometry_background_enable(-1)
+        try:
+            with torch.no_grad(), torch.cuda.stream(self.stream):
+                geo = self.backbone.geometry(coord, offset)
+                done = torch.cuda.Event()
+                done.record(self.stream)
+        finally:
+            _lib.lib().ptv2_geometry_background_enable(prev)
         return geo, done
 
     def _loop(self):
diff --git a/include/ptv2_geometry_hip.h b/include/ptv2_geometry_hip.h
--- /dev/null
+++ b/include/ptv2_geometry_hip.h
@@ -0,0 +1,14 @@
+#ifndef PTV2_GEOMETRY_HIP_H
+#define PTV2_GEOMETRY_HIP_H
+
+#ifdef __cplusplus
+extern "C" {
+#endif
+
+int ptv2_geometry_background_enable(int max_workgroups);
+
+#ifdef __cplusplus
+}
+#endif
+
+#endif
```

Result: no change. 12.82 million (-0.2%).
